# YoshikiMaekawa2000/ccv_mppi_path_tracker

Measured on AMD Instinct MI355X. Metric: trajectory rollouts/s (K×iters/s) + ms/MPPI-iteration, diff-drive T=50, higher is better.
Workload: dtype f64; 1 GPU; C2: diff_drive K=65536 T=50 sinusoid, u_dim=2, launch parameters; samples_per_gpu=65536, horizon=50, state_store=True

## Files before the change

ccv_mppi_path_tracker_amd/build.py:

```python
import os
import shutil
import subprocess

_PKG = os.path.dirname(os.path.abspath(__file__))
CSRC = os.path.join(_PKG, "csrc")
LIBDIR = os.path.join(_PKG, "lib")
LIB = os.path.join(LIBDIR, "libccv_mppi_hip.so")
KERNEL_UNITS = ["k_r4_fb.hip", "k_batch.hip", "k_batch_varied.hip", "k_batch_shift.hip", "k_batch_obst.hip", "k_batch_obst_shift.hip", "k_batch_moving.hip", "k_batch_moving_shift.hip", "k_batch_grid.hip", "k_batch_grid_shift.hip", "k_r4.hip", "k_r3.hip", "k_pc.hip", "k_pc_fb.hip",
                "k_solo.hip", "k_solo_fb.hip", "k_plain.hip", "k_update.hip", "k_fleet.hip", "k_fleet_pred.hip"]
CAPI_UNITS = ["ccv_mppi_capi.hip", "capi_exchange.hip", "capi_resident.hip", "capi_stage.hip", "capi_batch.hip"]
SOURCES = KERNEL_UNITS + ["mppi_launch.hip"] + CAPI_UNITS + ["ccv_mppi_host.cpp", os.path.join("host", "mppi_node.cpp")]
HEADERS = ["capi_internal.h", "mppi_diag.h", "mppi_kernels.h", "mppi_update.h", "mppi_launch.h", "mppi_rollout_pc.h", "mppi_rollout_r3.h", "mppi_rollout_r4.h",
           "mppi_rollout_solo.h", "k_batch_form.h", "mppi_resident.h", "mppi_update_device.h", "mppi_fleet.h", "mppi_fleet_device.h", "fast_trig.h", "noise_spec.h",
           os.path.join("..", "..", "include", "ccv_mppi.h"), os.path.join("..", "..", "include", "ccv_mppi_host.h"),
           os.path.join("..", "..", "include", "ccv_mppi_fleet.h"),
           os.path.join("..", "..", "include", "ccv_mppi_node.hpp")]
DEPS = SOURCES + HEADERS

HIPCC_FLAGS = [
    "--offload-arch=gfx950", "-O3", "-std=c++17", "-fPIC",
    "-ffp-contract=off",
    "-fhip-fp32-correctly-rounded-divide-sqrt",
    "-Wall", "-Wno-unused-result",
]


def hipcc():
    for cand in (shutil.which("hipcc"), "/opt/rocm/bin/hipcc"):
        if cand and os.path.exists(cand):
            return cand
    raise RuntimeError("hipcc not found: the MI355X path cannot be built (there is no CPU fallback)")


def stale():
    if not os.path.exists(LIB):
        return True
    t = os.path.getmtime(LIB)
    return any(os.path.getmtime(os.path.join(CSRC, d)) > t for d in DEPS)


def _run(cmd, verbose):
    if verbose:
        print(" ".join(cmd))
    res = subprocess.run(cmd, capture_output=True, text=True)
    if res.returncode != 0:
        raise RuntimeError("hipcc failed:\n" + " ".join(cmd) + "\n" + res.stdout + res.stderr)
    if verbose and res.stderr:
        print(res.stderr)


def build(force=False, verbose=False, extra_flags=(), out=None, jobs=None):
    if out is None and not force and not stale():
        return LIB
    os.makedirs(LIBDIR, exist_ok=True)
    target = out or LIB
    import fcntl
    with open(os.path.join(LIBDIR, ".build.lock"), "w") as lock:
        fcntl.flock(lock, fcntl.LOCK_EX)
        try:
            if out is None and not force and not stale():
                return LIB
            objdir = os.path.join(os.path.dirname(os.path.abspath(target)), "obj_%s_%d" % (os.path.basename(target), os.getpid()))
            os.makedirs(objdir, exist_ok=True)
            cc = hipcc()
            objs = [os.path.join(objdir, os.path.basename(s).rsplit(".", 1)[0] + ".o") for s in SOURCES]
            cmds = [[cc] + HIPCC_FLAGS + list(extra_flags) + ["-c", "-o", o, os.path.join(CSRC, s)] for s, o in zip(SOURCES, objs)]
            if jobs is None:
                try:
                    jobs = len(os.sched_getaffinity(0))
                except AttributeError:
                    jobs = os.cpu_count() or 1
                jobs = max(1, min(8, jobs))
            from concurrent.futures import ThreadPoolExecutor
            try:
                with ThreadPoolExecutor(jobs) as pool:
                    list(pool.map(lambda c: _run(c, verbose), cmds))
                tmp = target + ".tmp%d" % os.getpid()
                _run([cc, "--offload-arch=gfx950", "-fPIC", "-shared", "-o", tmp] + objs, verbose)
                os.replace(tmp, target)
            finally:
                shutil.rmtree(objdir, ignore_errors=True)
        finally:
            fcntl.flock(lock, fcntl.LOCK_UN)
    return target


if __name__ == "__main__":
    print(build(force=True, verbose=True))
```

ccv_mppi_path_tracker_amd/capi.py:

```python
import ctypes as C
import os

import numpy as np

from . import build as _build

MAX_UDIM = 5
MAX_HORIZON = 128
ABI_VERSION = 1

OK = 0
ERR_INVALID_ARG = -1
ERR_NO_DEVICE = -2
ERR_HIP = -3
ERR_STATE = -4
ERR_ALLOC = -5
ERR_TIMEOUT = -6

DIFF_DRIVE, STEERING_DIFF_DRIVE, FULL_BODY = 0, 1, 2
FLAG_ROLL_OFF, FLAG_STEER_OFF, FLAG_MIN_SHIFT, FLAG_NO_STATE_STORE = 0x1, 0x2, 0x4, 0x8
BATCH_MAX_SAMPLES = 1 << 29
BATCH_KERNEL_PLAIN, BATCH_KERNEL_ONE_WAVE, BATCH_KERNEL_FOUR_WAVE, BATCH_KERNEL_WIDE = 0, 1, 4, 16
BATCH_KERNEL_VARIED = 32
BATCH_KERNEL_SHIFT = 64
BATCH_KERNEL_OBST = 128
BATCH_KERNEL_MOVING = 256
BATCH_KERNEL_GRID = 512
MAX_OBSTACLES = 32
BATCH_TRACE_ROWS = 1024


class Config(C.Structure):
    _fields_ = [
        ("abi_version", C.c_int32), ("model", C.c_int32), ("num_samples", C.c_int32), ("horizon", C.c_int32),
        ("sample_offset", C.c_int32), ("device", C.c_int32), ("flags", C.c_int32), ("reserved", C.c_int32),
        ("control_noise", C.c_double), ("lam", C.c_double), ("v_ref", C.c_double),
        ("u_min", C.c_double * MAX_UDIM), ("u_max", C.c_double * MAX_UDIM),
        ("path_weight", C.c_double), ("v_weight", C.c_double), ("zmp_weight", C.c_double),
        ("roll_v_weight", C.c_double), ("back_weight", C.c_double), ("yaw_weight", C.c_double),
    ]


class Stats(C.Structure):
    _fields_ = [
        ("sum_w", C.c_double), ("min_cost", C.c_double), ("max_cost", C.c_double),
        ("n_zero_weight", C.c_int64), ("nonfinite", C.c_int32), ("reserved", C.c_int32),
        ("device_us", C.c_float), ("rollout_us", C.c_float),
    ]


class Grid(C.Structure):
    _fields_ = [
        ("origin_x", C.c_double), ("origin_y", C.c_double), ("resolution", C.c_double),
        ("outside", C.c_float), ("nx", C.c_int32), ("ny", C.c_int32), ("cells", C.POINTER(C.c_float)),
    ]


_dp = C.POINTER(C.c_double)
_H = C.c_void_p

SIGNATURES = {
    "ccv_mppi_create": (C.c_int, [C.POINTER(Config), C.POINTER(_H)]),
    "ccv_mppi_destroy": (C.c_int, [_H]),
    "ccv_mppi_set_stream": (C.c_int, [_H, C.c_void_p]),
    "ccv_mppi_last_error": (C.c_char_p, [_H]),
    "ccv_mppi_version": (C.c_char_p, []),
    "ccv_mppi_udim": (C.c_int, [C.c_int]),
    "ccv_mppi_set_nominal": (C.c_int, [_H, _dp]),
    "ccv_mppi_get_nominal": (C.c_int, [_H, _dp]),
    "ccv_mppi_iterate": (C.c_int, [_H, _dp, C.c_double, _dp, _dp, C.c_double, C.c_uint64, C.c_uint64, _dp,
                                   C.POINTER(Stats)]),
    "ccv_mppi_iterate_enqueue": (C.c_int, [_H, _dp, C.c_double, _dp, _dp, C.c_double, C.c_uint64, C.c_uint64]),
    "ccv_mppi_synchronize": (C.c_int, [_H]),
    "ccv_mppi_sample": (C.c_int, [_H, C.c_uint64, C.c_uint64]),
    "ccv_mppi_inject_controls": (C.c_int, [_H, _dp]),
    "ccv_mppi_rollout": (C.c_int, [_H, _dp, C.c_double]),
    "ccv_mppi_weights": (C.c_int, [_H, _dp, _dp, C.c_double]),
    "ccv_mppi_update": (C.c_int, [_H, _dp, C.POINTER(Stats)]),
    "ccv_mppi_read_candidates": (C.c_int, [_H, C.c_int32, C.c_int32, C.c_int32, _dp]),
    "ccv_mppi_read_top_candidates": (C.c_int, [_H, C.c_int32, C.POINTER(C.c_int32), _dp, _dp]),
    "ccv_mppi_read_costs": (C.c_int, [_H, C.c_int32, C.c_int32, _dp]),
    "ccv_mppi_read_weights": (C.c_int, [_H, C.c_int32, C.c_int32, _dp]),
    "ccv_mppi_read_controls": (C.c_int, [_H, C.c_int32, C.c_int32, _dp]),
    "ccv_mppi_partials_size": (C.c_int, [_H]),
    "ccv_mppi_iterate_partials_enqueue": (C.c_int, [_H, _dp, C.c_double, _dp, _dp, C.c_double, C.c_uint64,
                                                    C.c_uint64, C.c_void_p]),
    "ccv_mppi_apply_partials_enqueue": (C.c_int, [_H, C.c_void_p]),
    "ccv_mppi_exchange_handle_bytes": (C.c_int, []),
    "ccv_mppi_exchange_create": (C.c_int, [_H, C.c_int32, C.c_int32, C.c_void_p]),
    "ccv_mppi_exchange_connect": (C.c_int, [_H, C.c_void_p]),
    "ccv_mppi_exchange_info": (C.c_int, [_H, C.POINTER(C.c_int32), C.POINTER(C.c_int32), C.POINTER(C.c_int32), C.POINTER(C.c_int32)]),
    "ccv_mppi_iterate_exchange_enqueue": (C.c_int, [_H, _dp, C.c_double, _dp, _dp, C.c_double, C.c_uint64, C.c_uint64]),
    "ccv_mppi_resident_set_path": (C.c_int, [_H, _dp, _dp, C.c_int32, C.c_double]),
    "ccv_mppi_resident_set_pose": (C.c_int, [_H, _dp]),
    "ccv_mppi_resident_step_enqueue": (C.c_int, [_H, C.c_double, C.c_uint64, C.c_uint64, C.c_int32]),
    "ccv_mppi_resident_step_partials_enqueue": (C.c_int, [_H, C.c_double, C.c_uint64, C.c_uint64, C.c_int32, C.c_void_p]),
    "ccv_mppi_resident_step_exchange_enqueue": (C.c_int, [_H, C.c_double, C.c_uint64, C.c_uint64, C.c_int32]),
    "ccv_mppi_resident_read": (C.c_int, [_H, _dp, C.POINTER(C.c_int32), _dp, _dp, _dp, C.POINTER(C.c_int64)]),
    "ccv_mppi_resident_read_trace": (C.c_int, [_H, C.c_int32, _dp, C.POINTER(C.c_int32)]),
    "ccv_mppi_timing_enable": (C.c_int, [_H, C.c_int32]),
    "ccv_mppi_timing_read": (C.c_int, [_H, _dp, _dp, C.POINTER(C.c_int64), C.c_int32]),
    "ccv_mppi_batch_create": (C.c_int, [C.POINTER(Config), C.c_int32, C.POINTER(_H)]),
    "ccv_mppi_batch_destroy": (C.c_int, [_H]),
    "ccv_mppi_batch_set_stream": (C.c_int, [_H, C.c_void_p]),
    "ccv_mppi_batch_synchronize": (C.c_int, [_H]),
    "ccv_mppi_batch_last_error": (C.c_char_p, [_H]),
    "ccv_mppi_batch_size": (C.c_int, [_H]),
    "ccv_mppi_batch_last_kernel": (C.c_int, [_H]),
    "ccv_mppi_batch_set_nominal": (C.c_int, [_H, _dp]),
    "ccv_mppi_batch_get_nominal": (C.c_int, [_H, _dp]),
    "ccv_mppi_batch_set_params": (C.c_int, [_H, C.POINTER(Config)]),
    "ccv_mppi_batch_get_params": (C.c_int, [_H, C.POINTER(Config)]),
    "ccv_mppi_batch_set_min_shift": (C.c_int, [_H, C.c_int32]),
    "ccv_mppi_batch_get_min_shift": (C.c_int, [_H]),
    "ccv_mppi_batch_set_obstacles": (C.c_int, [_H, _dp, C.POINTER(C.c_int32), C.c_int32, _dp]),
    "ccv_mppi_batch_get_obstacles": (C.c_int, [_H, _dp, C.POINTER(C.c_int32), C.c_int32, _dp]),
    "ccv_mppi_batch_set_obstacle_velocities": (C.c_int, [_H, _dp, C.c_int32]),
    "ccv_mppi_batch_get_obstacle_velocities": (C.c_int, [_H, _dp, C.c_int32]),
    "ccv_mppi_batch_set_fleet_prediction": (C.c_int, [_H, C.c_int32]),
    "ccv_mppi_batch_get_fleet_prediction": (C.c_int, [_H]),
    "ccv_mppi_batch_read_fleet_velocities": (C.c_int, [_H, _dp]),
    "ccv_mppi_batch_set_grids": (C.c_int, [_H, C.POINTER(Grid), C.c_int32, C.POINTER(C.c_int32), _dp]),
    "ccv_mppi_batch_get_grids": (C.c_int, [_H, C.POINTER(Grid), C.c_int32, C.POINTER(C.c_int32), C.POINTER(C.c_int32), _dp]),
    "ccv_mppi_batch_read_grid_cells": (C.c_int, [_H, C.c_int32, C.POINTER(C.c_float)]),
    "ccv_mppi_batch_iterate": (C.c_int, [_H, _dp, _dp, _dp, _dp, _dp, C.POINTER(C.c_uint64), C.c_uint64, _dp,
                                         C.POINTER(Stats)]),
    "ccv_mppi_batch_iterate_enqueue": (C.c_int, [_H, _dp, _dp, _dp, _dp, _dp, C.POINTER(C.c_uint64), C.c_uint64]),
    "ccv_mppi_batch_read_costs": (C.c_int, [_H, C.c_int32, C.c_int32, C.c_int32, _dp]),
    "ccv_mppi_batch_read_weights": (C.c_int, [_H, C.c_int32, C.c_int32, C.c_int32, _dp]),
    "ccv_mppi_batch_read_candidates": (C.c_int, [_H, C.c_int32, C.c_int32, C.c_int32, C.c_int32, _dp]),
    "ccv_mppi_batch_timing_enable": (C.c_int, [_H, C.c_int32]),
    "ccv_mppi_batch_timing_read": (C.c_int, [_H, _dp, _dp, C.POINTER(C.c_int64), C.c_int32]),
    "ccv_mppi_batch_resident_set_paths": (C.c_int, [_H, _dp, _dp, C.POINTER(C.c_int32), _dp]),
    "ccv_mppi_batch_resident_set_poses": (C.c_int, [_H, _dp, C.POINTER(C.c_uint64)]),
    "ccv_mppi_batch_resident_step_enqueue": (C.c_int, [_H, C.c_double, C.c_uint64, C.c_int32]),
    "ccv_mppi_batch_resident_read": (C.c_int, [_H, _dp, C.POINTER(C.c_int32), _dp, _dp, _dp, C.POINTER(C.c_int64)]),
    "ccv_mppi_batch_resident_read_trace": (C.c_int, [_H, C.c_int32, C.c_int32, _dp, C.POINTER(C.c_int32)]),
    "ccv_mppi_calc_ref_path": (C.c_int, [_dp, _dp, C.c_int32, C.c_double, C.c_double, C.c_double, C.c_double,
                                         C.c_double, C.c_int32, _dp, _dp, _dp]),
    "ccv_mppi_path_cosine": (C.c_int, [_dp, _dp, _dp, C.c_double, C.c_double, C.c_double, C.c_double, _dp, _dp,
                                       C.c_int32]),
    "ccv_mppi_path_dkan": (C.c_int, [C.c_double, _dp, _dp, C.c_int32]),
    "ccv_mppi_plant_step": (C.c_int, [C.c_int32, _dp, _dp, C.c_double]),
    "ccv_mppi_node_create": (C.c_int, [C.c_int, C.POINTER(C.c_char_p), _dp, C.c_int, C.c_int, C.POINTER(_H)]),
    "ccv_mppi_node_destroy": (C.c_int, [_H]),
    "ccv_mppi_node_set_path": (C.c_int, [_H, _dp, _dp, C.c_int]),
    "ccv_mppi_node_set_state": (C.c_int, [_H, _dp]),
    "ccv_mppi_node_set_seed": (C.c_int, [_H, C.c_uint64]),
    "ccv_mppi_node_set_fused": (C.c_int, [_H, C.c_int]),
    "ccv_mppi_node_set_device_prologue": (C.c_int, [_H, C.c_int]),
    "ccv_mppi_node_run_once": (C.c_int, [_H, C.c_double, _dp]),
    "ccv_mppi_node_get_optimal": (C.c_int, [_H, _dp]),
    "ccv_mppi_node_get_ref_path": (C.c_int, [_H, _dp]),
    "ccv_mppi_node_get_optimal_path": (C.c_int, [_H, _dp]),
    "ccv_mppi_node_fb_imu": (C.c_int, [_H, _dp, _dp, _dp, _dp]),
    "ccv_mppi_node_fb_wrench": (C.c_int, [_H, C.c_int, _dp, _dp]),
    "ccv_mppi_node_fb_pose": (C.c_int, [_H, C.c_double, C.c_double, C.c_double]),
    "ccv_mppi_node_fb_update_state": (C.c_int, [_H, C.c_double]),
    "ccv_mppi_node_fb_read": (C.c_int, [_H, _dp]),
    "ccv_mppi_fb_estimator_create": (C.c_int, [C.POINTER(_H)]),
    "ccv_mppi_fb_estimator_destroy": (C.c_int, [_H]),
    "ccv_mppi_fb_estimator_imu": (C.c_int, [_H, _dp, _dp, _dp, _dp]),
    "ccv_mppi_fb_estimator_wrench": (C.c_int, [_H, C.c_int, _dp, _dp]),
    "ccv_mppi_fb_estimator_update": (C.c_int, [_H, C.c_double, C.c_double, C.c_double, C.c_double]),
    "ccv_mppi_fb_estimator_read": (C.c_int, [_H, _dp]),
}
FLEET_SIGNATURES = {
    "ccv_mppi_batch_resident_set_fleet": (C.c_int, [_H, _dp, C.c_double, C.c_int32, _dp]),
    "ccv_mppi_batch_resident_get_fleet": (C.c_int, [_H, _dp, C.POINTER(C.c_double), C.POINTER(C.c_int32)]),
    "ccv_mppi_batch_resident_read_fleet": (C.c_int, [_H, C.POINTER(C.c_int32), C.POINTER(C.c_int32), _dp]),
}

_lib = None


def load():
    global _lib
    if _lib is None:
        path = os.environ.get("CCV_MPPI_LIB") or _build.build()
        if not os.path.exists(path):
            raise ImportError("libccv_mppi_hip.so is missing and could not be built; there is no CPU fallback")
        lib = C.CDLL(path)
        for name, (res, args) in list(SIGNATURES.items()) + list(FLEET_SIGNATURES.items()):
            fn = getattr(lib, name)
            fn.restype = res
            fn.argtypes = args
        _lib = lib
    return _lib


def dptr(a):
    return a.ctypes.data_as(_dp)


def as_f64(a, shape=None):
    a = np.ascontiguousarray(a, dtype=np.float64)
    if shape is not None and tuple(a.shape) != tuple(shape):
        raise ValueError("expected shape %s, got %s" % (shape, a.shape))
    return a
```

ccv_mppi_path_tracker_amd/controller.py:

```python
import ctypes as C

import numpy as np

from . import capi
from .configs import MODEL_IDS, MPPIParams


class MPPIError(RuntimeError):
    def __init__(self, code, msg):
        super().__init__("ccv_mppi error %d: %s" % (code, msg))
        self.code = code


def make_config(p: MPPIParams, device=0, sample_offset=0, min_shift=False, no_state_store=False, num_samples=None):
    cfg = capi.Config()
    cfg.abi_version = capi.ABI_VERSION
    cfg.model = MODEL_IDS[p.model]
    cfg.num_samples = int(num_samples if num_samples is not None else p.num_samples)
    cfg.horizon = int(p.horizon)
    cfg.sample_offset = int(sample_offset)
    cfg.device = int(device)
    cfg.flags = ((capi.FLAG_ROLL_OFF if p.roll_off else 0) | (capi.FLAG_STEER_OFF if p.steer_off else 0) |
                 (capi.FLAG_MIN_SHIFT if min_shift else 0) | (capi.FLAG_NO_STATE_STORE if no_state_store else 0))
    cfg.control_noise, cfg.lam, cfg.v_ref = p.control_noise, p.lam, p.v_ref
    for d in range(p.udim):
        cfg.u_min[d], cfg.u_max[d] = p.u_min[d], p.u_max[d]
    cfg.path_weight, cfg.v_weight, cfg.zmp_weight = p.path_weight, p.v_weight, p.zmp_weight
    cfg.roll_v_weight, cfg.back_weight, cfg.yaw_weight = p.roll_v_weight, p.back_weight, p.yaw_weight
    return cfg


class MPPIController:

    def __init__(self, params: MPPIParams, device=0, sample_offset=0, num_samples=None, min_shift=False,
                 no_state_store=False):
        self.lib = capi.load()
        self.params = params
        self.K = int(num_samples if num_samples is not None else params.num_samples)
        self.H = params.horizon
        self.udim = params.udim
        self.nstate = params.nstate
        self._h = capi._H()
        cfg = make_config(params, device, sample_offset, min_shift, no_state_store, self.K)
        rc = self.lib.ccv_mppi_create(C.byref(cfg), C.byref(self._h))
        if rc != capi.OK:
            self._h = capi._H()
            raise MPPIError(rc, "ccv_mppi_create failed (no usable MI355X/HIP device?) -- there is no CPU fallback")

    def _check(self, rc):
        if rc != capi.OK:
            msg = self.lib.ccv_mppi_last_error(self._h)
            raise MPPIError(rc, msg.decode() if msg else "")

    def close(self):
        if getattr(self, "_h", None) and self._h.value:
            self.lib.ccv_mppi_destroy(self._h)
            self._h = capi._H()

    def __del__(self):
        try:
            self.close()
        except Exception:
            pass

    def _x0(self, x0):
        x = np.zeros(5)
        x[:len(x0)] = x0
        return x

    def set_stream(self, stream_ptr):
        self._check(self.lib.ccv_mppi_set_stream(self._h, C.c_void_p(stream_ptr)))

    def synchronize(self):
        self._check(self.lib.ccv_mppi_synchronize(self._h))

    def set_nominal(self, u):
        u = capi.as_f64(u, (self.H - 1, self.udim))
        self._check(self.lib.ccv_mppi_set_nominal(self._h, capi.dptr(u)))

    def get_nominal(self):
        u = np.empty((self.H - 1, self.udim))
        self._check(self.lib.ccv_mppi_get_nominal(self._h, capi.dptr(u)))
        return u

    def iterate(self, x0, dt, x_ref, y_ref, yaw_ref0, seed, iteration, want_stats=True):
        x = self._x0(x0)
        xr, yr = capi.as_f64(x_ref, (self.H,)), capi.as_f64(y_ref, (self.H,))
        u = np.empty((self.H - 1, self.udim))
        st = capi.Stats()
        self._check(self.lib.ccv_mppi_iterate(self._h, capi.dptr(x), float(dt), capi.dptr(xr), capi.dptr(yr),
                                              float(yaw_ref0), int(seed), int(iteration), capi.dptr(u),
                                              C.byref(st) if want_stats else None))
        return (u, st) if want_stats else u

    def iterate_enqueue(self, x0, dt, x_ref, y_ref, yaw_ref0, seed, iteration):
        x = self._x0(x0)
        xr, yr = capi.as_f64(x_ref, (self.H,)), capi.as_f64(y_ref, (self.H,))
        self._check(self.lib.ccv_mppi_iterate_enqueue(self._h, capi.dptr(x), float(dt), capi.dptr(xr), capi.dptr(yr),
                                                      float(yaw_ref0), int(seed), int(iteration)))

    def sampling(self, seed, iteration):
        self._check(self.lib.ccv_mppi_sample(self._h, int(seed), int(iteration)))

    def inject_controls(self, u_samples):
        u = capi.as_f64(u_samples, (self.K, self.H - 1, self.udim))
        self._check(self.lib.ccv_mppi_inject_controls(self._h, capi.dptr(u)))

    def predict_States(self, x0, dt):
        x = self._x0(x0)
        self._check(self.lib.ccv_mppi_rollout(self._h, capi.dptr(x), float(dt)))

    def calc_Weights(self, x_ref, y_ref, yaw_ref0=0.0):
        xr, yr = capi.as_f64(x_ref, (self.H,)), capi.as_f64(y_ref, (self.H,))
        self._check(self.lib.ccv_mppi_weights(self._h, capi.dptr(xr), capi.dptr(yr), float(yaw_ref0)))

    def determine_OptimalSolution(self, want_stats=False):
        u = np.empty((self.H - 1, self.udim))
        st = capi.Stats()
        self._check(self.lib.ccv_mppi_update(self._h, capi.dptr(u), C.byref(st)))
        return (u, st) if want_stats else u

    def read_candidates(self, first=0, count=None, stride=1):
        count = self.K if count is None else count
        out = np.empty((count, self.H, 2))
        self._check(self.lib.ccv_mppi_read_candidates(self._h, first, count, stride, capi.dptr(out)))
        return out

    def read_top_candidates(self, count, with_paths=True):
        idx = np.empty(count, dtype=np.int32)
        wts = np.empty(count)
        xy = np.empty((count, self.H, 2)) if with_paths else None
        self._check(self.lib.ccv_mppi_read_top_candidates(self._h, int(count), idx.ctypes.data_as(C.POINTER(C.c_int32)),
                                                          capi.dptr(wts), capi.dptr(xy) if with_paths else None))
        return idx, wts, xy

    def read_costs(self, first=0, count=None):
        count = self.K - first if count is None else count
        out = np.empty(count)
        self._check(self.lib.ccv_mppi_read_costs(self._h, first, count, capi.dptr(out)))
        return out

    def read_weights(self, first=0, count=None):
        count = self.K - first if count is None else count
        out = np.empty(count)
        self._check(self.lib.ccv_mppi_read_weights(self._h, first, count, capi.dptr(out)))
        return out

    def read_controls(self, first=0, count=None):
        count = self.K - first if count is None else count
        out = np.empty((count, self.H - 1, self.udim))
        self._check(self.lib.ccv_mppi_read_controls(self._h, first, count, capi.dptr(out)))
        return out

    def partials_size(self):
        return self.lib.ccv_mppi_partials_size(self._h)

    def iterate_partials_enqueue(self, x0, dt, x_ref, y_ref, yaw_ref0, seed, iteration, dev_ptr):
        x = self._x0(x0)
        xr, yr = capi.as_f64(x_ref, (self.H,)), capi.as_f64(y_ref, (self.H,))
        self._check(self.lib.ccv_mppi_iterate_partials_enqueue(
            self._h, capi.dptr(x), float(dt), capi.dptr(xr), capi.dptr(yr), float(yaw_ref0), int(seed),
            int(iteration), C.c_void_p(dev_ptr)))

    def apply_partials_enqueue(self, dev_ptr):
        self._check(self.lib.ccv_mppi_apply_partials_enqueue(self._h, C.c_void_p(dev_ptr)))

    def exchange_create(self, world, rank):
        buf = C.create_string_buffer(self.lib.ccv_mppi_exchange_handle_bytes())
        self._check(self.lib.ccv_mppi_exchange_create(self._h, int(world), int(rank), C.cast(buf, C.c_void_p)))
        return bytes(buf.raw)

    def exchange_connect(self, handles):
        blob = b"".join(handles)
        buf = C.create_string_buffer(blob, len(blob))
        self._check(self.lib.ccv_mppi_exchange_connect(self._h, C.cast(buf, C.c_void_p)))

    def exchange_info(self):
        w, r, f, c = C.c_int32(), C.c_int32(), C.c_int32(), C.c_int32()
        self._check(self.lib.ccv_mppi_exchange_info(self._h, C.byref(w), C.byref(r), C.byref(f), C.byref(c)))
        return {"world": w.value, "rank": r.value, "fine_grained": bool(f.value), "connected": bool(c.value)}

    def iterate_exchange_enqueue(self, x0, dt, x_ref, y_ref, yaw_ref0, seed, iteration):
        x = self._x0(x0)
        xr, yr = capi.as_f64(x_ref, (self.H,)), capi.as_f64(y_ref, (self.H,))
        self._check(self.lib.ccv_mppi_iterate_exchange_enqueue(
            self._h, capi.dptr(x), float(dt), capi.dptr(xr), capi.dptr(yr), float(yaw_ref0), int(seed), int(iteration)))

    def resident_set_path(self, path_x, path_y, resolution=None):
        px, py = capi.as_f64(path_x), capi.as_f64(path_y)
        res = self.params.resolution if resolution is None else resolution
        self._check(self.lib.ccv_mppi_resident_set_path(self._h, capi.dptr(px), capi.dptr(py), len(px), float(res)))

    def resident_set_pose(self, state):
        x = self._x0(state)
        self._check(self.lib.ccv_mppi_resident_set_pose(self._h, capi.dptr(x)))

    def resident_step_enqueue(self, dt, seed, iteration, advance=True):
        self._check(self.lib.ccv_mppi_resident_step_enqueue(self._h, float(dt), int(seed), int(iteration),
                                                            1 if advance else 0))

    def resident_step_partials_enqueue(self, dt, seed, iteration, advance, dev_ptr):
        self._check(self.lib.ccv_mppi_resident_step_partials_enqueue(self._h, float(dt), int(seed), int(iteration),
                                                                     1 if advance else 0, C.c_void_p(dev_ptr)))

    def resident_step_exchange_enqueue(self, dt, seed, iteration, advance=True):
        self._check(self.lib.ccv_mppi_resident_step_exchange_enqueue(self._h, float(dt), int(seed), int(iteration),
                                                                     1 if advance else 0))

    def resident_read(self):
        st = np.zeros(5)
        xr, yr = np.zeros(self.H), np.zeros(self.H)
        idx, yaw0, steps = C.c_int32(), C.c_double(), C.c_int64()
        self._check(self.lib.ccv_mppi_resident_read(self._h, capi.dptr(st), C.byref(idx), capi.dptr(xr), capi.dptr(yr),
                                                    C.byref(yaw0), C.byref(steps)))
        return st[:self.params.nstate].copy(), idx.value, xr, yr, yaw0.value, steps.value

    def resident_read_trace(self, max_rows=8192):
        rows = np.zeros((max_rows, 6))
        n = C.c_int32()
        self._check(self.lib.ccv_mppi_resident_read_trace(self._h, int(max_rows), capi.dptr(rows), C.byref(n)))
        return rows[:n.value].copy()

    def timing_enable(self, on=True, every=1):
        self._check(self.lib.ccv_mppi_timing_enable(self._h, (max(1, int(every)) if on else 0)))

    def timing_read(self, reset=True):
        a, b, n = C.c_double(), C.c_double(), C.c_int64()
        self._check(self.lib.ccv_mppi_timing_read(self._h, C.byref(a), C.byref(b), C.byref(n), 1 if reset else 0))
        return a.value, b.value, n.value



def calc_ref_path(path_x, path_y, cur_x, cur_y, v_ref, dt, resolution, horizon):
    lib = capi.load()
    px, py = capi.as_f64(path_x), capi.as_f64(path_y)
    xr, yr, yaw = np.zeros(horizon), np.zeros(horizon), np.zeros(horizon)
    idx = lib.ccv_mppi_calc_ref_path(capi.dptr(px), capi.dptr(py), len(px), cur_x, cur_y, v_ref, dt, resolution,
                                     horizon, capi.dptr(xr), capi.dptr(yr), capi.dptr(yaw))
    if idx < 0:
        raise MPPIError(idx, "ccv_mppi_calc_ref_path")
    return idx, xr, yr, yaw


def make_path(kind, resolution=0.1, length=None):
    lib = capi.load()
    cap = 4096 if length is None else int(length / resolution) + 16
    px, py = np.zeros(cap), np.zeros(cap)
    if kind == "dkan":
        n = lib.ccv_mppi_path_dkan(resolution, capi.dptr(px), capi.dptr(py), cap)
    else:
        if kind == "straight":
            A, om, de, course = (0.0, 0.0, 0.0), (0.0, 0.0, 0.0), (1.57, 1.57, 1.57), 10.0
        elif kind == "sinusoid":
            A, om, de, course = (1.0, 0.0, 0.0), (0.25, 0.0, 0.0), (0.0, 0.0, 0.0), 10.0
        else:
            raise KeyError(kind)
        A, om, de = capi.as_f64(A), capi.as_f64(om), capi.as_f64(de)
        n = lib.ccv_mppi_path_cosine(capi.dptr(A), capi.dptr(om), capi.dptr(de), resolution,
                                     course if length is None else float(length), 0.0, 0.0,
                                     capi.dptr(px), capi.dptr(py), cap)
    if n < 0:
        raise MPPIError(n, "path generator")
    return px[:n].copy(), py[:n].copy()


def plant_step(model, state, u, dt):
    lib = capi.load()
    s = capi.as_f64(state).copy()
    s5 = np.zeros(5)
    s5[:len(s)] = s
    uu = np.zeros(5)
    uu[:len(u)] = u
    rc = lib.ccv_mppi_plant_step(MODEL_IDS[model], capi.dptr(s5), capi.dptr(uu), float(dt))
    if rc != capi.OK:
        raise MPPIError(rc, "ccv_mppi_plant_step")
    return s5[:len(s)]
```

ccv_mppi_path_tracker_amd/csrc/capi_internal.h:

```cpp
#pragma once
#include <hip/hip_runtime.h>
#include <hip/hip_ext.h>

#include <cmath>
#include <cstddef>
#include <cstdint>
#include <cstdio>
#include <cstdlib>
#include <cstring>
#include <string>
#include <vector>

#include "fast_trig.h"
#include "mppi_kernels.h"
#include "mppi_launch.h"
#include "mppi_update.h"
#include "mppi_resident.h"
#include "mppi_fleet.h"

namespace ccv {

struct Shape {
    ccv_mppi_config cfg{};
    int udim = 0, K = 0, H = 0, R = 0, pitch = 0, nchunks = 0, nblocks = 0;
    int cu_count = 256;
};

struct KernelChoice {
    KernelFamily stagewise = KernelFamily::FourWave;
    KernelFamily fused = KernelFamily::FourWave;
    int lds_window = 1;
    bool fast_clamp_allowed = true;
    int prio_rotate = 0;
    int prune = 0;
};

struct DeviceBuffers {
    hipStream_t own_stream = nullptr;
    hipStream_t stream = nullptr;
    double* d_nominal = nullptr;
    double* d_u = nullptr;
    void* d_arena = nullptr;
    float* d_z = nullptr;
    double* d_nom_used = nullptr;
    bool controls_in_z = false;
    double* d_xs = nullptr;
    double* d_ys = nullptr;
    double* d_cost = nullptr;
    double* d_w = nullptr;
    double* d_partial = nullptr;
    double* d_statpart = nullptr;
    double* d_vec = nullptr;
    double* d_stats = nullptr;
    unsigned long long* d_dbg = nullptr;
    double* d_scratch = nullptr;
    size_t scratch_bytes = 0;
    int nparts_last = 0;
    double inj_absmax[CCV_MPPI_MAX_UDIM] = {0, 0, 0, 0, 0};
    double nom_absmax[CCV_MPPI_MAX_UDIM] = {0, 0, 0, 0, 0};
};

struct Mailbox {
    double* h_pin = nullptr;
    size_t pin_doubles = 0;
    unsigned long long* h_mail = nullptr;
    unsigned long long* d_mail = nullptr;
    uint32_t mail_seq = 0;
    bool want_mail = false;
    bool mail_pending = false;
    bool use_mail = true;
};

struct Throttle {
    static constexpr int kThrottleEvery = 16, kThrottleSlots = 3;
    hipEvent_t throttle_ev[kThrottleSlots] = {nullptr, nullptr, nullptr};
    bool throttle_used[kThrottleSlots] = {false, false, false};
    uint64_t enqueued = 0;
    bool throttle = true;
};

struct Timing {
    bool timing = false;
    int timing_every = 1;
    int64_t timing_count = 0;
    std::vector<hipEvent_t> ev;
    bool timed_now = false;
    size_t ev_slot = 0;
    size_t ev_used = 0;
    double t_roll_sum = 0.0, t_iter_sum = 0.0;
    int64_t t_n = 0;
    float last_iter_us = 0.f, last_roll_us = 0.f;
};

struct UpdatePlan {
    FinalizeArgs args{};
    int batch = 0;
    bool fused = true;
    const BatchParams* shift = nullptr;
    int K = 0;
};

struct DeferredUpdate {
    bool fin_pending = false;
    UpdatePlan fin{};
};

struct Core : Shape, KernelChoice, DeviceBuffers, Mailbox, Throttle, Timing, DeferredUpdate {
    std::string err;
};

struct StageState {
    bool have_controls = false, have_rollout = false, have_weights = false;
    double st_x0[5] = {0, 0, 0, 0, 0};
    double st_dt = 0.1;
    double* d_cmin = nullptr;
};

struct ResidentLoop {
    ResidentFrame* d_frame = nullptr;
    double* d_path = nullptr;
    double* d_trace = nullptr;
    static constexpr int kTraceRows = 8192;
    int n_path = 0;
    double path_resolution = 0.0;
    bool have_pose = false;
    int64_t res_steps = 0;
    double res_angle_abs[3] = {0, 0, 0};
};

struct Exchange {
    ExchangeBox* d_box = nullptr;
    ExchangeBox* box_peer[kMaxRanks] = {nullptr};
    bool box_opened[kMaxRanks] = {false};
    double* d_xvec = nullptr;
    int32_t* h_xflag = nullptr;
    int32_t* d_xflag = nullptr;
    double xchg_timeout_s = 10.0;
    int xchg_world = 0, xchg_rank = 0;
    bool xchg_connected = false;
    bool box_fine_grained = false;
    uint32_t xchg_nonce = 0;
    uint32_t xchg_base = 0;
    unsigned long long xchg_seq = 0;
    unsigned long long xchg_timeout_ticks = 1000000000ull;
};

}

using namespace ccv;

struct ccv_mppi_handle : Core, StageState, ResidentLoop, Exchange {
    const double* pending_vec = nullptr;
};

struct ccv_mppi_batch : Core {
    int B = 0, kpad = 0, rec_doubles = 0;
    double* d_rec = nullptr;
    static constexpr int kRecSlots = 4;
    double* h_rec[kRecSlots] = {nullptr, nullptr, nullptr, nullptr};
    hipEvent_t rec_ev[kRecSlots] = {nullptr, nullptr, nullptr, nullptr};
    bool rec_used[kRecSlots] = {false, false, false, false};
    int rec_next = 0;
    int last_kernel = -1;
    bool mail_any_size = false;
    bool have_result = false;
    ResidentFrame* d_rframe = nullptr;
    BatchInstance* d_inst = nullptr;
    double* d_rpath = nullptr;
    double* d_rtrace = nullptr;
    int64_t n_total = 0;
    std::vector<BatchInstance> inst;
    std::vector<double> res_angle_abs;
    bool have_paths = false, have_poses = false;
    int64_t res_steps = 0;
    bool varied = false;
    std::vector<ccv_mppi_config> cfgs;
    BatchParams* d_params = nullptr;
    bool min_shift = false;
    double* d_cmin = nullptr;
    bool obst = false;
    double* d_obst = nullptr;
    std::vector<double> obst_xyr;
    std::vector<int32_t> obst_n;
    std::vector<double> obst_w;
    bool moving = false;
    double* d_obst_v = nullptr;
    std::vector<double> obst_vxy;
    bool grid = false;
    GridRow* d_grid_rows = nullptr;
    float* d_grid_cells = nullptr;
    std::vector<ccv_mppi_grid> grid_maps;
    std::vector<size_t> grid_offset;
    std::vector<int32_t> grid_map_of;
    std::vector<double> grid_w;
    bool shift_result = false;
    bool fleet = false;
    double* d_fleet_xy = nullptr;
    double* d_fleet_radius = nullptr;
    int32_t* d_fleet_nstatic = nullptr;
    std::vector<double> fleet_radius;
    double fleet_range = 0.0;
    int32_t fleet_maxn = 0;
    bool fleet_pred = false;
    double* d_fleet_v = nullptr;
};

namespace ccv {

inline int fail(Core* h, int code, const char* what, hipError_t e = hipSuccess) {
    if (h) {
        h->err = what;
        if (e != hipSuccess) {
            h->err += ": ";
            h->err += hipGetErrorString(e);
        }
    }
    return code;
}

#define HIP_TRY(h, call)                                                            \
    do {                                                                            \
        hipError_t e__ = (call);                                                    \
        if (e__ != hipSuccess) return fail((h), CCV_MPPI_ERR_HIP, #call, e__);      \
    } while (0)

inline int round_up(int v, int m) { return (v + m - 1) / m * m; }

struct DeviceGuard {
    int prev = -1, mine = -1;
    explicit DeviceGuard(int device) : mine(device) {
        if (hipGetDevice(&prev) != hipSuccess) prev = -1;
    }
    ~DeviceGuard() {
        if (prev >= 0 && prev != mine) (void)hipSetDevice(prev);
    }
};

int check_config(const ccv_mppi_config* cfg);
int check_device(int device);
void set_shape(Shape& s, const ccv_mppi_config& cfg, int pitch, int nblocks);
void select_kernels(KernelChoice& k, const Shape& s, int64_t workgroups, bool batched);
struct BufferCounts {
    size_t nparts_max;
    size_t nominal, vec, stats;
    double** extra;
    size_t n_extra;
    size_t pin_doubles, mail_slots;
};
int create_buffers(Core* h, const BufferCounts& n);
void release_buffers(Core* h);
int set_stream(Core* h, void* hip_stream);
hipError_t ensure_scratch(DeviceBuffers& d, size_t bytes);

enum : int { kTrigUnsafe = 0, kTrigSafe = 1, kTrigWide = 2 };
int fast_trig_safe(const Core* h, const ccv_mppi_config& c, const RolloutArgs& A, int mode, bool has_wide);
inline KernelFamily family_of(const KernelChoice& k, const int mode) { return mode == MODE_FUSED ? k.fused : k.stagewise; }
inline bool has_wide_form(const KernelChoice& k, const int mode) {
    return mode == MODE_FUSED && (k.fused == KernelFamily::FourWave || k.fused == KernelFamily::OneWave);
}
inline RolloutPlan make_plan(const KernelChoice& k, const int model, const int mode, const int trig, const int batch, const BatchForm form,
                             const bool shift) {
    KernelFamily f = trig == kTrigUnsafe ? KernelFamily::Plain : family_of(k, mode);
    if (f == KernelFamily::OneWave && !has_one_wave_form(model, form)) f = KernelFamily::FourWave;
    return RolloutPlan{f, model, mode, f != KernelFamily::Plain && trig == kTrigWide, batch, form, shift, k.lds_window != 0};
}

RolloutPlan plan_of(const ccv_mppi_handle* h, const RolloutArgs& A, int mode);

void fill_params(const ccv_mppi_config& c, bool fast_clamp_allowed, RolloutArgs& A);
void fill_args(const Core* h, RolloutArgs& A, const double* x0, double dt, double yaw_ref0, uint64_t seed, uint64_t iter);
void window_coeffs(int H, const double* x_ref, const double* y_ref, double px, double py, double* a, double* b, double* c);
void track_absmax(const double* u, size_t n, int udim, double* absmax);
void launch_finalize(Core& h, const UpdatePlan& p);
void launch_finalize_advance(Core& h, const UpdatePlan& p, const AdvanceArgs& V);
void launch_finalize_advance(Core& h, const UpdatePlan& p, const BatchAdvanceArgs& G, BatchParams* table, const FleetArgs* fleet = nullptr,
                             const FleetPredArgs* pred = nullptr);
int flush_finalize(Core* h);
int flush_division(ccv_mppi_handle* h);
int flush_pending(ccv_mppi_handle* h);
int materialize_controls(ccv_mppi_handle* h);
int launch_rollout(ccv_mppi_handle* h, const RolloutArgs& A, const Window& W, int mode);
int launch_sample(ccv_mppi_handle* h, const RolloutArgs& A);
UpdateArgs update_args(const Core* h);
FinalizeArgs finalize_args(const Core* h, double* vec, int nparts, bool normalise);
void post_to_mail(Mailbox& m, FinalizeArgs& F);
int launch_update(ccv_mppi_handle* h, bool normalise, double* vec_out, bool exchange = false, bool defer = false);
int check_iter_args(ccv_mppi_handle* h, const double* x0, double dt, const double* x_ref, const double* y_ref);
int enqueue_iteration(ccv_mppi_handle* h, const double* x0, double dt, const double* x_ref, const double* y_ref, double yaw_ref0,
                      uint64_t seed, uint64_t iter, bool normalise, double* vec_out, bool resident = false, bool exchange = false);
hipError_t throttle_tick(Throttle& t, hipStream_t stream);
hipError_t timing_begin(Timing& t);
hipError_t timing_rollout_at(const Timing& t, hipStream_t stream, bool plain, LaunchAt& at);
hipError_t timing_rollout_done(const Timing& t, hipStream_t stream, bool plain);
hipError_t timing_end(Timing& t, hipStream_t stream);
hipError_t timing_collect(Timing& t, hipStream_t stream);
int timing_enable(Core* h, int32_t on);
int timing_read(Core* h, double* rollout_us_sum, double* iter_us_sum, int64_t* n_iters, int32_t reset);
int read_mail(Core* h, size_t n_slots, double* out);
void unpack_result(const Timing& t, int R, const double* v, double* u_opt_out, ccv_mppi_stats* stats);
int fetch_result(ccv_mppi_handle* h, double* u_opt_out, ccv_mppi_stats* stats);

void exchange_release(ccv_mppi_handle* h);
int exchange_check(ccv_mppi_handle* h);

struct FrameHead {
    double x0[5];
    double yaw_ref0;
    int32_t index, steps;
};
static_assert(offsetof(ResidentFrame, W) == sizeof(FrameHead), "frame head layout");
struct ResidentBounds {
    double angle[3];
    double heading;
};
ResidentBounds resident_bounds(const DeviceBuffers& d, const ccv_mppi_config& c, const double* angle_abs, double dt, int32_t advance);
hipError_t read_trace_ring(const double* d_ring, int64_t cap, int64_t steps, int32_t max_rows, double* rows, int32_t* n_rows);

}
```

ccv_mppi_path_tracker_amd/csrc/capi_stage.hip:

```cpp
#include <algorithm>

#include "capi_internal.h"

extern "C" {


int ccv_mppi_sample(ccv_mppi_handle* h, uint64_t seed, uint64_t iter) {
    if (!h) return CCV_MPPI_ERR_INVALID_ARG;
    RolloutArgs A;
    const double zero[5] = {0, 0, 0, 0, 0};
    fill_args(h, A, zero, 0.1, 0.0, seed, iter);
    int rc = launch_sample(h, A);
    if (rc) return rc;
    for (int d = 0; d < h->udim; ++d) h->inj_absmax[d] = std::fmax(std::fabs(h->cfg.u_min[d]), std::fabs(h->cfg.u_max[d]));
    h->controls_in_z = false;
    h->have_controls = true;
    h->have_rollout = h->have_weights = false;
    return CCV_MPPI_OK;
}

int ccv_mppi_inject_controls(ccv_mppi_handle* h, const double* u_samples) {
    if (!h || !u_samples) return CCV_MPPI_ERR_INVALID_ARG;
    std::vector<double> tmp((size_t)h->R * h->pitch, 0.0);
    for (int d = 0; d < CCV_MPPI_MAX_UDIM; ++d) h->inj_absmax[d] = 0.0;
    for (int i = 0; i < h->K; ++i)
        for (int n = 0; n < h->R; ++n) {
            const double v = u_samples[(size_t)i * h->R + n];
            tmp[(size_t)n * h->pitch + i] = v;
            const int d = n % h->udim;
            if (!(std::fabs(v) <= h->inj_absmax[d])) h->inj_absmax[d] = std::fabs(v);
        }
    HIP_TRY(h, hipMemcpyAsync(h->d_u, tmp.data(), tmp.size() * sizeof(double), hipMemcpyHostToDevice, h->stream));
    HIP_TRY(h, hipStreamSynchronize(h->stream));
    h->controls_in_z = false;
    h->have_controls = true;
    h->have_rollout = h->have_weights = false;
    return CCV_MPPI_OK;
}

int ccv_mppi_rollout(ccv_mppi_handle* h, const double* x0, double dt) {
    if (!h || !x0) return CCV_MPPI_ERR_INVALID_ARG;
    if (!h->have_controls) return fail(h, CCV_MPPI_ERR_STATE, "ccv_mppi_rollout before ccv_mppi_sample/inject_controls");
    RolloutArgs A;
    Window W;
    std::memset(&W, 0, sizeof(W));
    fill_args(h, A, x0, dt, 0.0, 0, 0);
    A.store_u = 0;
    A.store_xy = 1;
    A.do_cost = 0;
    int rc = launch_rollout(h, A, W, MODE_ROLLOUT);
    if (rc) return rc;
    std::memcpy(h->st_x0, A.x0, sizeof(h->st_x0));
    h->st_dt = dt;
    h->have_rollout = true;
    h->have_weights = false;
    return CCV_MPPI_OK;
}

int ccv_mppi_weights(ccv_mppi_handle* h, const double* x_ref, const double* y_ref, double yaw_ref0) {
    if (!h || !x_ref || !y_ref) return CCV_MPPI_ERR_INVALID_ARG;
    if (!h->have_rollout) return fail(h, CCV_MPPI_ERR_STATE, "ccv_mppi_weights before ccv_mppi_rollout");
    RolloutArgs A;
    Window W;
    fill_args(h, A, h->st_x0, h->st_dt, yaw_ref0, 0, 0);
    window_coeffs(h->H, x_ref, y_ref, h->st_x0[0], h->st_x0[1], W.a, W.b, W.c);
    A.store_u = 0;
    A.store_xy = 0;
    A.do_cost = 1;
    int rc = launch_rollout(h, A, W, MODE_COST);
    if (rc) return rc;
    rc = launch_update(h, false, nullptr);
    if (rc) return rc;
    h->have_weights = true;
    return CCV_MPPI_OK;
}

int ccv_mppi_update(ccv_mppi_handle* h, double* u_opt_out, ccv_mppi_stats* stats) {
    if (!h) return CCV_MPPI_ERR_INVALID_ARG;
    if (!h->have_weights) return fail(h, CCV_MPPI_ERR_STATE, "ccv_mppi_update before ccv_mppi_weights");
    h->want_mail = !(stats && h->timing);
    int rc = launch_update(h, true, nullptr);
    h->want_mail = false;
    if (rc) return rc;
    return fetch_result(h, u_opt_out, stats);
}


int ccv_mppi_read_candidates(ccv_mppi_handle* h, int32_t first, int32_t count, int32_t stride, double* xy_out) {
    if (!h || !xy_out || first < 0 || count < 0 || stride < 1) return CCV_MPPI_ERR_INVALID_ARG;
    if (h->cfg.flags & CCV_MPPI_FLAG_NO_STATE_STORE) return fail(h, CCV_MPPI_ERR_STATE, "state buffer disabled (NO_STATE_STORE)");
    if (!h->have_rollout) return fail(h, CCV_MPPI_ERR_STATE, "no rollout yet");
    if (count == 0) return CCV_MPPI_OK;
    if ((int64_t)first + (int64_t)(count - 1) * stride >= h->K) return fail(h, CCV_MPPI_ERR_INVALID_ARG, "candidate range exceeds num_samples");
    const size_t n = (size_t)count * h->H * 2;
    HIP_TRY(h, ensure_scratch(*h, n * sizeof(double)));
    hipLaunchKernelGGL(k_gather_xy, dim3((count * h->H + kBlock - 1) / kBlock), dim3(kBlock), 0, h->stream, h->d_xs, h->d_ys,
                       h->pitch, h->H, first, count, stride, h->d_scratch);
    HIP_TRY(h, hipGetLastError());
    HIP_TRY(h, hipMemcpyAsync(xy_out, h->d_scratch, n * sizeof(double), hipMemcpyDeviceToHost, h->stream));
    HIP_TRY(h, hipStreamSynchronize(h->stream));
    return CCV_MPPI_OK;
}

int ccv_mppi_read_top_candidates(ccv_mppi_handle* h, int32_t count, int32_t* sample_out, double* weight_out, double* xy_out) {
    if (!h || !sample_out || count < 0) return CCV_MPPI_ERR_INVALID_ARG;
    if (!h->have_weights) return fail(h, CCV_MPPI_ERR_STATE, "no weights yet");
    if (count > h->K) return fail(h, CCV_MPPI_ERR_INVALID_ARG, "count exceeds num_samples");
    if (xy_out && (h->cfg.flags & CCV_MPPI_FLAG_NO_STATE_STORE)) return fail(h, CCV_MPPI_ERR_STATE, "state buffer disabled (NO_STATE_STORE)");
    if (count == 0) return CCV_MPPI_OK;
    const size_t n_xy = xy_out ? (size_t)count * h->H * 2 : 0;
    HIP_TRY(h, ensure_scratch(*h, ((size_t)count * 2 + n_xy) * sizeof(double)));
    int* d_idx = reinterpret_cast<int*>(h->d_scratch);
    double* d_wsel = h->d_scratch + count;
    double* d_xy = h->d_scratch + 2 * (size_t)count;
    hipLaunchKernelGGL(k_top_weights, dim3(1), dim3(kTopBlock), 0, h->stream, h->d_w, h->K, count, d_idx, d_wsel);
    HIP_TRY(h, hipGetLastError());
    std::vector<int> idx(count);
    std::vector<double> wsel(count);
    HIP_TRY(h, hipMemcpyAsync(idx.data(), d_idx, (size_t)count * sizeof(int), hipMemcpyDeviceToHost, h->stream));
    HIP_TRY(h, hipMemcpyAsync(wsel.data(), d_wsel, (size_t)count * sizeof(double), hipMemcpyDeviceToHost, h->stream));
    HIP_TRY(h, hipStreamSynchronize(h->stream));
    std::vector<int> order(count);
    for (int i = 0; i < count; ++i) order[i] = i;
    auto key = [&](int i) { return (unsigned long long)*reinterpret_cast<const long long*>(&wsel[i]); };
    std::sort(order.begin(), order.end(), [&](int a, int b) { return key(a) != key(b) ? key(a) > key(b) : idx[a] < idx[b]; });
    std::vector<int> sorted_idx(count);
    for (int i = 0; i < count; ++i) {
        sorted_idx[i] = idx[order[i]];
        sample_out[i] = sorted_idx[i];
        if (weight_out) weight_out[i] = wsel[order[i]];
    }
    if (xy_out) {
        HIP_TRY(h, hipMemcpyAsync(d_idx, sorted_idx.data(), (size_t)count * sizeof(int), hipMemcpyHostToDevice, h->stream));
        hipLaunchKernelGGL(k_gather_xy_list, dim3((count * h->H + kBlock - 1) / kBlock), dim3(kBlock), 0, h->stream, h->d_xs, h->d_ys,
                           h->pitch, h->H, d_idx, count, d_xy);
        HIP_TRY(h, hipGetLastError());
        HIP_TRY(h, hipMemcpyAsync(xy_out, d_xy, n_xy * sizeof(double), hipMemcpyDeviceToHost, h->stream));
        HIP_TRY(h, hipStreamSynchronize(h->stream));
    }
    return CCV_MPPI_OK;
}

static int check_range(ccv_mppi_handle* h, int32_t first, int32_t count, const void* out) {
    if (!h || !out || first < 0 || count < 0) return CCV_MPPI_ERR_INVALID_ARG;
    if ((int64_t)first + count > h->K) return fail(h, CCV_MPPI_ERR_INVALID_ARG, "range exceeds num_samples");
    return CCV_MPPI_OK;
}

int ccv_mppi_read_costs(ccv_mppi_handle* h, int32_t first, int32_t count, double* out) {
    int rc = check_range(h, first, count, out);
    if (rc) return rc;
    if (!h->have_weights) return fail(h, CCV_MPPI_ERR_STATE, "no costs yet");
    HIP_TRY(h, hipMemcpyAsync(out, h->d_cost + first, (size_t)count * sizeof(double), hipMemcpyDeviceToHost, h->stream));
    HIP_TRY(h, hipStreamSynchronize(h->stream));
    return CCV_MPPI_OK;
}

int ccv_mppi_read_weights(ccv_mppi_handle* h, int32_t first, int32_t count, double* out) {
    int rc = check_range(h, first, count, out);
    if (rc) return rc;
    if (!h->have_weights) return fail(h, CCV_MPPI_ERR_STATE, "no weights yet");
    if (count == 0) return CCV_MPPI_OK;
    if ((rc = flush_pending(h)) != CCV_MPPI_OK) return rc;
    HIP_TRY(h, ensure_scratch(*h, (size_t)count * sizeof(double)));
    hipLaunchKernelGGL(k_normalise_weights, dim3((count + kBlock - 1) / kBlock), dim3(kBlock), 0, h->stream, h->d_w, h->d_stats,
                       first, count, h->d_scratch);
    HIP_TRY(h, hipGetLastError());
    HIP_TRY(h, hipMemcpyAsync(out, h->d_scratch, (size_t)count * sizeof(double), hipMemcpyDeviceToHost, h->stream));
    HIP_TRY(h, hipStreamSynchronize(h->stream));
    return CCV_MPPI_OK;
}

int ccv_mppi_read_controls(ccv_mppi_handle* h, int32_t first, int32_t count, double* out) {
    int rc = check_range(h, first, count, out);
    if (rc) return rc;
    if (!h->have_controls) return fail(h, CCV_MPPI_ERR_STATE, "no controls yet");
    if (count == 0) return CCV_MPPI_OK;
    std::vector<double> tmp((size_t)h->R * count);
    HIP_TRY(h, hipStreamSynchronize(h->stream));
    if (h->controls_in_z) {
        std::vector<float> zt((size_t)h->R * count);
        std::vector<double> nom((size_t)h->R);
        HIP_TRY(h, hipMemcpy2D(zt.data(), (size_t)count * sizeof(float), h->d_z + first, (size_t)h->pitch * sizeof(float),
                               (size_t)count * sizeof(float), (size_t)h->R, hipMemcpyDeviceToHost));
        HIP_TRY(h, hipMemcpy(nom.data(), h->d_nom_used, (size_t)h->R * sizeof(double), hipMemcpyDeviceToHost));
        const bool steer_off = h->cfg.model == CCV_MPPI_FULL_BODY && (h->cfg.flags & CCV_MPPI_FLAG_STEER_OFF);
        for (int n = 0; n < h->R; ++n) {
            const int d = n % h->udim;
            const double lo = h->cfg.u_min[d], hi = h->cfg.u_max[d], sigma = h->cfg.control_noise;
            for (int i = 0; i < count; ++i) {
                const double prod = (double)zt[(size_t)n * count + i] * sigma;
                double v = prod + nom[n];
                v = v < lo ? lo : (v > hi ? hi : v);
                if (steer_off && d == 2) v = 0.0;
                tmp[(size_t)n * count + i] = v;
            }
        }
    } else
    HIP_TRY(h, hipMemcpy2D(tmp.data(), (size_t)count * sizeof(double), h->d_u + first, (size_t)h->pitch * sizeof(double),
                           (size_t)count * sizeof(double), (size_t)h->R, hipMemcpyDeviceToHost));
    for (int i = 0; i < count; ++i)
        for (int n = 0; n < h->R; ++n) out[(size_t)i * h->R + n] = tmp[(size_t)n * count + i];
    return CCV_MPPI_OK;
}


#if defined(CCV_DIAG)
extern "C" int ccv_mppi_debug_blocks(ccv_mppi_handle* h, unsigned long long* out, int nblocks) {
    if (!h || !out || nblocks < 0 || nblocks > kDiagBlocks) return CCV_MPPI_ERR_INVALID_ARG;
    HIP_TRY(h, hipStreamSynchronize(h->stream));
    HIP_TRY(h, hipMemcpy(out, h->d_dbg + kDiagHeader, (size_t)nblocks * kDiagSlots * sizeof(unsigned long long), hipMemcpyDeviceToHost));
    return CCV_MPPI_OK;
}
#endif


int ccv_mppi_timing_enable(ccv_mppi_handle* h, int32_t on) { return h ? timing_enable(h, on) : CCV_MPPI_ERR_INVALID_ARG; }

int ccv_mppi_timing_read(ccv_mppi_handle* h, double* rollout_us_sum, double* iter_us_sum, int64_t* n_iters, int32_t reset) {
    return h ? timing_read(h, rollout_us_sum, iter_us_sum, n_iters, reset) : CCV_MPPI_ERR_INVALID_ARG;
}

int ccv_mppi_batch_timing_enable(ccv_mppi_batch* bh, int32_t on) { return bh ? timing_enable(bh, on) : CCV_MPPI_ERR_INVALID_ARG; }

int ccv_mppi_batch_timing_read(ccv_mppi_batch* bh, double* rollout_us_sum, double* iter_us_sum, int64_t* n_iters, int32_t reset) {
    return bh ? timing_read(bh, rollout_us_sum, iter_us_sum, n_iters, reset) : CCV_MPPI_ERR_INVALID_ARG;
}

}
```

ccv_mppi_path_tracker_amd/csrc/ccv_mppi_capi.hip:

```cpp
#include <chrono>
#include <new>

#include "capi_internal.h"

namespace ccv {

hipError_t ensure_scratch(DeviceBuffers& d, size_t bytes) {
    if (bytes <= d.scratch_bytes) return hipSuccess;
    if (d.d_scratch) {
        if (hipError_t e = hipFree(d.d_scratch)) return e;
    }
    d.d_scratch = nullptr;
    d.scratch_bytes = 0;
    if (hipError_t e = hipMalloc(&d.d_scratch, bytes)) return e;
    d.scratch_bytes = bytes;
    return hipSuccess;
}

void fill_params(const ccv_mppi_config& c, const bool fast_clamp_allowed, RolloutArgs& A) {
    A.sigma = c.control_noise;
    A.lambda = c.lambda;
    A.v_ref = c.v_ref;
    for (int d = 0; d < CCV_MPPI_MAX_UDIM; ++d) {
        A.umin[d] = c.u_min[d];
        A.umax[d] = c.u_max[d];
    }
    A.fast_clamp = std::isfinite(c.control_noise) ? 1 : 0;
    for (int d = 0; d < udim_of(c.model); ++d)
        if (!(c.u_min[d] <= c.u_max[d])) A.fast_clamp = 0;
    if (!fast_clamp_allowed) A.fast_clamp = 0;
    const bool roll_off = (c.flags & CCV_MPPI_FLAG_ROLL_OFF) != 0;
    A.w_path = c.path_weight;
    A.w_v = c.v_weight;
    A.w_zmp = roll_off ? 0.0 : c.zmp_weight;
    A.w_rollv = roll_off ? 0.0 : c.roll_v_weight;
    A.w_back = c.back_weight;
    A.w_yaw = c.yaw_weight;
}

void fill_args(const Core* h, RolloutArgs& A, const double* x0, double dt, double yaw_ref0, uint64_t seed,
               uint64_t iter) {
    const ccv_mppi_config& c = h->cfg;
    std::memset(&A, 0, sizeof(A));
    const int nx = c.model == CCV_MPPI_FULL_BODY ? 5 : 3;
    for (int i = 0; i < nx; ++i) A.x0[i] = x0[i];
    A.dt = dt;
    A.yaw_ref0 = yaw_ref0;
    fill_params(c, h->fast_clamp_allowed, A);
    const double upper_body_height = 0.8075, upper_body_width = 0.208, mass = 60.0;
    const double base2CoM = upper_body_height / 2;
    A.fb_mass = mass;
    A.fb_L = base2CoM;
    A.fb_Ixx = (mass * (upper_body_width * upper_body_width + upper_body_height * upper_body_height)) / 12 + mass * base2CoM * base2CoM;
    A.fb_gz = -9.8;
    A.inv_dt = 1.0 / dt;
    A.seed_lo = (uint32_t)seed;
    A.seed_hi = (uint32_t)(seed >> 32);
    A.iter_lo = (uint32_t)iter;
    A.iter_hi = (uint32_t)(iter >> 32);
    A.K = h->K;
    A.pitch = h->pitch;
    A.H = h->H;
    A.k_offset = c.sample_offset;
    A.steer_off = (c.flags & CCV_MPPI_FLAG_STEER_OFF) ? 1 : 0;
    A.nominal = h->d_nominal;
    A.u = h->d_u;
    A.z = h->d_z;
    A.nominal_used = h->d_nom_used;
    A.xs = h->d_xs;
    A.ys = h->d_ys;
    A.cost = h->d_cost;
    A.w = h->d_w;
    A.partial = h->d_partial;
    A.statpart = h->d_statpart;
    A.nparts = h->nblocks;
    A.fuse_update = 0;
    A.prio_rotate = h->prio_rotate;
    A.pending_vec = nullptr;
    A.nominal_w = h->d_nominal;
    A.stats_w = h->d_stats;
    A.cu_count = h->cu_count;
    A.prune = h->prune;
    A.dbg = h->d_dbg;
}

void window_coeffs(const int H, const double* x_ref, const double* y_ref, const double px, const double py, double* a, double* b,
                   double* c) {
    for (int j = 0; j < H; ++j) {
        const double xl = x_ref[j] - px, yl = y_ref[j] - py;
        a[j] = -2.0 * xl;
        b[j] = -2.0 * yl;
        c[j] = xl * xl + yl * yl;
    }
}

void launch_finalize(Core& h, const UpdatePlan& p) {
    const unsigned blocks = finalize_blocks(p.args.R);
    if (p.batch && p.shift) hipLaunchKernelGGL(k_finalize_batch_shift, dim3(blocks, p.batch), dim3(kBlock), 0, h.stream, p.args, p.shift, p.K);
    else if (p.batch) hipLaunchKernelGGL(k_finalize_batch, dim3(blocks, p.batch), dim3(kBlock), 0, h.stream, p.args, p.fused ? 1 : 0);
    else hipLaunchKernelGGL(k_finalize, dim3(blocks), dim3(kBlock), 0, h.stream, p.args);
}

void launch_finalize_advance(Core& h, const UpdatePlan& p, const AdvanceArgs& V) {
    hipLaunchKernelGGL(k_finalize_advance, dim3(finalize_blocks(p.args.R) + 1), dim3(kBlock), 0, h.stream, p.args, V);
}

void launch_finalize_advance(Core& h, const UpdatePlan& p, const BatchAdvanceArgs& G, BatchParams* table, const FleetArgs* fleet,
                             const FleetPredArgs* pred) {
    const dim3 grid(finalize_blocks(p.args.R) + 1, p.batch);
    if (fleet && pred && p.shift)
        hipLaunchKernelGGL(k_finalize_advance_batch_shift_fleet_pred, grid, dim3(kBlock), 0, h.stream, p.args, G, table, *fleet, *pred);
    else if (fleet && pred) hipLaunchKernelGGL(k_finalize_advance_batch_fleet_pred, grid, dim3(kBlock), 0, h.stream, p.args, G, table, *fleet, *pred);
    else if (fleet && p.shift) hipLaunchKernelGGL(k_finalize_advance_batch_shift_fleet, grid, dim3(kBlock), 0, h.stream, p.args, G, table, *fleet);
    else if (fleet) hipLaunchKernelGGL(k_finalize_advance_batch_fleet, grid, dim3(kBlock), 0, h.stream, p.args, G, table, *fleet);
    else if (p.shift) hipLaunchKernelGGL(k_finalize_advance_batch_shift, grid, dim3(kBlock), 0, h.stream, p.args, G, p.shift);
    else if (table) hipLaunchKernelGGL(k_finalize_advance_batch_varied, grid, dim3(kBlock), 0, h.stream, p.args, G, table);
    else hipLaunchKernelGGL(k_finalize_advance_batch, grid, dim3(kBlock), 0, h.stream, p.args, G);
}

int flush_finalize(Core* h) {
    if (!h->fin_pending) return CCV_MPPI_OK;
    launch_finalize(*h, h->fin);
    h->fin_pending = false;
    HIP_TRY(h, hipGetLastError());
    return CCV_MPPI_OK;
}

int flush_division(ccv_mppi_handle* h) {
    if (!h->pending_vec) return CCV_MPPI_OK;
    hipLaunchKernelGGL(k_apply_partials, dim3(1), dim3(kBlock), 0, h->stream, h->pending_vec, h->d_nominal, h->d_stats, h->R);
    h->pending_vec = nullptr;
    HIP_TRY(h, hipGetLastError());
    return CCV_MPPI_OK;
}

int flush_pending(ccv_mppi_handle* h) {
    if (int rc = flush_finalize(h)) return rc;
    return flush_division(h);
}

int materialize_controls(ccv_mppi_handle* h) {
    if (!h->controls_in_z) return CCV_MPPI_OK;
    MaterializeArgs M;
    M.z = h->d_z;
    M.nominal_used = h->d_nom_used;
    M.u = h->d_u;
    M.sigma = h->cfg.control_noise;
    for (int d = 0; d < CCV_MPPI_MAX_UDIM; ++d) {
        M.umin[d] = h->cfg.u_min[d];
        M.umax[d] = h->cfg.u_max[d];
    }
    M.K = h->K;
    M.pitch = h->pitch;
    M.R = h->R;
    M.udim = h->udim;
    M.zero_dim = (h->cfg.model == CCV_MPPI_FULL_BODY && (h->cfg.flags & CCV_MPPI_FLAG_STEER_OFF)) ? 2 : -1;
    hipLaunchKernelGGL(k_materialize_controls, dim3((h->K + kBlock - 1) / kBlock, h->R), dim3(kBlock), 0, h->stream, M);
    HIP_TRY(h, hipGetLastError());
    h->controls_in_z = false;
    return CCV_MPPI_OK;
}

int fast_trig_safe(const Core* h, const ccv_mppi_config& c, const RolloutArgs& A, const int mode, const bool has_wide) {
    const int ud = h->udim;
    double umax[CCV_MPPI_MAX_UDIM];
    for (int d = 0; d < ud; ++d) {
        umax[d] = mode == MODE_FUSED ? std::fmax(std::fabs(c.u_min[d]), std::fabs(c.u_max[d])) : h->inj_absmax[d];
    }
    const double steps = (double)(h->H - 1) * std::fabs(A.dt);
    double bound = std::fabs(A.x0[2]) + steps * umax[1];
    if (h->cfg.model != CCV_MPPI_DIFF_DRIVE) bound += umax[2];
    if (h->cfg.model == CCV_MPPI_FULL_BODY) {
        bound = std::fmax(bound, std::fabs(A.x0[3]) + steps * umax[3]);
        bound = std::fmax(bound, std::fabs(A.x0[4]) + steps * umax[4]);
    }
    bool wide = false;
    if (h->cfg.model == CCV_MPPI_DIFF_DRIVE && !(umax[1] * std::fabs(A.dt) <= kSmallTurnLimit)) {
        if (!has_wide) return kTrigUnsafe;
        wide = true;
    }
    if (h->cfg.model == CCV_MPPI_FULL_BODY) {
        if (!(umax[1] * std::fabs(A.dt) <= kSmallTurnLimit) || !(umax[3] * std::fabs(A.dt) <= kSmallTurnLimit) ||
            !(umax[4] * std::fabs(A.dt) <= kSmallTurnLimit) || !(umax[2] <= kSmallTurnLimit))
            return kTrigUnsafe;
        if (!(std::fabs(A.dt) >= 1.0e-100 && std::fabs(A.dt) <= 1.0e100) || !(umax[0] <= 1.0e100) || !(umax[3] <= 1.0e100)) return kTrigUnsafe;
    }
    if (!(bound <= kFastTrigLimit)) return kTrigUnsafe;
    return wide ? kTrigWide : kTrigSafe;
}

RolloutPlan plan_of(const ccv_mppi_handle* h, const RolloutArgs& A, const int mode) {
    return make_plan(*h, h->cfg.model, mode, fast_trig_safe(h, h->cfg, A, mode, has_wide_form(*h, mode)), 0, BatchForm::Single, false);
}

int launch_rollout(ccv_mppi_handle* h, const RolloutArgs& A_in, const Window& W, int mode) {
    RolloutArgs A = A_in;
    const RolloutPlan plan = plan_of(h, A, mode);
    const bool coop = plan.family != KernelFamily::Plain;
    A.fuse_update = (coop && mode != MODE_ROLLOUT && !(h->cfg.flags & CCV_MPPI_FLAG_MIN_SHIFT)) ? 1 : 0;
    if (int rc = flush_finalize(h)) return rc;
    if (h->pending_vec) {
        if (coop && mode == MODE_FUSED) {
            A.pending_vec = h->pending_vec;
            h->pending_vec = nullptr;
        } else {
            if (int rc = flush_division(h)) return rc;
        }
    }
    if (mode != MODE_ROLLOUT) h->nparts_last = A.fuse_update ? h->nblocks : 0;
    if (mode != MODE_FUSED) {
        if (int rc = materialize_controls(h)) return rc;
    }
    LaunchAt at{h->stream, nullptr, nullptr};
    if (mode == MODE_FUSED) HIP_TRY(h, timing_rollout_at(*h, h->stream, !coop, at));
    launch_rollout(plan, at, A, W);
    if (mode == MODE_FUSED) HIP_TRY(h, timing_rollout_done(*h, h->stream, !coop));
    HIP_TRY(h, hipGetLastError());
    if (mode == MODE_FUSED) h->controls_in_z = coop;
    return CCV_MPPI_OK;
}

int launch_sample(ccv_mppi_handle* h, const RolloutArgs& A) {
    if (int rc = flush_pending(h)) return rc;
    launch_sample(h->cfg.model, h->stream, A);
    HIP_TRY(h, hipGetLastError());
    return CCV_MPPI_OK;
}

UpdateArgs update_args(const Core* h) {
    UpdateArgs U;
    U.u = h->d_u;
    U.w = h->d_w;
    U.cost = h->d_cost;
    U.partial = h->d_partial;
    U.statpart = h->d_statpart;
    U.K = h->K;
    U.pitch = h->pitch;
    U.R = h->R;
    U.nchunks = h->nchunks;
    return U;
}

FinalizeArgs finalize_args(const Core* h, double* vec, const int nparts, const bool normalise) {
    FinalizeArgs F;
    F.partial = h->d_partial;
    F.statpart = h->d_statpart;
    F.nominal = h->d_nominal;
    F.vec = vec;
    F.stats = h->d_stats;
    F.R = h->R;
    F.nchunks = nparts;
    F.normalise = normalise ? 1 : 0;
    F.mail = nullptr;
    F.mail_seq = 0;
    return F;
}

void post_to_mail(Mailbox& m, FinalizeArgs& F) {
    if (++m.mail_seq == 0) m.mail_seq = 1;
    F.mail = m.d_mail;
    F.mail_seq = m.mail_seq;
    m.mail_pending = true;
}

int launch_update(ccv_mppi_handle* h, bool normalise, double* vec_out, bool exchange, bool defer) {
    if (h->fin_pending) {
        if (int rc = flush_pending(h)) return rc;
    }
    int nparts = h->nparts_last;
    if (nparts == 0) {
        if (int rc = materialize_controls(h)) return rc;
        if (h->cfg.flags & CCV_MPPI_FLAG_MIN_SHIFT) {
            hipLaunchKernelGGL(k_min_cost, dim3(1), dim3(1024), 0, h->stream, h->d_cost, h->K, h->d_cmin);
            hipLaunchKernelGGL(k_reweight, dim3((h->K + kBlock - 1) / kBlock), dim3(kBlock), 0, h->stream, h->d_cost, h->d_cmin,
                               h->cfg.lambda, h->K, h->d_w);
        }
        hipLaunchKernelGGL(k_update_partials, dim3(h->nchunks, h->R + 1), dim3(kBlock), 0, h->stream, update_args(h));
        nparts = h->nchunks;
    }
    FinalizeArgs F = finalize_args(h, vec_out ? vec_out : h->d_vec, nparts, normalise);
    const bool post = h->want_mail && h->use_mail && normalise && !exchange && !defer && h->d_mail;
    h->want_mail = false;
    if (post) post_to_mail(*h, F);
    if (exchange) {
        ExchangeArgs X;
        for (int r = 0; r < kMaxRanks; ++r) X.peer[r] = h->box_peer[r];
        X.local = h->d_box;
        X.reduced = h->d_xvec;
        ++h->xchg_seq;
        X.seq = (uint32_t)(((unsigned long long)h->xchg_base + h->xchg_seq) % 0xFFFFFFFFull) + 1u;
        X.timeout_flag = h->d_xflag;
        X.world = h->xchg_world;
        X.rank = h->xchg_rank;
        X.parity = (int)(h->xchg_seq & 1);
        X.timeout_ticks = h->xchg_timeout_ticks;
        hipLaunchKernelGGL(k_finalize_exchange, dim3(finalize_blocks(h->R)), dim3(kBlock), 0, h->stream, F, X);
        HIP_TRY(h, hipGetLastError());
        h->pending_vec = h->d_xvec;
        return CCV_MPPI_OK;
    }
    if (defer && nparts == h->nblocks && normalise) {
        h->fin = UpdatePlan{F};
        h->fin_pending = true;
        return CCV_MPPI_OK;
    }
    launch_finalize(*h, UpdatePlan{F});
    HIP_TRY(h, hipGetLastError());
    return CCV_MPPI_OK;
}

hipError_t timing_begin(Timing& t) {
    t.timed_now = t.timing && (t.timing_count++ % t.timing_every) == 0;
    if (!t.timed_now) return hipSuccess;
    const size_t slot = t.ev_slot = t.ev_used;
    if (t.ev.size() < slot + 3) {
        for (int i = 0; i < 3; ++i) {
            hipEvent_t e;
            if (hipError_t err = hipEventCreate(&e)) return err;
            t.ev.push_back(e);
        }
    }
    t.ev_used += 3;
    return hipSuccess;
}

hipError_t timing_rollout_at(const Timing& t, hipStream_t stream, const bool plain, LaunchAt& at) {
    at = LaunchAt{stream, nullptr, nullptr};
    if (!t.timed_now) return hipSuccess;
    if (plain) return hipEventRecord(t.ev[t.ev_slot], stream);
    at = LaunchAt{stream, t.ev[t.ev_slot], t.ev[t.ev_slot + 1]};
    return hipSuccess;
}

hipError_t timing_rollout_done(const Timing& t, hipStream_t stream, const bool plain) {
    return t.timed_now && plain ? hipEventRecord(t.ev[t.ev_slot + 1], stream) : hipSuccess;
}

hipError_t timing_end(Timing& t, hipStream_t stream) {
    const bool timed = t.timed_now;
    t.timed_now = false;
    return timed ? hipEventRecord(t.ev[t.ev_slot + 2], stream) : hipSuccess;
}

hipError_t throttle_tick(Throttle& t, hipStream_t stream) {
    if (!t.throttle || ++t.enqueued % Throttle::kThrottleEvery != 0) return hipSuccess;
    const int ts = (int)((t.enqueued / Throttle::kThrottleEvery) % Throttle::kThrottleSlots);
    if (t.throttle_used[ts]) {
        if (hipError_t e = hipEventSynchronize(t.throttle_ev[ts])) return e;
    }
    if (hipError_t e = hipEventRecord(t.throttle_ev[ts], stream)) return e;
    t.throttle_used[ts] = true;
    return hipSuccess;
}

hipError_t timing_collect(Timing& t, hipStream_t stream) {
    if (t.ev_used == 0) return hipSuccess;
    if (hipError_t e = hipStreamSynchronize(stream)) return e;
    for (size_t s = 0; s + 3 <= t.ev_used; s += 3) {
        float a = 0.f, b = 0.f;
        if (hipError_t e = hipEventElapsedTime(&a, t.ev[s], t.ev[s + 1])) return e;
        if (hipError_t e = hipEventElapsedTime(&b, t.ev[s], t.ev[s + 2])) return e;
        t.t_roll_sum += (double)a * 1000.0;
        t.t_iter_sum += (double)b * 1000.0;
        t.t_n += 1;
        t.last_roll_us = a * 1000.f;
        t.last_iter_us = b * 1000.f;
    }
    t.ev_used = 0;
    return hipSuccess;
}

int timing_enable(Core* h, const int32_t on) {
    HIP_TRY(h, timing_collect(*h, h->stream));
    h->timing = on != 0;
    h->timing_every = on > 1 ? on : 1;
    h->timing_count = 0;
    return CCV_MPPI_OK;
}

int timing_read(Core* h, double* rollout_us_sum, double* iter_us_sum, int64_t* n_iters, const int32_t reset) {
    HIP_TRY(h, timing_collect(*h, h->stream));
    if (rollout_us_sum) *rollout_us_sum = h->t_roll_sum;
    if (iter_us_sum) *iter_us_sum = h->t_iter_sum;
    if (n_iters) *n_iters = h->t_n;
    if (reset) {
        h->t_roll_sum = h->t_iter_sum = 0.0;
        h->t_n = 0;
    }
    return CCV_MPPI_OK;
}

int check_iter_args(ccv_mppi_handle* h, const double* x0, double dt, const double* x_ref, const double* y_ref) {
    if (!h) return CCV_MPPI_ERR_INVALID_ARG;
    if (!x0 || !x_ref || !y_ref) return fail(h, CCV_MPPI_ERR_INVALID_ARG, "null pointer argument");
    if (!(dt == dt)) return fail(h, CCV_MPPI_ERR_INVALID_ARG, "dt is NaN");
    return CCV_MPPI_OK;
}

int enqueue_iteration(ccv_mppi_handle* h, const double* x0, double dt, const double* x_ref, const double* y_ref,
                      double yaw_ref0, uint64_t seed, uint64_t iter, bool normalise, double* vec_out, bool resident, bool exchange) {
    RolloutArgs A;
    Window W;
    fill_args(h, A, x0, dt, yaw_ref0, seed, iter);
    if (resident) {
        std::memset(&W, 0, sizeof(W));
        A.frame = h->d_frame;
        if (plan_of(h, A, MODE_FUSED).family == KernelFamily::Plain)
            return fail(h, CCV_MPPI_ERR_STATE, "the resident loop needs the cooperative kernels and bounded pose angles");
    } else {
        window_coeffs(h->H, x_ref, y_ref, x0[0], x0[1], W.a, W.b, W.c);
    }
    A.store_u = 1;
    A.store_xy = (h->cfg.flags & CCV_MPPI_FLAG_NO_STATE_STORE) ? 0 : 1;
    A.do_cost = 1;
    HIP_TRY(h, timing_begin(*h));
    int rc = launch_rollout(h, A, W, MODE_FUSED);
    if (rc) return rc;
    rc = launch_update(h, normalise, vec_out, exchange, resident && normalise && !vec_out && !exchange && !h->timed_now);
    if (rc) return rc;
    HIP_TRY(h, timing_end(*h, h->stream));
    HIP_TRY(h, throttle_tick(*h, h->stream));
    std::memcpy(h->st_x0, A.x0, sizeof(h->st_x0));
    h->st_dt = dt;
    h->have_controls = h->have_rollout = h->have_weights = true;
    return CCV_MPPI_OK;
}

int read_mail(Core* h, const size_t n_slots, double* out) {
    const uint32_t seq = h->mail_seq;
    volatile unsigned long long* m = h->h_mail;
    const auto t0 = std::chrono::steady_clock::now();
    size_t next = 0;
    bool synced = false;
    for (unsigned spin = 0; next < n_slots; ++spin) {
        while (next < n_slots && (uint32_t)m[2 * next] == seq && (uint32_t)m[2 * next + 1] == seq) ++next;
        if (next == n_slots) break;
        if (synced) return fail(h, CCV_MPPI_ERR_HIP, "the update kernel finished without posting its result");
        asm volatile("" ::: "memory");
        if ((spin & 1023u) == 1023u) {
            const double waited = std::chrono::duration<double>(std::chrono::steady_clock::now() - t0).count();
            if (waited > 1.0e-3) {
                HIP_TRY(h, hipStreamSynchronize(h->stream));
                synced = true;
            }
        }
    }
    for (size_t i = 0; i < n_slots; ++i) {
        const unsigned long long hi = h->h_mail[2 * i], lo = h->h_mail[2 * i + 1];
        const unsigned long long bits = (hi & 0xFFFFFFFF00000000ull) | (lo >> 32);
        std::memcpy(&out[i], &bits, sizeof(double));
    }
    return CCV_MPPI_OK;
}

void unpack_result(const Timing& t, const int R, const double* v, double* u_opt_out, ccv_mppi_stats* stats) {
    const size_t n = (size_t)R;
    int nonfinite = 0;
    for (size_t i = 0; i < n; ++i) {
        if (!std::isfinite(v[i])) nonfinite = 1;
        if (u_opt_out) u_opt_out[i] = v[i];
    }
    if (!stats) return;
    std::memset(stats, 0, sizeof(*stats));
    stats->sum_w = v[n + 0];
    stats->min_cost = v[n + 1];
    stats->max_cost = v[n + 2];
    stats->n_zero_weight = (int64_t)v[n + 3];
    stats->nonfinite = nonfinite;
    if (t.timing) {
        stats->device_us = t.last_iter_us;
        stats->rollout_us = t.last_roll_us;
    }
}

int fetch_result(ccv_mppi_handle* h, double* u_opt_out, ccv_mppi_stats* stats) {
    if (int rc = flush_pending(h)) return rc;
    const size_t n = (size_t)h->R;
    if (h->mail_pending) {
        h->mail_pending = false;
        if (int rc = read_mail(h, n + (stats ? 4u : 0u), h->h_pin)) return rc;
    } else {
        HIP_TRY(h, hipMemcpyAsync(h->h_pin, h->d_nominal, n * sizeof(double), hipMemcpyDeviceToHost, h->stream));
        HIP_TRY(h, hipMemcpyAsync(h->h_pin + n, h->d_stats, 4 * sizeof(double), hipMemcpyDeviceToHost, h->stream));
        HIP_TRY(h, hipStreamSynchronize(h->stream));
    }
    if (stats && h->timing) HIP_TRY(h, timing_collect(*h, h->stream));
    unpack_result(*h, h->R, h->h_pin, u_opt_out, stats);
    return CCV_MPPI_OK;
}

static int r4_prio_levels(int model) {
    auto levels = [](int noise, int dynamics, int distance, int store) { return 16 + (noise | dynamics << 2 | distance << 4 | store << 6); };
    return model == CCV_MPPI_DIFF_DRIVE ? levels(3, 2, 1, 0) : model == CCV_MPPI_STEERING_DIFF_DRIVE ? levels(2, 3, 1, 0) : levels(0, 1, 2, 3);
}

void select_kernels(KernelChoice& k, const Shape& s, const int64_t workgroups, const bool batched) {
    const int64_t cus = s.cu_count;
    const bool fb = s.cfg.model == CCV_MPPI_FULL_BODY;
    const char* kenv = getenv("CCV_MPPI_KERNEL");
    const bool coop = !(kenv && std::strcmp(kenv, "v1") == 0) && k.lds_window;
    const char* forced = batched || !coop ? nullptr : kenv;
    KernelFamily f = coop ? KernelFamily::TwoWave : KernelFamily::Plain;
    if (coop && (!fb || workgroups <= cus)) f = KernelFamily::FourWave;
    if (forced && std::strcmp(forced, "r4") == 0) f = KernelFamily::FourWave;
    if (forced && std::strcmp(forced, "r3") == 0 && !fb) f = KernelFamily::ThreeWave;
    if (forced && std::strcmp(forced, "pc") == 0) f = KernelFamily::TwoWave;
    bool solo = coop && !forced && workgroups > (fb ? (batched ? 1 : 4) : 5) * cus;
    if (forced && std::strcmp(forced, "solo") == 0) solo = true;
    k.stagewise = f;
    k.fused = solo ? KernelFamily::OneWave : f;
    k.prio_rotate = f == KernelFamily::FourWave ? r4_prio_levels(s.cfg.model) : coop ? 1 : 0;
    k.prune = (coop && s.H > 16) ? 1 : 0;
}

int check_config(const ccv_mppi_config* cfg) {
    if (cfg->abi_version != CCV_MPPI_ABI_VERSION) return CCV_MPPI_ERR_INVALID_ARG;
    if (cfg->model < CCV_MPPI_DIFF_DRIVE || cfg->model > CCV_MPPI_FULL_BODY) return CCV_MPPI_ERR_INVALID_ARG;
    if (cfg->num_samples < 1 || cfg->horizon < 3 || cfg->horizon > CCV_MPPI_MAX_HORIZON) return CCV_MPPI_ERR_INVALID_ARG;
    return CCV_MPPI_OK;
}

int check_device(const int device) {
    int ndev = 0;
    if (hipGetDeviceCount(&ndev) != hipSuccess || ndev <= 0) return CCV_MPPI_ERR_NO_DEVICE;
    if (device < 0 || device >= ndev) return CCV_MPPI_ERR_NO_DEVICE;
    return CCV_MPPI_OK;
}

void set_shape(Shape& s, const ccv_mppi_config& cfg, const int pitch, const int nblocks) {
    s.cfg = cfg;
    s.udim = udim_of(cfg.model);
    s.K = cfg.num_samples;
    s.H = cfg.horizon;
    s.R = (s.H - 1) * s.udim;
    s.pitch = pitch;
    s.nchunks = (s.K + kChunk - 1) / kChunk;
    s.nblocks = nblocks;
    hipDeviceProp_t prop;
    if (hipGetDeviceProperties(&prop, cfg.device) == hipSuccess && prop.multiProcessorCount > 0) s.cu_count = prop.multiProcessorCount;
}

int create_buffers(Core* h, const BufferCounts& n) {
    hipError_t e;
    if ((e = hipStreamCreateWithFlags(&h->own_stream, hipStreamNonBlocking)) != hipSuccess) return fail(h, CCV_MPPI_ERR_HIP, "hipStreamCreate", e);
    h->stream = h->own_stream;
    const size_t P = (size_t)h->pitch;
    struct Piece { void** p; size_t bytes; } pieces[] = {
        {(void**)&h->d_z, (size_t)h->R * P * sizeof(float)},
        {(void**)&h->d_xs, (size_t)h->H * P * sizeof(double)},
        {(void**)&h->d_ys, (size_t)h->H * P * sizeof(double)},
        {(void**)&h->d_u, (size_t)h->R * P * sizeof(double)},
        {(void**)&h->d_cost, P * sizeof(double)},
        {(void**)&h->d_w, P * sizeof(double)},
        {(void**)&h->d_partial, (size_t)(h->R + 1) * n.nparts_max * sizeof(double)},
    };
    constexpr size_t kPieceAlign = (size_t)2 << 20;
    size_t arena_bytes = 0;
    for (const Piece& pc : pieces) arena_bytes += (pc.bytes + kPieceAlign - 1) / kPieceAlign * kPieceAlign;
    if ((e = hipMalloc(&h->d_arena, arena_bytes)) != hipSuccess) return fail(h, CCV_MPPI_ERR_ALLOC, "hipMalloc", e);
    if ((e = hipMemset(h->d_arena, 0, arena_bytes)) != hipSuccess) return fail(h, CCV_MPPI_ERR_HIP, "hipMemset", e);
    {
        size_t at = 0;
        for (const Piece& pc : pieces) {
            *pc.p = static_cast<char*>(h->d_arena) + at;
            at += (pc.bytes + kPieceAlign - 1) / kPieceAlign * kPieceAlign;
        }
    }
    struct { double** p; size_t n; } allocs[] = {
        {&h->d_nominal, n.nominal},
        {&h->d_nom_used, (size_t)(CCV_MPPI_MAX_HORIZON + 8) * CCV_MPPI_MAX_UDIM},
        {&h->d_statpart, n.nparts_max * 3},
        {&h->d_vec, n.vec},
        {&h->d_stats, n.stats},
        {n.extra, n.n_extra},
    };
    for (auto& a : allocs) {
        if ((e = hipMalloc(a.p, a.n * sizeof(double))) != hipSuccess) return fail(h, CCV_MPPI_ERR_ALLOC, "hipMalloc", e);
        if ((e = hipMemset(*a.p, 0, a.n * sizeof(double))) != hipSuccess) return fail(h, CCV_MPPI_ERR_HIP, "hipMemset", e);
    }
    if (const char* tv = std::getenv("CCV_MPPI_THROTTLE")) h->throttle = std::strcmp(tv, "0") != 0;
    for (hipEvent_t& te : h->throttle_ev)
        if ((e = hipEventCreateWithFlags(&te, hipEventDisableTiming)) != hipSuccess) return fail(h, CCV_MPPI_ERR_HIP, "hipEventCreate", e);
    h->pin_doubles = n.pin_doubles;
    if ((e = hipHostMalloc(&h->h_pin, h->pin_doubles * sizeof(double), hipHostMallocDefault)) != hipSuccess)
        return fail(h, CCV_MPPI_ERR_ALLOC, "hipHostMalloc", e);
    const size_t mail_bytes = n.mail_slots * 2 * sizeof(unsigned long long);
    if ((e = hipHostMalloc(reinterpret_cast<void**>(&h->h_mail), mail_bytes, hipHostMallocMapped)) != hipSuccess)
        return fail(h, CCV_MPPI_ERR_ALLOC, "hipHostMalloc(mailbox)", e);
    std::memset(h->h_mail, 0, mail_bytes);
    if ((e = hipHostGetDevicePointer(reinterpret_cast<void**>(&h->d_mail), h->h_mail, 0)) != hipSuccess)
        return fail(h, CCV_MPPI_ERR_HIP, "hipHostGetDevicePointer(mailbox)", e);
    if (const char* mv = std::getenv("CCV_MPPI_MAILBOX")) h->use_mail = std::strcmp(mv, "0") != 0;
    if ((e = hipDeviceSynchronize()) != hipSuccess) return fail(h, CCV_MPPI_ERR_HIP, "hipDeviceSynchronize", e);
    return CCV_MPPI_OK;
}

void release_buffers(Core* h) {
    if (h->stream) (void)hipStreamSynchronize(h->stream);
    if (h->own_stream && h->own_stream != h->stream) (void)hipStreamSynchronize(h->own_stream);
    for (hipEvent_t e : h->ev) (void)hipEventDestroy(e);
    for (hipEvent_t e : h->throttle_ev)
        if (e) (void)hipEventDestroy(e);
    void* bufs[] = {h->d_arena, h->d_nominal, h->d_nom_used, h->d_statpart, h->d_vec, h->d_stats,
                    h->d_scratch, h->d_dbg};
    for (void* b : bufs)
        if (b) (void)hipFree(b);
    if (h->h_pin) (void)hipHostFree(h->h_pin);
    if (h->h_mail) (void)hipHostFree(h->h_mail);
    if (h->own_stream) (void)hipStreamDestroy(h->own_stream);
}

int set_stream(Core* h, void* hip_stream) {
    HIP_TRY(h, hipStreamSynchronize(h->stream));
    h->stream = hip_stream ? (hipStream_t)hip_stream : h->own_stream;
    for (bool& u : h->throttle_used) u = false;
    return CCV_MPPI_OK;
}

void track_absmax(const double* u, const size_t n, const int udim, double* absmax) {
    for (int d = 0; d < CCV_MPPI_MAX_UDIM; ++d) absmax[d] = 0.0;
    for (size_t i = 0; i < n; ++i) {
        const double a = std::fabs(u[i]), m = absmax[i % (size_t)udim];
        if (a != a || (m == m && a > m)) absmax[i % (size_t)udim] = a;
    }
}

}

extern "C" {

const char* ccv_mppi_version(void) { return "ccv_mppi_hip 0.1 (gfx950)"; }

int ccv_mppi_udim(int model) {
    if (model < CCV_MPPI_DIFF_DRIVE || model > CCV_MPPI_FULL_BODY) return CCV_MPPI_ERR_INVALID_ARG;
    return udim_of(model);
}

const char* ccv_mppi_last_error(const ccv_mppi_handle* h) { return h ? h->err.c_str() : "null handle"; }

int ccv_mppi_create(const ccv_mppi_config* cfg, ccv_mppi_handle** out) {
    if (!cfg || !out) return CCV_MPPI_ERR_INVALID_ARG;
    *out = nullptr;
    if (int rc = check_config(cfg)) return rc;
    if (cfg->sample_offset < 0 || cfg->sample_offset > INT32_MAX - cfg->num_samples) return CCV_MPPI_ERR_INVALID_ARG;
    if (int rc = check_device(cfg->device)) return rc;
    ccv_mppi_handle* h = new (std::nothrow) ccv_mppi_handle();
    if (!h) return CCV_MPPI_ERR_ALLOC;
    set_shape(*h, *cfg, round_up(cfg->num_samples, 64), (cfg->num_samples + kPcSamples - 1) / kPcSamples);
    const char* env = getenv("CCV_MPPI_WINDOW");
    h->lds_window = !(env && std::strcmp(env, "scalar") == 0);
    select_kernels(*h, *h, h->nblocks, false);
    if (const char* pv = std::getenv("CCV_MPPI_PRIO")) {
        const int v = std::atoi(pv);
        h->prio_rotate = v == 0 ? 0 : (((v >= 2 && v <= 5) || (v >= 16 && v < 16 + 256)) && h->stagewise == KernelFamily::FourWave) ? v : h->prio_rotate;
    }
    if (const char* pv = std::getenv("CCV_MPPI_PRUNE")) h->prune = std::strcmp(pv, "0") != 0;
    if (const char* pv = std::getenv("CCV_MPPI_FAST_CLAMP")) h->fast_clamp_allowed = std::strcmp(pv, "0") != 0;

    auto bail = [&](int code) {
        std::fprintf(stderr, "ccv_mppi_create: %s\n", h->err.c_str());
        ccv_mppi_destroy(h);
        return code;
    };
    const DeviceGuard guard(cfg->device);
    hipError_t e;
    if ((e = hipSetDevice(cfg->device)) != hipSuccess) return bail(fail(h, CCV_MPPI_ERR_NO_DEVICE, "hipSetDevice", e));
    const size_t nparts_max = (size_t)(h->nblocks > h->nchunks ? h->nblocks : h->nchunks);
    const size_t pad = (size_t)(CCV_MPPI_MAX_HORIZON + 8) * CCV_MPPI_MAX_UDIM;
    const size_t R = (size_t)h->R;
    if (int rc = create_buffers(h, BufferCounts{nparts_max, pad, R + 1, 4, &h->d_cmin, 1,
                                                R + 16, R + 4}))
        return bail(rc);
#if defined(CCV_DIAG)
    {
        const size_t dbg_bytes = (size_t)(kDiagHeader + kDiagSlots * kDiagBlocks) * sizeof(unsigned long long);
        if ((e = hipMalloc(&h->d_dbg, dbg_bytes)) != hipSuccess) return bail(fail(h, CCV_MPPI_ERR_ALLOC, "hipMalloc", e));
        if ((e = hipMemset(h->d_dbg, 0, dbg_bytes)) != hipSuccess) return bail(fail(h, CCV_MPPI_ERR_HIP, "hipMemset", e));
        if ((e = hipDeviceSynchronize()) != hipSuccess) return bail(fail(h, CCV_MPPI_ERR_HIP, "hipDeviceSynchronize", e));
    }
#endif
    *out = h;
    return CCV_MPPI_OK;
}

int ccv_mppi_destroy(ccv_mppi_handle* h) {
    if (!h) return CCV_MPPI_ERR_INVALID_ARG;
    const DeviceGuard guard(h->cfg.device);
    (void)hipSetDevice(h->cfg.device);
    release_buffers(h);
    exchange_release(h);
    void* bufs[] = {h->d_cmin, h->d_frame, h->d_path, h->d_trace};
    for (void* b : bufs)
        if (b) (void)hipFree(b);
    delete h;
    return CCV_MPPI_OK;
}

int ccv_mppi_set_stream(ccv_mppi_handle* h, void* hip_stream) {
    if (!h) return CCV_MPPI_ERR_INVALID_ARG;
    if (int rc = flush_pending(h)) return rc;
    return set_stream(h, hip_stream);
}

int ccv_mppi_synchronize(ccv_mppi_handle* h) {
    if (!h) return CCV_MPPI_ERR_INVALID_ARG;
    if (int rc = flush_pending(h)) return rc;
    HIP_TRY(h, hipStreamSynchronize(h->stream));
    return exchange_check(h);
}

int ccv_mppi_set_nominal(ccv_mppi_handle* h, const double* u) {
    if (!h || !u) return CCV_MPPI_ERR_INVALID_ARG;
    h->pending_vec = nullptr;
    if (int rc = flush_pending(h)) return rc;
    HIP_TRY(h, hipMemcpyAsync(h->d_nominal, u, (size_t)h->R * sizeof(double), hipMemcpyHostToDevice, h->stream));
    HIP_TRY(h, hipStreamSynchronize(h->stream));
    track_absmax(u, (size_t)h->R, h->udim, h->nom_absmax);
    return CCV_MPPI_OK;
}

int ccv_mppi_get_nominal(ccv_mppi_handle* h, double* u) {
    if (!h || !u) return CCV_MPPI_ERR_INVALID_ARG;
    if (int rc = flush_pending(h)) return rc;
    HIP_TRY(h, hipMemcpyAsync(u, h->d_nominal, (size_t)h->R * sizeof(double), hipMemcpyDeviceToHost, h->stream));
    HIP_TRY(h, hipStreamSynchronize(h->stream));
    return exchange_check(h);
}

int ccv_mppi_iterate(ccv_mppi_handle* h, const double* x0, double dt, const double* x_ref, const double* y_ref,
                     double yaw_ref0, uint64_t seed, uint64_t iter, double* u_opt_out, ccv_mppi_stats* stats) {
    int rc = check_iter_args(h, x0, dt, x_ref, y_ref);
    if (rc) return rc;
    h->want_mail = !(stats && h->timing);
    rc = enqueue_iteration(h, x0, dt, x_ref, y_ref, yaw_ref0, seed, iter, true, nullptr);
    h->want_mail = false;
    if (rc) return rc;
    return fetch_result(h, u_opt_out, stats);
}

int ccv_mppi_iterate_enqueue(ccv_mppi_handle* h, const double* x0, double dt, const double* x_ref, const double* y_ref,
                             double yaw_ref0, uint64_t seed, uint64_t iter) {
    int rc = check_iter_args(h, x0, dt, x_ref, y_ref);
    if (rc) return rc;
    return enqueue_iteration(h, x0, dt, x_ref, y_ref, yaw_ref0, seed, iter, true, nullptr);
}

int ccv_mppi_partials_size(const ccv_mppi_handle* h) { return h ? h->R + 1 : CCV_MPPI_ERR_INVALID_ARG; }

int ccv_mppi_iterate_partials_enqueue(ccv_mppi_handle* h, const double* x0, double dt, const double* x_ref,
                                      const double* y_ref, double yaw_ref0, uint64_t seed, uint64_t iter,
                                      double* dev_partials) {
    int rc = check_iter_args(h, x0, dt, x_ref, y_ref);
    if (rc) return rc;
    if (!dev_partials) return fail(h, CCV_MPPI_ERR_INVALID_ARG, "dev_partials is null");
    if (h->cfg.flags & CCV_MPPI_FLAG_MIN_SHIFT)
        return fail(h, CCV_MPPI_ERR_INVALID_ARG, "MIN_SHIFT needs a cross-device min; not supported with partials");
    return enqueue_iteration(h, x0, dt, x_ref, y_ref, yaw_ref0, seed, iter, false, dev_partials);
}

int ccv_mppi_apply_partials_enqueue(ccv_mppi_handle* h, const double* dev_partials) {
    if (!h || !dev_partials) return CCV_MPPI_ERR_INVALID_ARG;
    if (int rc = flush_pending(h)) return rc;
    h->pending_vec = dev_partials;
    return CCV_MPPI_OK;
}

}
```

ccv_mppi_path_tracker_amd/csrc/k_update.hip:

```cpp
#include "mppi_update_device.h"

namespace ccv {

__global__ __launch_bounds__(kBlock) void k_materialize_controls(const MaterializeArgs A) {
    const int k = blockIdx.x * kBlock + threadIdx.x;
    const int n = blockIdx.y;
    if (k >= A.K) return;
    const int d = n % A.udim;
    double v = (double)A.z[(size_t)n * A.pitch + k] * A.sigma + A.nominal_used[n];
    v = clampd(v, A.umin[d], A.umax[d]);
    if (d == A.zero_dim) v = 0.0;
    A.u[(size_t)n * A.pitch + k] = v;
}

__device__ __forceinline__ void update_partials(const UpdateArgs& A) {
    __shared__ double red[4][4];
    const int row = blockIdx.y;
    const int chunk = blockIdx.x;
    const int base = chunk * kChunk;
    const bool wrow = row == A.R;
    const double* urow = A.u + (size_t)row * A.pitch;
    double acc = 0.0, mn = INFINITY, mx = -INFINITY, nz = 0.0;
#pragma unroll
    for (int i = 0; i < kChunk / (2 * kBlock); ++i) {
        const int k = base + i * 2 * kBlock + threadIdx.x * 2;
        if (k + 1 < A.K) {
            const double2 wv = *reinterpret_cast<const double2*>(A.w + k);
            if (wrow) {
                acc += wv.x;
                acc += wv.y;
                const double2 cv = *reinterpret_cast<const double2*>(A.cost + k);
                mn = fmin(mn, fmin(cv.x, cv.y));
                mx = fmax(mx, fmax(cv.x, cv.y));
                nz += (wv.x == 0.0 ? 1.0 : 0.0) + (wv.y == 0.0 ? 1.0 : 0.0);
            } else {
                const double2 uv = *reinterpret_cast<const double2*>(urow + k);
                acc += wv.x * uv.x;
                acc += wv.y * uv.y;
            }
        } else if (k < A.K) {
            const double wv = A.w[k];
            if (wrow) {
                acc += wv;
                const double cv = A.cost[k];
                mn = fmin(mn, cv);
                mx = fmax(mx, cv);
                nz += (wv == 0.0 ? 1.0 : 0.0);
            } else {
                acc += wv * urow[k];
            }
        }
    }
    const int lane = threadIdx.x & 63, wid = threadIdx.x >> 6;
    acc = wave_sum(acc);
    if (wrow) {
        mn = wave_min(mn);
        mx = wave_max(mx);
        nz = wave_sum(nz);
    }
    if (lane == 0) {
        red[0][wid] = acc;
        red[1][wid] = mn;
        red[2][wid] = mx;
        red[3][wid] = nz;
    }
    __syncthreads();
    if (threadIdx.x == 0) {
        A.partial[(size_t)row * A.nchunks + chunk] = (red[0][0] + red[0][1]) + (red[0][2] + red[0][3]);
        if (wrow) {
            A.statpart[chunk * 3 + 0] = fmin(fmin(red[1][0], red[1][1]), fmin(red[1][2], red[1][3]));
            A.statpart[chunk * 3 + 1] = fmax(fmax(red[2][0], red[2][1]), fmax(red[2][2], red[2][3]));
            A.statpart[chunk * 3 + 2] = (red[3][0] + red[3][1]) + (red[3][2] + red[3][3]);
        }
    }
}
__global__ __launch_bounds__(kBlock) void k_update_partials(const UpdateArgs A) { update_partials(A); }
__global__ __launch_bounds__(kBlock) void k_update_partials_batch(UpdateArgs A, const int kpad) {
    const size_t b = blockIdx.z;
    A.u += b * kpad;
    A.w += b * kpad;
    A.cost += b * kpad;
    A.partial += b * (size_t)(A.R + 1) * A.nchunks;
    A.statpart += b * (size_t)A.nchunks * 3;
    update_partials(A);
}

__global__ __launch_bounds__(kBlock) void k_finalize(const FinalizeArgs A) { finalize_rows(A, (size_t)A.nchunks, RowSum<false>{}); }

__global__ __launch_bounds__(kBlock) void k_finalize_batch(FinalizeArgs A, const int fused) {
    const size_t b = blockIdx.y;
    const size_t stride = fused ? (size_t)gridDim.y * A.nchunks : (size_t)A.nchunks;
    A.partial += fused ? b * A.nchunks : b * (size_t)(A.R + 1) * A.nchunks;
    A.statpart += b * (size_t)A.nchunks * 3;
    A.nominal += b * A.R;
    A.vec += b * (size_t)(A.R + 1);
    A.stats += b * 4;
    if (A.mail) A.mail += 2 * b * (size_t)(A.R + 4);
    finalize_rows(A, stride, RowSum<false>{});
}
__global__ __launch_bounds__(kBlock) void k_finalize_batch_shift(FinalizeArgs A, const BatchParams* P, const int K) {
    const size_t b = blockIdx.y;
    const size_t stride = (size_t)gridDim.y * A.nchunks;
    A.partial += b * A.nchunks;
    A.statpart += b * (size_t)A.nchunks * 3;
    A.nominal += b * A.R;
    A.vec += b * (size_t)(A.R + 1);
    A.stats += b * 4;
    if (A.mail) A.mail += 2 * b * (size_t)(A.R + 4);
    finalize_rows(A, stride, RowSum<true>{P[b].lambda, K});
}

__device__ __forceinline__ unsigned long long load_system(const unsigned long long* p) {
    unsigned long long v;
    asm volatile("global_load_dwordx2 %0, %1, off sc0 sc1\n\ts_waitcnt vmcnt(0)" : "=&v"(v) : "v"(p) : "memory");
    return v;
}

__global__ __launch_bounds__(kBlock) void k_finalize_exchange(const FinalizeArgs A, const ExchangeArgs X) {
    const int lane = threadIdx.x & 63;
    const int n = blockIdx.x * (kBlock / 64) + (threadIdx.x >> 6);
    if (n > A.R) {
        if (n == A.R + 1) finalize_cost_stats(A, lane);
        return;
    }
    double s, v;
    RowSum<false>{}(A, (size_t)A.nchunks, n < A.R ? n : A.R, lane, s, v);
    const int slot = n < A.R ? 1 + n : 0;
    const double mine = n < A.R ? v : s;
    if (lane < X.world) {
        const uint32_t seq = X.seq;
        store_packets(&X.peer[lane]->pkt[X.parity][X.rank][slot][0], mine, seq);
    }
    if (lane == 0) {
        A.vec[slot] = mine;
        if (n == A.R) A.stats[0] = s;
    }
    const unsigned long long t0 = __builtin_amdgcn_s_memrealtime();
    const unsigned long long* src = &X.local->pkt[X.parity][lane < X.world ? lane : 0][slot][0];
    unsigned long long hi = 0, lo = 0;
    bool arrived = lane >= X.world;
    while (true) {
        if (!arrived) {
            hi = load_system(src + 0);
            lo = load_system(src + 1);
            arrived = (uint32_t)hi == X.seq && (uint32_t)lo == X.seq;
        }
        if (__all(arrived)) break;
        if (__builtin_amdgcn_s_memrealtime() - t0 > X.timeout_ticks) break;
        __builtin_amdgcn_s_sleep(4);
    }
    const bool ok = __all(arrived);
    const double theirs = __longlong_as_double((long long)((hi & 0xFFFFFFFF00000000ull) | (lo >> 32)));
    double acc = 0.0;
    for (int r = 0; r < X.world; ++r) acc += lane_value(theirs, r);
    if (lane == 0) {
        X.reduced[slot] = ok ? acc : __builtin_nan("");
        if (!ok && X.timeout_flag) __hip_atomic_store(X.timeout_flag, 1, __ATOMIC_RELAXED, __HIP_MEMORY_SCOPE_SYSTEM);
    }
}

__global__ __launch_bounds__(kBlock) void k_apply_partials(const double* vec, double* nominal, double* stats, int R) {
    const double S = vec[0];
    if (threadIdx.x == 0) stats[0] = S;
    for (int n = threadIdx.x; n < R; n += kBlock) nominal[n] = vec[1 + n] / S;
}

__device__ __forceinline__ double block_min_cost(const double* cost, const int K) {
    __shared__ double red[16];
    double mn = INFINITY;
    for (int k = threadIdx.x; k < K; k += 1024) mn = fmin(mn, cost[k]);
    mn = wave_min(mn);
    if ((threadIdx.x & 63) == 0) red[threadIdx.x >> 6] = mn;
    __syncthreads();
    double r = red[0];
    if (threadIdx.x == 0) {
        for (int i = 1; i < 16; ++i) r = fmin(r, red[i]);
    }
    return r;
}
__global__ __launch_bounds__(1024) void k_min_cost(const double* cost, int K, double* out_min) {
    const double r = block_min_cost(cost, K);
    if (threadIdx.x == 0) *out_min = r;
}
__global__ __launch_bounds__(kBlock) void k_reweight(const double* cost, const double* cmin, double lambda, int K, double* w) {
    const int k = blockIdx.x * kBlock + threadIdx.x;
    if (k < K) w[k] = exp(-(cost[k] - *cmin) / lambda);
}

__global__ __launch_bounds__(1024) void k_min_cost_batch(const double* cost, int K, int kpad, double* out_min) {
    const double r = block_min_cost(cost + (size_t)blockIdx.x * kpad, K);
    if (threadIdx.x == 0) out_min[blockIdx.x] = r;
}
__global__ __launch_bounds__(kBlock) void k_reweight_batch(const double* cost, const double* cmin, const BatchParams* P, int K,
                                                          int kpad, double* w) {
    const int k = blockIdx.x * kBlock + threadIdx.x;
    const size_t b = blockIdx.y;
    if (k < K) w[b * kpad + k] = exp(-(cost[b * kpad + k] - cmin[b]) / P[b].lambda);
}

__global__ __launch_bounds__(kBlock) void k_gather_xy(const double* xs, const double* ys, int pitch, int H, int first,
                                                      int count, int stride, double* out) {
    const int idx = blockIdx.x * kBlock + threadIdx.x;
    if (idx >= count * H) return;
    const int c = idx / H, t = idx % H;
    const size_t src = (size_t)t * pitch + first + (size_t)c * stride;
    out[(size_t)idx * 2 + 0] = xs[src];
    out[(size_t)idx * 2 + 1] = ys[src];
}

__global__ __launch_bounds__(kTopBlock) void k_top_weights(const double* w, int K, int N, int* idx_out, double* w_out) {
    __shared__ unsigned int hist[256];
    __shared__ unsigned long long s_prefix;
    __shared__ int s_remaining;
    __shared__ int wsum[kTopBlock / 64][2];
    __shared__ int s_base[2];
    const int tid = threadIdx.x, lane = tid & 63, wv = tid >> 6;
    if (tid == 0) {
        s_prefix = 0ull;
        s_remaining = N;
    }
    __syncthreads();
    for (int pass = 7; pass >= 0; --pass) {
        if (tid < 256) hist[tid] = 0u;
        __syncthreads();
        const unsigned long long prefix = s_prefix;
        for (int i = tid; i < K; i += kTopBlock) {
            const unsigned long long key = (unsigned long long)__double_as_longlong(w[i]);
            const bool match = pass == 7 || (key >> (8 * (pass + 1))) == prefix;
            if (match) atomicAdd(&hist[(unsigned int)(key >> (8 * pass)) & 255u], 1u);
        }
        __syncthreads();
        if (tid == 0) {
            int rem = s_remaining, b = 255;
            for (; b > 0; --b) {
                if ((int)hist[b] >= rem) break;
                rem -= (int)hist[b];
            }
            s_remaining = rem;
            s_prefix = (prefix << 8) | (unsigned long long)b;
        }
        __syncthreads();
    }
    const unsigned long long T = s_prefix;
    const int n_equal = s_remaining, n_greater = N - n_equal;
    if (tid == 0) s_base[0] = s_base[1] = 0;
    __syncthreads();
    for (int i0 = 0; i0 < K; i0 += kTopBlock) {
        const int i = i0 + tid;
        const unsigned long long key = i < K ? (unsigned long long)__double_as_longlong(w[i]) : 0ull;
        const int fg = (i < K && key > T) ? 1 : 0, fe = (i < K && key == T) ? 1 : 0;
        const unsigned long long bg = __ballot(fg), be = __ballot(fe);
        const unsigned long long below = lane == 0 ? 0ull : (~0ull >> (64 - lane));
        const int pg = __popcll(bg & below), pe = __popcll(be & below);
        if (lane == 0) {
            wsum[wv][0] = __popcll(bg);
            wsum[wv][1] = __popcll(be);
        }
        __syncthreads();
        int og = s_base[0], oe = s_base[1];
        for (int j = 0; j < wv; ++j) {
            og += wsum[j][0];
            oe += wsum[j][1];
        }
        if (fg) {
            idx_out[og + pg] = i;
            w_out[og + pg] = w[i];
        }
        if (fe && oe + pe < n_equal) {
            idx_out[n_greater + oe + pe] = i;
            w_out[n_greater + oe + pe] = w[i];
        }
        __syncthreads();
        if (tid == 0) {
            int tg = 0, te = 0;
            for (int j = 0; j < kTopBlock / 64; ++j) {
                tg += wsum[j][0];
                te += wsum[j][1];
            }
            s_base[0] += tg;
            s_base[1] += te;
        }
        __syncthreads();
    }
}

__global__ __launch_bounds__(kBlock) void k_gather_xy_list(const double* xs, const double* ys, int pitch, int H, const int* idx,
                                                           int count, double* out) {
    const int j = blockIdx.x * kBlock + threadIdx.x;
    if (j >= count * H) return;
    const int c = j / H, t = j % H;
    const size_t src = (size_t)t * pitch + idx[c];
    out[(size_t)j * 2 + 0] = xs[src];
    out[(size_t)j * 2 + 1] = ys[src];
}

__global__ __launch_bounds__(kBlock) void k_normalise_weights(const double* w, const double* stats, int first, int count,
                                                             double* out) {
    const int i = blockIdx.x * kBlock + threadIdx.x;
    if (i < count) out[i] = w[first + i] / stats[0];
}

__global__ __launch_bounds__(kBlock) void k_normalise_weights_shift(const double* w, const double* statpart, const double* stats,
                                                                   double lambda, int first, int count, double* out) {
    const int i = blockIdx.x * kBlock + threadIdx.x;
    if (i >= count) return;
    const int k = first + i;
    const double sg = exp(-(statpart[(k / kPcSamples) * 3 + 0] - stats[1]) / lambda);
    out[i] = (w[k] * sg) / stats[0];
}

__global__ __launch_bounds__(kAdvanceThreads) void k_advance(const AdvanceArgs A) { advance_body<kAdvanceThreads>(A, A.nominal); }

__global__ __launch_bounds__(kBlock) void k_finalize_advance(const FinalizeArgs F, const AdvanceArgs A) {
    if ((int)blockIdx.x < finalize_blocks(F.R)) {
        finalize_rows(F, (size_t)F.nchunks, RowSum<false>{});
        return;
    }
    __shared__ double cmd[CCV_MPPI_MAX_UDIM + 3];
    if (A.advance) form_command(cmd, F, (size_t)F.nchunks, A.model, RowSum<false>{});
    __syncthreads();
    advance_body<kBlock>(A, cmd);
}

__global__ __launch_bounds__(kBatchAdvanceThreads) void k_advance_batch(const BatchAdvanceArgs G) {
    double* rec;
    const AdvanceArgs A = batch_advance_view(G, (int)blockIdx.x, rec);
    advance_body<kBatchAdvanceThreads, true>(A, A.nominal, rec);
}

template <bool VARIED>
__device__ __forceinline__ void finalize_advance_batch(FinalizeArgs I, const BatchAdvanceArgs& G, const BatchParams* P) {
    const size_t b = blockIdx.y;
    const size_t stride = (size_t)gridDim.y * I.nchunks;
    const RowSum<false> sum{};
    I.partial += b * I.nchunks;
    if ((int)blockIdx.x < finalize_blocks(I.R)) {
        I.statpart += b * (size_t)I.nchunks * 3;
        I.nominal += b * I.R;
        I.vec += b * (size_t)(I.R + 1);
        I.stats += b * 4;
        finalize_rows(I, stride, sum);
        return;
    }
    __shared__ double cmd[CCV_MPPI_MAX_UDIM + 3];
    if (G.advance) form_command(cmd, I, stride, G.model, sum);
    __syncthreads();
    double* rec;
    const AdvanceArgs A = batch_advance_view<VARIED>(G, (int)b, rec, P);
    advance_body<kBlock, true>(A, cmd, rec);
}
__global__ __launch_bounds__(kBlock) void k_finalize_advance_batch(FinalizeArgs F, const BatchAdvanceArgs G) {
    finalize_advance_batch<false>(F, G, nullptr);
}

__global__ __launch_bounds__(kBatchAdvanceThreads) void k_advance_batch_varied(const BatchAdvanceArgs G, const BatchParams* P) {
    double* rec;
    const AdvanceArgs A = batch_advance_view<true>(G, (int)blockIdx.x, rec, P);
    advance_body<kBatchAdvanceThreads, true>(A, A.nominal, rec);
}
__global__ __launch_bounds__(kBlock) void k_finalize_advance_batch_varied(FinalizeArgs F, const BatchAdvanceArgs G,
                                                                           const BatchParams* P) {
    finalize_advance_batch<true>(F, G, P);
}

__global__ __launch_bounds__(kBlock) void k_finalize_advance_batch_shift(FinalizeArgs F, const BatchAdvanceArgs G, const BatchParams* P) {
    const size_t b = blockIdx.y;
    const size_t stride = (size_t)gridDim.y * F.nchunks;
    const double lambda = P[b].lambda;
    F.partial += b * F.nchunks;
    F.statpart += b * (size_t)F.nchunks * 3;
    if ((int)blockIdx.x < finalize_blocks(F.R)) {
        F.nominal += b * F.R;
        F.vec += b * (size_t)(F.R + 1);
        F.stats += b * 4;
        finalize_rows(F, stride, RowSum<true>{lambda, G.K});
        return;
    }
    __shared__ double cmd[CCV_MPPI_MAX_UDIM + 3];
    if (G.advance) {
        const int lane = threadIdx.x & 63, wv = threadIdx.x >> 6, ud = udim_of(G.model);
        for (int d = wv; d < ud; d += kBlock / 64) {
            double s, v;
            shift_scaled_sum2(F.partial + (size_t)F.R * stride, F.partial + (size_t)d * stride, F.statpart, lambda, F.nchunks, lane, s, v);
            s = wave_sum(s);
            v = wave_sum(v);
            if (lane == 0) cmd[d] = v / s;
        }
    }
    __syncthreads();
    double* rec;
    const AdvanceArgs A = batch_advance_view<true>(G, (int)b, rec, P);
    advance_body<kBlock, true>(A, cmd, rec);
}

}
```

ccv_mppi_path_tracker_amd/csrc/mppi_launch.h:

```cpp
#pragma once
#include <hip/hip_runtime.h>
#include <hip/hip_ext.h>

#include "mppi_kernels.h"

namespace ccv {

struct LaunchAt {
    hipStream_t stream;
    hipEvent_t ev_start, ev_stop;
};

enum class KernelFamily : int { Plain, TwoWave, ThreeWave, FourWave, OneWave };

struct RolloutPlan {
    KernelFamily family;
    int model;
    int mode;
    bool wide;
    int batch;
    BatchForm form;
    bool shift;
    bool lds_window;
};

constexpr bool has_one_wave_form(const int model, const BatchForm form) { return !(model == CCV_MPPI_FULL_BODY && form >= BatchForm::Grid); }

void launch_rollout(const RolloutPlan& plan, const LaunchAt& at, const RolloutArgs& A, const Window& W);
void launch_sample(int model, hipStream_t stream, const RolloutArgs& A);

template <class KERNEL>
inline void launch_at(KERNEL kernel, const dim3 grid, const dim3 block, const LaunchAt& at, const RolloutArgs& A, const Window& W) {
    if (at.ev_start) hipExtLaunchKernelGGL(kernel, grid, block, 0, at.stream, at.ev_start, at.ev_stop, 0, A, W);
    else hipLaunchKernelGGL(kernel, grid, block, 0, at.stream, A, W);
}
inline dim3 blocks_of_64(const RolloutArgs& A, const int batch) { return dim3((unsigned)(batch ? batch : 1) * (unsigned)((A.K + 63) / 64)); }
inline dim3 blocks_plain(const RolloutArgs& A, const int batch) { return dim3((unsigned)((A.K + kBlock - 1) / kBlock), (unsigned)(batch ? batch : 1)); }

}
```

ccv_mppi_path_tracker_amd/csrc/mppi_launch.hip:

```cpp
#include "mppi_launch.h"
#include "mppi_rollout_pc.h"

namespace ccv {

void launch_r4(const RolloutPlan& p, bool tail, const LaunchAt& at, const RolloutArgs& A, const Window& W);
void launch_r4_fb(const RolloutPlan& p, bool tail, const LaunchAt& at, const RolloutArgs& A, const Window& W);
void launch_r3(const RolloutPlan& p, const LaunchAt& at, const RolloutArgs& A, const Window& W);
void launch_pc(const RolloutPlan& p, const LaunchAt& at, const RolloutArgs& A, const Window& W);
void launch_pc_fb(const RolloutPlan& p, const LaunchAt& at, const RolloutArgs& A, const Window& W);
void launch_solo(const RolloutPlan& p, const LaunchAt& at, const RolloutArgs& A, const Window& W);
void launch_solo_fb(const RolloutPlan& p, const LaunchAt& at, const RolloutArgs& A, const Window& W);
void launch_plain(const RolloutPlan& p, const LaunchAt& at, const RolloutArgs& A, const Window& W);
void launch_batch(const RolloutPlan& p, bool tail, const LaunchAt& at, const RolloutArgs& A, const Window& W);
void launch_batch_varied(const RolloutPlan& p, bool tail, const LaunchAt& at, const RolloutArgs& A, const Window& W);
void launch_batch_shift(const RolloutPlan& p, bool tail, const LaunchAt& at, const RolloutArgs& A, const Window& W);
void launch_batch_obst(const RolloutPlan& p, bool tail, const LaunchAt& at, const RolloutArgs& A, const Window& W);
void launch_batch_obst_shift(const RolloutPlan& p, bool tail, const LaunchAt& at, const RolloutArgs& A, const Window& W);
void launch_batch_moving(const RolloutPlan& p, bool tail, const LaunchAt& at, const RolloutArgs& A, const Window& W);
void launch_batch_moving_shift(const RolloutPlan& p, bool tail, const LaunchAt& at, const RolloutArgs& A, const Window& W);
void launch_batch_grid(const RolloutPlan& p, bool tail, const LaunchAt& at, const RolloutArgs& A, const Window& W);
void launch_batch_grid_shift(const RolloutPlan& p, bool tail, const LaunchAt& at, const RolloutArgs& A, const Window& W);

void launch_rollout(const RolloutPlan& p, const LaunchAt& at, const RolloutArgs& A, const Window& W) {
    const bool fb = p.model == CCV_MPPI_FULL_BODY;
    const bool tail = (A.H - 1) % kTU >= kPartialMin;
    const bool shift = p.shift && p.family != KernelFamily::Plain;
    switch (p.form) {
    case BatchForm::Grid: return shift ? launch_batch_grid_shift(p, tail, at, A, W) : launch_batch_grid(p, tail, at, A, W);
    case BatchForm::Moving: return shift ? launch_batch_moving_shift(p, tail, at, A, W) : launch_batch_moving(p, tail, at, A, W);
    case BatchForm::Obst: return shift ? launch_batch_obst_shift(p, tail, at, A, W) : launch_batch_obst(p, tail, at, A, W);
    case BatchForm::Varied: return shift ? launch_batch_shift(p, tail, at, A, W) : launch_batch_varied(p, tail, at, A, W);
    case BatchForm::Batch:
        if (p.family == KernelFamily::Plain) return launch_plain(p, at, A, W);
        return p.family == KernelFamily::FourWave && !fb ? launch_r4(p, tail, at, A, W) : launch_batch(p, tail, at, A, W);
    case BatchForm::Single: break;
    }
    switch (p.family) {
    case KernelFamily::Plain: return launch_plain(p, at, A, W);
    case KernelFamily::TwoWave: return fb ? launch_pc_fb(p, at, A, W) : launch_pc(p, at, A, W);
    case KernelFamily::ThreeWave: return launch_r3(p, at, A, W);
    case KernelFamily::FourWave: return fb ? launch_r4_fb(p, tail, at, A, W) : launch_r4(p, tail, at, A, W);
    case KernelFamily::OneWave: return fb ? launch_solo_fb(p, at, A, W) : launch_solo(p, at, A, W);
    }
}

}
```

ccv_mppi_path_tracker_amd/csrc/mppi_rollout_r4.h:

```cpp
#pragma once
#include "mppi_rollout_r3.h"

namespace ccv {

constexpr int kR4Waves = 4;
template <int MODEL>
constexpr int kR4RB = MODEL == CCV_MPPI_FULL_BODY ? 15 : 12;

struct R4Rows {
    static constexpr int BR = 60;
    int first, n;
    __device__ __forceinline__ int count() const { return n; }
    __device__ __forceinline__ int row(const int m) const { return first + m; }
};
template <int UD>
__device__ __forceinline__ R4Rows r4_rows(const int H, const int nblocks, const int wv, int& nb_early) {
    const int R = (H - 1) * UD;
    nb_early = max(0, nblocks - 3);
    if (nb_early == 0) {
        const int per = ((R / UD + kR4Waves - 1) / kR4Waves) * UD;
        const int first = min(R, wv * per);
        return R4Rows{first, min(per, R - first)};
    }
    const int r_early = min(R, nb_early * kTU * UD);
    const int half_e = ((r_early / UD + 1) / 2) * UD, half_l = (((R - r_early) / UD + 1) / 2) * UD;
    switch (wv) {
        case 0: return R4Rows{0, half_e};
        case 1: return R4Rows{half_e, r_early - half_e};
        case 2: return R4Rows{r_early, half_l};
        default: return R4Rows{r_early + half_l, R - r_early - half_l};
    }
}
template <class T>
__device__ __forceinline__ void r4_fetch0(const RolloutArgs& A, T (&v)[kUpdCH], const R4Rows& rows, const int kk) {
    const size_t pitch = (size_t)A.pitch;
    const char* p0;
    if constexpr (std::is_same<T, float>::value) p0 = reinterpret_cast<const char*>(A.z + (size_t)rows.first * pitch);
    else p0 = reinterpret_cast<const char*>(A.u + (size_t)rows.first * pitch);
    const uint32_t koff = (uint32_t)kk * (uint32_t)sizeof(T);
#pragma unroll
    for (int i = 0; i < kUpdCH; ++i) {
        v[i] = 0;
        if (i < rows.n) v[i] = *reinterpret_cast<const T*>(p0 + (size_t)i * (pitch * sizeof(T)) + koff);
    }
}

template <int MODEL>
struct R4Shared {
    static constexpr bool kStage = true;
    static constexpr int kPBuf = 2;
    double p[2][kTU][2][kPcSamples];
    double2 ab[kMaxH + 4];
    double c[kMaxH + 4];
    float zs[2][kTU * udim_of(MODEL)][kPcSamples];
    double cost[kR4Waves][kPcSamples];
    alignas(32) double nom[(kMaxH + 8) * udim_of(MODEL)];
    int seq[8];
    int nan_seen[kR4Waves];
};

template <int MODEL, class SH>
__device__ __forceinline__ void r4_noise_block(const RolloutArgs& A, SH& sh, const int b, const int lane, const uint32_t kg) {
    constexpr int UD = udim_of(MODEL), NCALL = kTU * UD / 4;
    auto group = [&](auto C0_, auto CN_) {
        constexpr int C0 = decltype(C0_)::value, CN = decltype(CN_)::value;
        float z[4 * CN];
        pc_block_normals<MODEL, C0, CN>(A, b, kg, z);
#pragma unroll
        for (int i = 0; i < 4 * CN; ++i) sh.zs[b & 1][4 * C0 + i][lane] = z[i];
    };
    using std::integral_constant;
    if constexpr (NCALL == 4) {
        group(integral_constant<int, 0>{}, integral_constant<int, 4>{});
    } else if constexpr (NCALL == 6) {
        group(integral_constant<int, 0>{}, integral_constant<int, 3>{});
        group(integral_constant<int, 3>{}, integral_constant<int, 3>{});
    } else {
        static_assert(NCALL == 10, "full body: 4 + 3 + 3 Philox calls");
        group(integral_constant<int, 0>{}, integral_constant<int, 4>{});
        group(integral_constant<int, 4>{}, integral_constant<int, 3>{});
        group(integral_constant<int, 7>{}, integral_constant<int, 3>{});
    }
}

template <int MODEL, class SH>
__device__ __forceinline__ void r4_noise_call(const RolloutArgs& A, SH& sh, const int b, const int call, const int lane, const uint32_t kg) {
    constexpr int UD = udim_of(MODEL);
    const Philox4 r = philox4x32_10(kg, (uint32_t)((b * kTU * UD) >> 2) + (uint32_t)call, A.iter_lo, A.iter_hi, A.seed_lo, A.seed_hi);
    float z[4];
    box_muller_f32(r.x, r.y, z[0], z[1]);
    box_muller_f32(r.z, r.w, z[2], z[3]);
#pragma unroll
    for (int i = 0; i < 4; ++i) sh.zs[b & 1][4 * call + i][lane] = z[i];
}

template <int MODEL, int NT>
struct R4Staged {
    static constexpr int kPerThread = ((kMaxH - 1 + kTU) * udim_of(MODEL) + NT - 1) / NT;
    double wa, wb, wc;
    double nv[kPerThread];
    double S;
};
template <int MODEL, int NT, bool BATCH = false>
__device__ __forceinline__ void r4_stage_issue(const RolloutArgs& A, const Window& Wk, const int tid, R4Staged<MODEL, NT>& L) {
    static_assert(NT >= kMaxH + 4, "one window point per thread");
    const int H = A.H, R = (H - 1) * udim_of(MODEL);
    L.wa = L.wb = 0.0;
    L.wc = INFINITY;
    if (tid < H) {
        if constexpr (BATCH) {
            const double* win = reinterpret_cast<const double*>(A.frame) + kBatchHeadDoubles;
            L.wa = win[tid];
            L.wb = win[H + tid];
            L.wc = win[2 * H + tid];
        } else if (A.frame) {
            const Window& W = A.frame->W;
            L.wa = W.a[tid];
            L.wb = W.b[tid];
            L.wc = W.c[tid];
        } else {
            L.wa = Wk.a[tid];
            L.wb = Wk.b[tid];
            L.wc = Wk.c[tid];
        }
    }
    const double* src = A.pending_vec ? A.pending_vec + 1 : A.nominal;
    L.S = A.pending_vec ? A.pending_vec[0] : 1.0;
#pragma unroll
    for (int i = 0; i < R4Staged<MODEL, NT>::kPerThread; ++i) {
        const int j = tid + i * NT;
        L.nv[i] = j < R ? src[j] : 0.0;
    }
}
template <int MODEL, int NT, class SH>
__device__ __forceinline__ bool r4_stage_commit(const RolloutArgs& A, SH& sh, const int tid, const R4Staged<MODEL, NT>& L) {
    const int H = A.H, H4 = (H + 3) & ~3, R = (H - 1) * udim_of(MODEL);
    if (tid < H4) {
        sh.ab[tid] = make_double2(L.wa, L.wb);
        sh.c[tid] = L.wc;
    }
    bool bad = false;
#pragma unroll
    for (int i = 0; i < R4Staged<MODEL, NT>::kPerThread; ++i) {
        const int j = tid + i * NT;
        if (j < R + kTU * udim_of(MODEL)) {
            const double v = (A.pending_vec && j < R) ? L.nv[i] / L.S : L.nv[i];
            sh.nom[j] = v;
            bad |= v != v;
            if (blockIdx.x == 0 && j < R) {
                if (A.pending_vec) A.nominal_w[j] = v;
                A.nominal_used[j] = v;
            }
        }
    }
    if (A.pending_vec && blockIdx.x == 0 && tid == 0) A.stats_w[0] = L.S;
    return bad;
}

struct R4Lane {
    int lane, k, kk;
    bool live;
    uint32_t kg;
};
__device__ __forceinline__ R4Lane r4_lane(const RolloutArgs& A) {
    R4Lane L;
    L.lane = (int)__builtin_amdgcn_mbcnt_hi(~0u, __builtin_amdgcn_mbcnt_lo(~0u, 0u));
    asm volatile("" : "+v"(L.lane));
    L.k = (int)blockIdx.x * kPcSamples + L.lane;
    L.live = L.k < A.K;
    L.kk = L.live ? L.k : A.K - 1;
    L.kg = (uint32_t)(A.k_offset + L.kk);
    return L;
}

template <int MODEL, int MODE, bool WIDE = false, bool TAIL = false, BatchForm FORM = BatchForm::Single, bool SHIFT = false>
__global__ __launch_bounds__(kR4Waves * 64, MODEL == CCV_MPPI_FULL_BODY ? 1 : 4) void k_rollout_r4(const RolloutArgs Ak, const Window Wk) {
    constexpr bool BATCH = FORM >= BatchForm::Batch, VARIED = FORM >= BatchForm::Varied, OBST = FORM >= BatchForm::Obst,
                   MOVING = FORM >= BatchForm::Moving, GRID = FORM >= BatchForm::Grid;
    constexpr bool FB = MODEL == CCV_MPPI_FULL_BODY;
    constexpr bool COST = MODE != MODE_ROLLOUT;
    constexpr int UD = udim_of(MODEL);
    static_assert(!WIDE || (MODEL == CCV_MPPI_DIFF_DRIVE && MODE == MODE_FUSED), "the wide-turn form exists for the fused diff-drive iteration");
    static_assert(!TAIL || MODE == MODE_FUSED, "the stage-wise modes carry the masked producer anyway");
    static_assert(!BATCH || MODE == MODE_FUSED, "batch handles run the fused iteration only");
    static_assert(!SHIFT || VARIED, "the shifted weights are built on the per-instance-parameter kernels");
    static_assert(!OBST || MODE == MODE_FUSED, "the obstacle term is the fused iteration's");
    __shared__ R4Shared<MODEL> sh;
    ObstLds* obst_lds = nullptr;
    ObstMovLds* obst_mov = nullptr;
    if constexpr (MOVING) {
        __shared__ ObstMovLds s_obst_mov;
        obst_mov = &s_obst_mov;
    } else if constexpr (OBST) {
        __shared__ ObstLds s_obst;
        obst_lds = &s_obst;
    }
    static_assert(offsetof(R4Shared<MODEL>, zs) + sizeof(sh.zs) >= kR4Waves * kR4RB<MODEL> * (kPcSamples + 2) * sizeof(double), "epilogue buffers");
    touch_rollout_args();
    const RolloutArgs A = rollout_view<MODEL, BATCH, VARIED>(Ak);
    if (A.prio_rotate) pc_set_priority((int)blockIdx.x / A.cu_count);
    const int H = A.H;
    const int wv = __builtin_amdgcn_readfirstlane(threadIdx.x >> 6);
    if (wv == 0) CCV_DIAG_STAMP(A, 0);
    const int nblocks = (H + kTU - 1) / kTU;
    const int nstates = FB ? H - 2 : H;
    const int nfull = MODE == MODE_FUSED ? (TAIL ? (H - 1 + kTU - kPartialMin) / kTU : (H - 1) / kTU) : 0;
    int* const seq_noise = &sh.seq[0];
    if (threadIdx.x < 8) sh.seq[threadIdx.x] = (threadIdx.x == 0 && nfull > 0) ? 1 : 0;
    PcState<MODEL> S;
    bool bad_nominal = false;
    if constexpr (MODE == MODE_FUSED) {
        R4Staged<MODEL, kR4Waves * 64> staged;
        r4_stage_issue<MODEL, kR4Waves * 64, BATCH>(A, Wk, (int)threadIdx.x, staged);
        if (nfull > 0) {
            constexpr int NCALL = kTU * UD / 4;
            const R4Lane L = r4_lane(A);
            for (int c = wv; c < NCALL; c += kR4Waves) r4_noise_call<MODEL>(A, sh, 0, c, L.lane, L.kg);
        }
        if (wv == 0) CCV_DIAG_STAMP(A, 3);
        if (wv == 1) {
            S.x = A.x0[0];
            S.y = A.x0[1];
            S.yaw = A.x0[2];
            S.roll = A.x0[3];
            S.pitch = A.x0[4];
            S.p_v = S.p_rv = S.p_sdir = S.p_c2 = S.p_c3 = S.p_ac = 0.0;
            S.p_cdir = 1.0;
            fast_sincos(A.x0[2], S.sn, S.cs);
            CCV_DIAG_STAMP(A, 1);
        }
        bad_nominal = r4_stage_commit<MODEL>(A, sh, (int)threadIdx.x, staged);
        if constexpr (MOVING) {
            const int j = (int)threadIdx.x - 2 * 64;
            if (j >= 0 && j < kMaxObst) obst_stage_moving(A, *obst_mov, j);
        } else if constexpr (OBST) {
            const int j = (int)threadIdx.x - 2 * 64;
            if (j >= 0 && j < kMaxObst) obst_stage(A, *obst_lds, j);
        }
        const bool wave_bad = __builtin_amdgcn_ballot_w64(bad_nominal) != 0ull;
        if (r4_lane(A).lane == 0) sh.nan_seen[wv] = wave_bad ? 1 : 0;
    } else {
        if constexpr (COST) stage_window(A, Wk, sh, kR4Waves * 64);
        if (wv == 1) {
            S.x = A.x0[0];
            S.y = A.x0[1];
            S.yaw = A.x0[2];
            S.roll = A.x0[3];
            S.pitch = A.x0[4];
            S.p_v = S.p_rv = S.p_sdir = S.p_c2 = S.p_c3 = S.p_ac = 0.0;
            S.p_cdir = 1.0;
            fast_sincos(A.x0[2], S.sn, S.cs);
        }
    }
    __syncthreads();
    if (wv == 1) CCV_DIAG_STAMP(A, 2);
    const bool fast_clamp = MODE == MODE_FUSED && A.fast_clamp &&
                            __builtin_amdgcn_readfirstlane(sh.nan_seen[0] | sh.nan_seen[1] | sh.nan_seen[2] | sh.nan_seen[3]) == 0;
    int* const seq_ready = &sh.seq[1];
    int* const seq_dist = &sh.seq[2];
    int* const seq_store = &sh.seq[3];
    int* const seq_stored = &sh.seq[4];
    int nb_early;
    R4Rows rows = r4_rows<UD>(H, nblocks, wv, nb_early);
    if (!(COST && A.fuse_update)) rows.n = 0;
    UpdT<MODE> upd[kUpdCH];
    auto early_fetch = [&]() {
        if constexpr (MODE == MODE_FUSED) {
            if (rows.n > 0 && nb_early > 0) {
                pc_wait_for(seq_stored, nb_early);
                r4_fetch0(A, upd, rows, r4_lane(A).kk);
            }
        }
    };
    if (wv == 0) {
        if constexpr (MODE == MODE_FUSED) {
            const R4Lane L = r4_lane(A);
            const int lane = L.lane;
            const uint32_t kg = L.kg;
            for (int b = 1; b < nfull; ++b) {
                r4_rotate_priority(A, b, 0);
                if (b >= 2) {
                    pc_wait_for(seq_ready, b - 1);
                    pc_wait_for(seq_store, b - 1);
                }
                r4_noise_block<MODEL>(A, sh, b, lane, kg);
                pc_publish(seq_noise, b + 1);
            }
            CCV_DIAG_STAMP(A, 15);
        }
        if constexpr (COST) sh.cost[0][r4_lane(A).lane] = 0.0;
        if (A.prio_rotate) __builtin_amdgcn_s_setprio(0);
        early_fetch();
    } else if (wv == 1) {
        const R4Lane L = r4_lane(A);
        const int lane = L.lane, k = L.k, kk = L.kk;
        const bool live = L.live;
        const uint32_t kg = L.kg;
        double cost = 0.0;
        if constexpr (FB && COST) cost += A.w_yaw * (A.x0[2] - A.yaw_ref0) * (A.x0[2] - A.yaw_ref0);
        for (int b = 0; b < nblocks; ++b) {
            r4_rotate_priority(A, b, 1);
            if (b >= 2) {
                pc_wait_for(seq_dist, b - 1);
                pc_wait_for(seq_store, b - 1);
            }
            const int nctl = min(kTU, H - 1 - b * kTU);
            if (b < nfull) {
                pc_wait_for(seq_noise, b + 1);
                if (b == 0) CCV_DIAG_STAMP(A, 4);
                if (!TAIL || nctl == kTU) {
                    if (fast_clamp)
                        pc_produce_batched<MODEL, MODE, R4Shared<MODEL>, true, true, WIDE>(A, sh, S, cost, b, lane, k, kk, live, kg);
                    else
                        pc_produce_batched<MODEL, MODE, R4Shared<MODEL>, true, false, WIDE>(A, sh, S, cost, b, lane, k, kk, live, kg);
                } else if constexpr (TAIL) {
                    if (fast_clamp && nctl == 6)
                        pc_produce_batched<MODEL, MODE, R4Shared<MODEL>, true, true, WIDE, true, 6>(A, sh, S, cost, b, lane, k, kk, live, kg, nullptr, nctl);
                    else if (fast_clamp)
                        pc_produce_batched<MODEL, MODE, R4Shared<MODEL>, true, true, WIDE, true>(A, sh, S, cost, b, lane, k, kk, live, kg, nullptr, nctl);
                    else
                        pc_produce_batched<MODEL, MODE, R4Shared<MODEL>, true, false, WIDE, true>(A, sh, S, cost, b, lane, k, kk, live, kg, nullptr, nctl);
                }
            } else if (MODE != MODE_FUSED && nctl == kTU) {
                pc_produce_batched<MODEL, MODE>(A, sh, S, cost, b, lane, k, kk, live, kg);
            } else if (MODE != MODE_FUSED && nctl >= kPartialMin) {
                pc_produce_batched<MODEL, MODE, R4Shared<MODEL>, false, false, false, true>(A, sh, S, cost, b, lane, k, kk, live, kg, nullptr, nctl);
            } else {
                pc_produce<MODEL, MODE, false>(A, sh, S, cost, b, lane, k, kk, live, kg);
            }
            pc_publish(seq_ready, b + 1);
            if (b == 0) CCV_DIAG_STAMP(A, 5);
        }
        CCV_DIAG_STAMP(A, 6);
        if constexpr (COST) sh.cost[1][lane] = cost;
        if (A.prio_rotate) __builtin_amdgcn_s_setprio(0);
        early_fetch();
    } else if (wv == 2) {
        int prune_on = 1;
        const int lane = r4_lane(A).lane;
        double cost = 0.0;
        for (int b = 0; b < nblocks; ++b) {
            r4_rotate_priority(A, b, 2);
            pc_wait_for(seq_ready, b + 1);
            bool taken = false;
            if constexpr (COST) {
                const int nv = min(kR3CStates, nstates - b * kTU);
                taken = nv > 0;
                switch (nv) {
                    case 8: pc_consume<8, MODEL, R4Shared<MODEL>, true, OBST, MOVING>(A, sh, cost, b, lane, 0, &prune_on, seq_dist, b + 1, obst_lds, obst_mov); break;
                    case 7: pc_consume<7, MODEL, R4Shared<MODEL>, true, OBST, MOVING>(A, sh, cost, b, lane, 0, &prune_on, seq_dist, b + 1, obst_lds, obst_mov); break;
                    case 6: pc_consume<6, MODEL, R4Shared<MODEL>, true, OBST, MOVING>(A, sh, cost, b, lane, 0, &prune_on, seq_dist, b + 1, obst_lds, obst_mov); break;
                    case 5: pc_consume<5, MODEL, R4Shared<MODEL>, true, OBST, MOVING>(A, sh, cost, b, lane, 0, &prune_on, seq_dist, b + 1, obst_lds, obst_mov); break;
                    case 4: pc_consume<4, MODEL, R4Shared<MODEL>, true, OBST, MOVING>(A, sh, cost, b, lane, 0, &prune_on, seq_dist, b + 1, obst_lds, obst_mov); break;
                    case 3: pc_consume<3, MODEL, R4Shared<MODEL>, true, OBST, MOVING>(A, sh, cost, b, lane, 0, &prune_on, seq_dist, b + 1, obst_lds, obst_mov); break;
                    case 2: pc_consume<2, MODEL, R4Shared<MODEL>, true, OBST, MOVING>(A, sh, cost, b, lane, 0, &prune_on, seq_dist, b + 1, obst_lds, obst_mov); break;
                    case 1: pc_consume<1, MODEL, R4Shared<MODEL>, true, OBST, MOVING>(A, sh, cost, b, lane, 0, &prune_on, seq_dist, b + 1, obst_lds, obst_mov); break;
                    default: break;
                }
            }
            if (!taken) pc_publish(seq_dist, b + 1);
            if (b == 0) CCV_DIAG_STAMP(A, 14);
        }
        CCV_DIAG_STAMP(A, 7);
        if constexpr (COST) sh.cost[2][lane] = cost;
    } else {
        const size_t pitch = (size_t)A.pitch;
        const R4Lane L = r4_lane(A);
        const int lane = L.lane;
        const uint32_t koff4 = (uint32_t)L.k * 4u, koff8 = (uint32_t)L.k * 8u;
        GridAcc grid_acc{};
        if constexpr (GRID) grid_acc = GridAcc{grid_row(A), 0.0, nstates, nullptr};
        for (int b = 0; b < nblocks; ++b) {
            r4_rotate_priority(A, b, 3);
            pc_wait_for(seq_ready, b + 1);
            const int t0 = b * kTU;
            float zv[kTU * UD];
            double xv[kTU], yv[kTU];
            if constexpr (MODE == MODE_FUSED) {
#pragma unroll
                for (int r = 0; r < kTU * UD; ++r) zv[r] = sh.zs[b & 1][r][lane];
            }
            if constexpr (MODE != MODE_COST) {
#pragma unroll
                for (int tt = 0; tt < kTU; ++tt) {
                    xv[tt] = sh.p[b & 1][tt][0][lane];
                    yv[tt] = sh.p[b & 1][tt][1][lane];
                }
            }
            asm volatile("s_waitcnt lgkmcnt(0)" ::: "memory");
            pc_publish(seq_store, b + 1);
            GridTap tap[kTU];
            if constexpr (GRID) {
                grid_issue(grid_acc, xv, yv, tap);
            }
            if constexpr (MODE == MODE_FUSED) {
                const int nrows = min(kTU, H - 1 - t0) * UD;
                char* const zrow = reinterpret_cast<char*>(A.z + (size_t)(t0 * UD) * pitch);
                static_for<kTU * UD>([&](auto RR) {
                    constexpr int r = decltype(RR)::value;
                    if (r < nrows) pc_store_f32(zrow + (size_t)r * (pitch * 4), koff4, zv[r]);
                });
            }
            if constexpr (MODE != MODE_COST) {
                if (A.store_xy) {
                    const int nst = min(kTU, H - t0);
                    char* const xrow = reinterpret_cast<char*>(A.xs + (size_t)t0 * pitch);
                    char* const yrow = reinterpret_cast<char*>(A.ys + (size_t)t0 * pitch);
#pragma unroll
                    for (int tt = 0; tt < kTU; ++tt) {
                        if (tt < nst) {
                            pc_store_f64_stream(xrow + (size_t)tt * (pitch * 8), koff8, xv[tt]);
                            pc_store_f64_stream(yrow + (size_t)tt * (pitch * 8), koff8, yv[tt]);
                        }
                    }
                }
            }
            if constexpr (GRID) {
                grid_sum(grid_acc, tap, t0);
            }
            if constexpr (MODE == MODE_FUSED) {
                constexpr int kRowsZ = kTU * UD, kRowsAll = kTU * UD + 2 * kTU;
                static_assert(kRowsAll <= 63, "vmcnt is a 6-bit counter");
                if (t0 + kTU <= H - 1 && A.store_xy) asm volatile("s_waitcnt vmcnt(%0)" ::"n"(kRowsAll) : "memory");
                else if (t0 + kTU <= H - 1) asm volatile("s_waitcnt vmcnt(%0)" ::"n"(kRowsZ) : "memory");
                else asm volatile("s_waitcnt vmcnt(0)" ::: "memory");
                pc_publish(seq_stored, b);
            }
        }
        asm volatile("s_waitcnt vmcnt(0)" ::: "memory");
        if constexpr (GRID) sh.cost[3][lane] = grid_acc.G;
        else if constexpr (COST) sh.cost[3][lane] = 0.0;
    }
    if (A.prio_rotate) __builtin_amdgcn_s_setprio(0);
    if constexpr (COST) {
        const int R = (H - 1) * UD;
        const int mcount = rows.n;
        const R4Lane L = r4_lane(A);
        const int lane = L.lane, k = L.k, kk = L.kk;
        const bool live = L.live;
        pc_barrier_lds();
        if (wv == 0) CCV_DIAG_STAMP(A, 8);
        bool from_lds = false;
        if constexpr (MODE == MODE_FUSED) {
            from_lds = nblocks <= 2;
            if (from_lds) {
                constexpr int kMaxLdsRows = 4 * UD;
                static_assert(kMaxLdsRows <= kUpdCH, "first chunk");
#pragma unroll
                for (int i = 0; i < kMaxLdsRows; ++i) {
                    const int row = rows.first + min(i, max(mcount - 1, 0));
                    upd[i] = sh.zs[(row / (kTU * UD)) & 1][row % (kTU * UD)][lane];
                }
                pc_barrier_lds();
            }
        }
        if (!from_lds && (MODE != MODE_FUSED || wv >= 2 || nb_early == 0) && mcount > 0) r4_fetch0(A, upd, rows, kk);
        double total_;
        if constexpr (GRID) {
            total_ = ((sh.cost[0][lane] + sh.cost[1][lane]) + sh.cost[2][lane]) + 0.0;
            const ConstGridRow g = grid_row(A);
            if (g) total_ = fma(g->w, sh.cost[3][lane], total_);
        } else {
            total_ = ((sh.cost[0][lane] + sh.cost[1][lane]) + sh.cost[2][lane]) + sh.cost[3][lane];
        }
        const double total = total_;
        double wgt_;
        if constexpr (SHIFT) wgt_ = pc_shifted_weight(A, total, live);
        else wgt_ = live ? exp(-total / A.lambda) : 0.0;
        const double wgt = wgt_;
        if (wv == 0 && live) {
            A.cost[k] = total;
            A.w[k] = wgt;
        }
        if (wv == 0) CCV_DIAG_STAMP_VALUE(A, 9, wgt);
        if (wv == 2) CCV_DIAG_STAMP_VALUE(A, 11, wgt);
        if (A.fuse_update) {
            double* buf = &sh.p[0][0][0][0] + wv * (kR4RB<MODEL> * (kPcSamples + 2));
            pc_reduce_rows<kR4RB<MODEL>, MODEL, true>(A, sh, buf, upd, rows, mcount, wgt, lane, kk, fast_clamp);
            if (wv == kR4Waves - 1) pc_block_stats(A, R, wgt, total, live, lane);
        }
        if (wv == 0) CCV_DIAG_STAMP(A, 10);
        if (wv == 2) CCV_DIAG_STAMP(A, 12);
        if (wv == 3) CCV_DIAG_STAMP(A, 13);
    }
}

}
```

ccv_mppi_path_tracker_amd/csrc/mppi_update.h:

```cpp
#pragma once
#include "mppi_kernels.h"

namespace ccv {

struct MaterializeArgs {
    const float* z;
    const double* nominal_used;
    double* u;
    double sigma;
    double umin[5], umax[5];
    int32_t K, pitch, R, udim, zero_dim;
};
__global__ void k_materialize_controls(MaterializeArgs A);

struct UpdateArgs {
    const double* u;
    const double* w;
    const double* cost;
    double* partial;
    double* statpart;
    int32_t K, pitch, R, nchunks;
};
__global__ void k_update_partials(UpdateArgs A);
__global__ void k_update_partials_batch(UpdateArgs A, int kpad);

struct FinalizeArgs {
    const double* partial;
    const double* statpart;
    double* nominal;
    double* vec;
    double* stats;
    int32_t R, nchunks, normalise;
    unsigned long long* mail;
    uint32_t mail_seq;
};
constexpr int finalize_blocks(int R) { return (R + 2 + kBlock / 64 - 1) / (kBlock / 64); }
__global__ void k_finalize(FinalizeArgs A);
__global__ void k_finalize_batch(FinalizeArgs A, int fused);
__global__ void k_finalize_batch_shift(FinalizeArgs A, const BatchParams* P, int K);

constexpr int kMaxRanks = 8;
constexpr int kMaxVec = 1 + (kMaxH - 1) * CCV_MPPI_MAX_UDIM;
struct ExchangeBox {
    unsigned long long pkt[2][kMaxRanks][kMaxVec][2];
};
struct ExchangeArgs {
    ExchangeBox* peer[kMaxRanks];
    ExchangeBox* local;
    double* reduced;
    uint32_t seq;
    int32_t world, rank, parity;
    unsigned long long timeout_ticks;
    int32_t* timeout_flag;
};
__global__ void k_finalize_exchange(FinalizeArgs A, ExchangeArgs X);
__global__ void k_apply_partials(const double* vec, double* nominal, double* stats, int R);

__global__ void k_min_cost(const double* cost, int K, double* out_min);
__global__ void k_reweight(const double* cost, const double* cmin, double lambda, int K, double* w);
__global__ void k_min_cost_batch(const double* cost, int K, int kpad, double* out_min);
__global__ void k_reweight_batch(const double* cost, const double* cmin, const BatchParams* P, int K, int kpad, double* w);

__global__ void k_gather_xy(const double* xs, const double* ys, int pitch, int H, int first, int count, int stride, double* out);
constexpr int kTopBlock = 1024;
__global__ void k_top_weights(const double* w, int K, int N, int* idx_out, double* w_out);
__global__ void k_gather_xy_list(const double* xs, const double* ys, int pitch, int H, const int* idx, int count, double* out);
__global__ void k_normalise_weights(const double* w, const double* stats, int first, int count, double* out);
__global__ void k_normalise_weights_shift(const double* w, const double* statpart, const double* stats, double lambda, int first,
                                          int count, double* out);

}
```

include/ccv_mppi.h:

```cpp
#ifndef CCV_MPPI_H_
#define CCV_MPPI_H_

#include <stdint.h>

#ifdef __cplusplus
extern "C" {
#endif

#define CCV_MPPI_ABI_VERSION 1
#define CCV_MPPI_MAX_UDIM 5
#define CCV_MPPI_MAX_HORIZON 128

#define CCV_MPPI_OK 0
#define CCV_MPPI_ERR_INVALID_ARG (-1)
#define CCV_MPPI_ERR_NO_DEVICE (-2)
#define CCV_MPPI_ERR_HIP (-3)
#define CCV_MPPI_ERR_STATE (-4)
#define CCV_MPPI_ERR_ALLOC (-5)
#define CCV_MPPI_ERR_TIMEOUT (-6)

#define CCV_MPPI_DIFF_DRIVE 0
#define CCV_MPPI_STEERING_DIFF_DRIVE 1
#define CCV_MPPI_FULL_BODY 2

#define CCV_MPPI_FLAG_ROLL_OFF 0x1
#define CCV_MPPI_FLAG_STEER_OFF 0x2
#define CCV_MPPI_FLAG_MIN_SHIFT 0x4
#define CCV_MPPI_FLAG_NO_STATE_STORE 0x8

typedef struct ccv_mppi_config {
    int32_t abi_version;
    int32_t model;
    int32_t num_samples;
    int32_t horizon;
    int32_t sample_offset;
    int32_t device;
    int32_t flags;
    int32_t reserved;
    double control_noise;
    double lambda;
    double v_ref;
    double u_min[CCV_MPPI_MAX_UDIM];
    double u_max[CCV_MPPI_MAX_UDIM];
    double path_weight;
    double v_weight;
    double zmp_weight;
    double roll_v_weight;
    double back_weight;
    double yaw_weight;
} ccv_mppi_config;

typedef struct ccv_mppi_stats {
    double sum_w;
    double min_cost;
    double max_cost;
    int64_t n_zero_weight;
    int32_t nonfinite;
    int32_t reserved;
    float device_us;
    float rollout_us;
} ccv_mppi_stats;

typedef struct ccv_mppi_handle ccv_mppi_handle;

int ccv_mppi_create(const ccv_mppi_config* cfg, ccv_mppi_handle** out);
int ccv_mppi_destroy(ccv_mppi_handle* h);
int ccv_mppi_set_stream(ccv_mppi_handle* h, void* hip_stream);
const char* ccv_mppi_last_error(const ccv_mppi_handle* h);
const char* ccv_mppi_version(void);
int ccv_mppi_udim(int model);

int ccv_mppi_set_nominal(ccv_mppi_handle* h, const double* u);
int ccv_mppi_get_nominal(ccv_mppi_handle* h, double* u);

int ccv_mppi_iterate(ccv_mppi_handle* h, const double* x0, double dt, const double* x_ref, const double* y_ref,
                     double yaw_ref0, uint64_t seed, uint64_t iter, double* u_opt_out, ccv_mppi_stats* stats);
int ccv_mppi_iterate_enqueue(ccv_mppi_handle* h, const double* x0, double dt, const double* x_ref,
                             const double* y_ref, double yaw_ref0, uint64_t seed, uint64_t iter);
int ccv_mppi_synchronize(ccv_mppi_handle* h);

int ccv_mppi_sample(ccv_mppi_handle* h, uint64_t seed, uint64_t iter);
int ccv_mppi_inject_controls(ccv_mppi_handle* h, const double* u_samples);
int ccv_mppi_rollout(ccv_mppi_handle* h, const double* x0, double dt);
int ccv_mppi_weights(ccv_mppi_handle* h, const double* x_ref, const double* y_ref, double yaw_ref0);
int ccv_mppi_update(ccv_mppi_handle* h, double* u_opt_out, ccv_mppi_stats* stats);

int ccv_mppi_read_candidates(ccv_mppi_handle* h, int32_t first, int32_t count, int32_t stride, double* xy_out);
int ccv_mppi_read_top_candidates(ccv_mppi_handle* h, int32_t count, int32_t* sample_out, double* weight_out, double* xy_out);
int ccv_mppi_read_costs(ccv_mppi_handle* h, int32_t first, int32_t count, double* out);
int ccv_mppi_read_weights(ccv_mppi_handle* h, int32_t first, int32_t count, double* out);
int ccv_mppi_read_controls(ccv_mppi_handle* h, int32_t first, int32_t count, double* out);

int ccv_mppi_partials_size(const ccv_mppi_handle* h);
int ccv_mppi_iterate_partials_enqueue(ccv_mppi_handle* h, const double* x0, double dt, const double* x_ref,
                                      const double* y_ref, double yaw_ref0, uint64_t seed, uint64_t iter,
                                      double* dev_partials);
int ccv_mppi_apply_partials_enqueue(ccv_mppi_handle* h, const double* dev_partials);

int ccv_mppi_exchange_handle_bytes(void);
int ccv_mppi_exchange_create(ccv_mppi_handle* h, int32_t world, int32_t rank, void* ipc_handle_out);
int ccv_mppi_exchange_connect(ccv_mppi_handle* h, const void* ipc_handles);
int ccv_mppi_exchange_info(const ccv_mppi_handle* h, int32_t* world, int32_t* rank, int32_t* fine_grained, int32_t* connected);
int ccv_mppi_iterate_exchange_enqueue(ccv_mppi_handle* h, const double* x0, double dt, const double* x_ref,
                                      const double* y_ref, double yaw_ref0, uint64_t seed, uint64_t iter);

int ccv_mppi_resident_set_path(ccv_mppi_handle* h, const double* path_x, const double* path_y, int32_t n_path,
                               double resolution);
int ccv_mppi_resident_set_pose(ccv_mppi_handle* h, const double* state);
int ccv_mppi_resident_step_enqueue(ccv_mppi_handle* h, double dt, uint64_t seed, uint64_t iter, int32_t advance);
int ccv_mppi_resident_step_partials_enqueue(ccv_mppi_handle* h, double dt, uint64_t seed, uint64_t iter, int32_t advance,
                                            double* dev_partials);
int ccv_mppi_resident_step_exchange_enqueue(ccv_mppi_handle* h, double dt, uint64_t seed, uint64_t iter, int32_t advance);
int ccv_mppi_resident_read(ccv_mppi_handle* h, double* state, int32_t* current_index, double* x_ref, double* y_ref,
                           double* yaw_ref0, int64_t* steps);
int ccv_mppi_resident_read_trace(ccv_mppi_handle* h, int32_t max_rows, double* rows, int32_t* n_rows);

int ccv_mppi_timing_enable(ccv_mppi_handle* h, int32_t on);
int ccv_mppi_timing_read(ccv_mppi_handle* h, double* rollout_us_sum, double* iter_us_sum, int64_t* n_iters,
                         int32_t reset);

#define CCV_MPPI_BATCH_MAX_SAMPLES (1 << 29)
#define CCV_MPPI_BATCH_KERNEL_PLAIN 0
#define CCV_MPPI_BATCH_KERNEL_ONE_WAVE 1
#define CCV_MPPI_BATCH_KERNEL_FOUR_WAVE 4
#define CCV_MPPI_BATCH_KERNEL_WIDE 16
#define CCV_MPPI_BATCH_KERNEL_VARIED 32
#define CCV_MPPI_BATCH_KERNEL_SHIFT 64
#define CCV_MPPI_BATCH_KERNEL_OBST 128
#define CCV_MPPI_BATCH_KERNEL_MOVING 256
#define CCV_MPPI_BATCH_KERNEL_GRID 512
#define CCV_MPPI_MAX_OBSTACLES 32
#define CCV_MPPI_GRID_MAX_DIM 32768
#define CCV_MPPI_GRID_MAX_CELLS (1 << 26)

typedef struct ccv_mppi_batch ccv_mppi_batch;

int ccv_mppi_batch_create(const ccv_mppi_config* cfg, int32_t batch, ccv_mppi_batch** out);
int ccv_mppi_batch_destroy(ccv_mppi_batch* b);
int ccv_mppi_batch_set_stream(ccv_mppi_batch* b, void* hip_stream);
int ccv_mppi_batch_synchronize(ccv_mppi_batch* b);
const char* ccv_mppi_batch_last_error(const ccv_mppi_batch* b);
int ccv_mppi_batch_size(const ccv_mppi_batch* b);
int ccv_mppi_batch_last_kernel(const ccv_mppi_batch* b);
int ccv_mppi_batch_set_nominal(ccv_mppi_batch* b, const double* u);
int ccv_mppi_batch_get_nominal(ccv_mppi_batch* b, double* u);
int ccv_mppi_batch_set_params(ccv_mppi_batch* b, const ccv_mppi_config* cfgs);
int ccv_mppi_batch_get_params(ccv_mppi_batch* b, ccv_mppi_config* out);
int ccv_mppi_batch_set_min_shift(ccv_mppi_batch* b, int32_t on);
int ccv_mppi_batch_get_min_shift(const ccv_mppi_batch* b);
int ccv_mppi_batch_set_obstacles(ccv_mppi_batch* b, const double* xyr, const int32_t* n, int32_t max_n, const double* weight);
int ccv_mppi_batch_get_obstacles(ccv_mppi_batch* b, double* xyr, int32_t* n, int32_t max_n, double* weight);
int ccv_mppi_batch_set_obstacle_velocities(ccv_mppi_batch* b, const double* vxy, int32_t max_n);
int ccv_mppi_batch_get_obstacle_velocities(ccv_mppi_batch* b, double* vxy, int32_t max_n);
int ccv_mppi_batch_set_fleet_prediction(ccv_mppi_batch* b, int32_t on);
int ccv_mppi_batch_get_fleet_prediction(const ccv_mppi_batch* b);
int ccv_mppi_batch_read_fleet_velocities(ccv_mppi_batch* b, double* vxy);
typedef struct ccv_mppi_grid { double origin_x, origin_y, resolution; float outside; int32_t nx, ny; const float* cells; } ccv_mppi_grid;
int ccv_mppi_batch_set_grids(ccv_mppi_batch* b, const ccv_mppi_grid* maps, int32_t n_maps, const int32_t* map_of, const double* weight);
int ccv_mppi_batch_get_grids(ccv_mppi_batch* b, ccv_mppi_grid* maps, int32_t max_maps, int32_t* n_maps, int32_t* map_of, double* weight);
int ccv_mppi_batch_read_grid_cells(ccv_mppi_batch* b, int32_t map, float* cells_out);
int ccv_mppi_batch_iterate(ccv_mppi_batch* b, const double* x0, const double* dt, const double* x_ref, const double* y_ref,
                           const double* yaw_ref0, const uint64_t* seed, uint64_t iter, double* u_opt_out, ccv_mppi_stats* stats);
int ccv_mppi_batch_iterate_enqueue(ccv_mppi_batch* b, const double* x0, const double* dt, const double* x_ref, const double* y_ref,
                                   const double* yaw_ref0, const uint64_t* seed, uint64_t iter);
int ccv_mppi_batch_read_costs(ccv_mppi_batch* b, int32_t instance, int32_t first, int32_t count, double* out);
int ccv_mppi_batch_read_weights(ccv_mppi_batch* b, int32_t instance, int32_t first, int32_t count, double* out);
int ccv_mppi_batch_read_candidates(ccv_mppi_batch* b, int32_t instance, int32_t first, int32_t count, int32_t stride,
                                   double* xy_out);
int ccv_mppi_batch_timing_enable(ccv_mppi_batch* b, int32_t on);
int ccv_mppi_batch_timing_read(ccv_mppi_batch* b, double* rollout_us_sum, double* iter_us_sum, int64_t* n_iters, int32_t reset);

#define CCV_MPPI_BATCH_TRACE_ROWS 1024
int ccv_mppi_batch_resident_set_paths(ccv_mppi_batch* b, const double* path_x, const double* path_y, const int32_t* n_path,
                                      const double* resolution);
int ccv_mppi_batch_resident_set_poses(ccv_mppi_batch* b, const double* state, const uint64_t* seed);
int ccv_mppi_batch_resident_step_enqueue(ccv_mppi_batch* b, double dt, uint64_t iter, int32_t advance);
int ccv_mppi_batch_resident_read(ccv_mppi_batch* b, double* state, int32_t* current_index, double* x_ref, double* y_ref,
                                 double* yaw_ref0, int64_t* steps);
int ccv_mppi_batch_resident_read_trace(ccv_mppi_batch* b, int32_t instance, int32_t max_rows, double* rows, int32_t* n_rows);

#ifdef __cplusplus
}
#endif
#include "ccv_mppi_fleet.h"
#endif
```

Before: 1.892 billion rollouts/s.

## Draw next iteration's Gaussian noise inside the finalize kernel ahead of rollout

Extends the finalize kernel with extra blocks that generate the Philox/Box-Muller normals for iteration iter+1 into a second z buffer. When the next fused rollout arrives with the matching seed, iteration and stream, the z buffers are swapped and a new AHEAD variant of the four-wave rollout kernel runs. That variant loads the normals from memory instead of generating them and skips writing z back. The aim is to take RNG work and the z store off the rollout's critical path and run them in the otherwise lightly occupied finalize launch. The cost is an extra z-sized allocation, host-side key tracking that must be invalidated on injects, stream changes and errors, and extra global reads in the rollout.

Result: slower. 1.582 billion rollouts/s (-16.4%).

```diff
diff --git a/ccv_mppi_path_tracker_amd/build.py b/ccv_mppi_path_tracker_amd/build.py
--- a/ccv_mppi_path_tracker_amd/build.py
+++ b/ccv_mppi_path_tracker_amd/build.py
@@ -6,7 +6,7 @@
 CSRC = os.path.join(_PKG, "csrc")
 LIBDIR = os.path.join(_PKG, "lib")
 LIB = os.path.join(LIBDIR, "libccv_mppi_hip.so")
-KERNEL_UNITS = ["k_r4_fb.hip", "k_batch.hip", "k_batch_varied.hip", "k_batch_shift.hip", "k_batch_obst.hip", "k_batch_obst_shift.hip", "k_batch_moving.hip", "k_batch_moving_shift.hip", "k_batch_grid.hip", "k_batch_grid_shift.hip", "k_r4.hip", "k_r3.hip", "k_pc.hip", "k_pc_fb.hip",
+KERNEL_UNITS = ["k_r4_fb.hip", "k_batch.hip", "k_batch_varied.hip", "k_batch_shift.hip", "k_batch_obst.hip", "k_batch_obst_shift.hip", "k_batch_moving.hip", "k_batch_moving_shift.hip", "k_batch_grid.hip", "k_batch_grid_shift.hip", "k_r4.hip", "k_r4_ahead.hip", "k_r3.hip", "k_pc.hip", "k_pc_fb.hip",
                 "k_solo.hip", "k_solo_fb.hip", "k_plain.hip", "k_update.hip", "k_fleet.hip", "k_fleet_pred.hip"]
 CAPI_UNITS = ["ccv_mppi_capi.hip", "capi_exchange.hip", "capi_resident.hip", "capi_stage.hip", "capi_batch.hip"]
 SOURCES = KERNEL_UNITS + ["mppi_launch.hip"] + CAPI_UNITS + ["ccv_mppi_host.cpp", os.path.join("host", "mppi_node.cpp")]
diff --git a/ccv_mppi_path_tracker_amd/capi.py b/ccv_mppi_path_tracker_amd/capi.py
--- a/ccv_mppi_path_tracker_amd/capi.py
+++ b/ccv_mppi_path_tracker_amd/capi.py
@@ -18,7 +18,7 @@
 ERR_TIMEOUT = -6
 
 DIFF_DRIVE, STEERING_DIFF_DRIVE, FULL_BODY = 0, 1, 2
-FLAG_ROLL_OFF, FLAG_STEER_OFF, FLAG_MIN_SHIFT, FLAG_NO_STATE_STORE = 0x1, 0x2, 0x4, 0x8
+FLAG_ROLL_OFF, FLAG_STEER_OFF, FLAG_MIN_SHIFT, FLAG_NO_STATE_STORE, FLAG_NO_NOISE_AHEAD = 0x1, 0x2, 0x4, 0x8, 0x10
 BATCH_MAX_SAMPLES = 1 << 29
 BATCH_KERNEL_PLAIN, BATCH_KERNEL_ONE_WAVE, BATCH_KERNEL_FOUR_WAVE, BATCH_KERNEL_WIDE = 0, 1, 4, 16
 BATCH_KERNEL_VARIED = 32
@@ -99,6 +99,7 @@
     "ccv_mppi_resident_read": (C.c_int, [_H, _dp, C.POINTER(C.c_int32), _dp, _dp, _dp, C.POINTER(C.c_int64)]),
     "ccv_mppi_resident_read_trace": (C.c_int, [_H, C.c_int32, _dp, C.POINTER(C.c_int32)]),
     "ccv_mppi_timing_enable": (C.c_int, [_H, C.c_int32]),
+    "ccv_mppi_noise_ahead_hits": (C.c_int, [_H, C.POINTER(C.c_uint64)]),
     "ccv_mppi_timing_read": (C.c_int, [_H, _dp, _dp, C.POINTER(C.c_int64), C.c_int32]),
     "ccv_mppi_batch_create": (C.c_int, [C.POINTER(Config), C.c_int32, C.POINTER(_H)]),
     "ccv_mppi_batch_destroy": (C.c_int, [_H]),
diff --git a/ccv_mppi_path_tracker_amd/controller.py b/ccv_mppi_path_tracker_amd/controller.py
--- a/ccv_mppi_path_tracker_amd/controller.py
+++ b/ccv_mppi_path_tracker_amd/controller.py
@@ -12,7 +12,8 @@
         self.code = code
 
 
-def make_config(p: MPPIParams, device=0, sample_offset=0, min_shift=False, no_state_store=False, num_samples=None):
+def make_config(p: MPPIParams, device=0, sample_offset=0, min_shift=False, no_state_store=False, num_samples=None,
+                no_noise_ahead=False):
     cfg = capi.Config()
     cfg.abi_version = capi.ABI_VERSION
     cfg.model = MODEL_IDS[p.model]
@@ -21,7 +22,8 @@
     cfg.sample_offset = int(sample_offset)
     cfg.device = int(device)
     cfg.flags = ((capi.FLAG_ROLL_OFF if p.roll_off else 0) | (capi.FLAG_STEER_OFF if p.steer_off else 0) |
-                 (capi.FLAG_MIN_SHIFT if min_shift else 0) | (capi.FLAG_NO_STATE_STORE if no_state_store else 0))
+                 (capi.FLAG_MIN_SHIFT if min_shift else 0) | (capi.FLAG_NO_STATE_STORE if no_state_store else 0) |
+                 (capi.FLAG_NO_NOISE_AHEAD if no_noise_ahead else 0))
     cfg.control_noise, cfg.lam, cfg.v_ref = p.control_noise, p.lam, p.v_ref
     for d in range(p.udim):
         cfg.u_min[d], cfg.u_max[d] = p.u_min[d], p.u_max[d]
@@ -33,7 +35,7 @@
 class MPPIController:
 
     def __init__(self, params: MPPIParams, device=0, sample_offset=0, num_samples=None, min_shift=False,
-                 no_state_store=False):
+                 no_state_store=False, no_noise_ahead=False):
         self.lib = capi.load()
         self.params = params
         self.K = int(num_samples if num_samples is not None else params.num_samples)
@@ -41,7 +43,7 @@
         self.udim = params.udim
         self.nstate = params.nstate
         self._h = capi._H()
-        cfg = make_config(params, device, sample_offset, min_shift, no_state_store, self.K)
+        cfg = make_config(params, device, sample_offset, min_shift, no_state_store, self.K, no_noise_ahead)
         rc = self.lib.ccv_mppi_create(C.byref(cfg), C.byref(self._h))
         if rc != capi.OK:
             self._h = capi._H()
@@ -223,6 +225,11 @@
 
     def timing_enable(self, on=True, every=1):
         self._check(self.lib.ccv_mppi_timing_enable(self._h, (max(1, int(every)) if on else 0)))
+
+    def noise_ahead_hits(self):
+        n = C.c_uint64()
+        self._check(self.lib.ccv_mppi_noise_ahead_hits(self._h, C.byref(n)))
+        return n.value
 
     def timing_read(self, reset=True):
         a, b, n = C.c_double(), C.c_double(), C.c_int64()
diff --git a/ccv_mppi_path_tracker_amd/csrc/capi_internal.h b/ccv_mppi_path_tracker_amd/csrc/capi_internal.h
--- a/ccv_mppi_path_tracker_amd/csrc/capi_internal.h
+++ b/ccv_mppi_path_tracker_amd/csrc/capi_internal.h
@@ -98,6 +98,8 @@
     bool fused = true;
     const BatchParams* shift = nullptr;
     int K = 0;
+    bool draw = false;
+    DrawArgs draw_args{};
 };
 
 struct DeferredUpdate {
@@ -105,9 +107,21 @@
     UpdatePlan fin{};
 };
 
-struct Core : Shape, KernelChoice, DeviceBuffers, Mailbox, Throttle, Timing, DeferredUpdate {
+struct NoiseAhead {
+    float* d_z_next = nullptr;
+    float* d_z_second = nullptr;
+    bool key_valid = false;
+    uint64_t key_seed = 0, key_iter = 0;
+    hipStream_t key_stream = nullptr;
+    bool draw_armed = false;
+    uint64_t cur_seed = 0, cur_iter = 0;
+    uint64_t hits = 0;
+};
+
+struct Core : Shape, KernelChoice, DeviceBuffers, Mailbox, Throttle, Timing, DeferredUpdate, NoiseAhead {
     std::string err;
 };
+inline void noise_ahead_drop(NoiseAhead& n) { n.key_valid = n.draw_armed = false; }
 
 struct StageState {
     bool have_controls = false, have_rollout = false, have_weights = false;
@@ -210,6 +224,7 @@
 inline int fail(Core* h, int code, const char* what, hipError_t e = hipSuccess) {
     if (h) {
         h->err = what;
+        if (code == CCV_MPPI_ERR_HIP) noise_ahead_drop(*h);
         if (e != hipSuccess) {
             h->err += ": ";
             h->err += hipGetErrorString(e);
@@ -262,7 +277,7 @@
                              const bool shift) {
     KernelFamily f = trig == kTrigUnsafe ? KernelFamily::Plain : family_of(k, mode);
     if (f == KernelFamily::OneWave && !has_one_wave_form(model, form)) f = KernelFamily::FourWave;
-    return RolloutPlan{f, model, mode, f != KernelFamily::Plain && trig == kTrigWide, batch, form, shift, k.lds_window != 0};
+    return RolloutPlan{f, model, mode, f != KernelFamily::Plain && trig == kTrigWide, batch, form, shift, k.lds_window != 0, false};
 }
 
 RolloutPlan plan_of(const ccv_mppi_handle* h, const RolloutArgs& A, int mode);
diff --git a/ccv_mppi_path_tracker_amd/csrc/capi_stage.hip b/ccv_mppi_path_tracker_amd/csrc/capi_stage.hip
--- a/ccv_mppi_path_tracker_amd/csrc/capi_stage.hip
+++ b/ccv_mppi_path_tracker_amd/csrc/capi_stage.hip
@@ -21,6 +21,7 @@
 
 int ccv_mppi_inject_controls(ccv_mppi_handle* h, const double* u_samples) {
     if (!h || !u_samples) return CCV_MPPI_ERR_INVALID_ARG;
+    noise_ahead_drop(*h);
     std::vector<double> tmp((size_t)h->R * h->pitch, 0.0);
     for (int d = 0; d < CCV_MPPI_MAX_UDIM; ++d) h->inj_absmax[d] = 0.0;
     for (int i = 0; i < h->K; ++i)
diff --git a/ccv_mppi_path_tracker_amd/csrc/ccv_mppi_capi.hip b/ccv_mppi_path_tracker_amd/csrc/ccv_mppi_capi.hip
--- a/ccv_mppi_path_tracker_amd/csrc/ccv_mppi_capi.hip
+++ b/ccv_mppi_path_tracker_amd/csrc/ccv_mppi_capi.hip
@@ -1,4 +1,5 @@
 #include <chrono>
+#include <utility>
 #include <new>
 
 #include "capi_internal.h"
@@ -98,7 +99,26 @@
     const unsigned blocks = finalize_blocks(p.args.R);
     if (p.batch && p.shift) hipLaunchKernelGGL(k_finalize_batch_shift, dim3(blocks, p.batch), dim3(kBlock), 0, h.stream, p.args, p.shift, p.K);
     else if (p.batch) hipLaunchKernelGGL(k_finalize_batch, dim3(blocks, p.batch), dim3(kBlock), 0, h.stream, p.args, p.fused ? 1 : 0);
+    else if (p.draw)
+        hipLaunchKernelGGL(k_finalize_draw, dim3(blocks + (unsigned)(p.draw_args.col_blocks * draw_call_groups(p.args.R))), dim3(kBlock), 0, h.stream,
+                           p.args, p.draw_args);
     else hipLaunchKernelGGL(k_finalize, dim3(blocks), dim3(kBlock), 0, h.stream, p.args);
+}
+
+static DrawArgs draw_args(const Core& h) {
+    const uint64_t next = h.cur_iter + 1;
+    DrawArgs D;
+    D.z = h.d_z_next;
+    D.seed_lo = (uint32_t)h.cur_seed;
+    D.seed_hi = (uint32_t)(h.cur_seed >> 32);
+    D.iter_lo = (uint32_t)next;
+    D.iter_hi = (uint32_t)(next >> 32);
+    D.K = h.K;
+    D.pitch = h.pitch;
+    D.R = h.R;
+    D.k_offset = h.cfg.sample_offset;
+    D.col_blocks = (h.pitch + kBlock - 1) / kBlock;
+    return D;
 }
 
 void launch_finalize_advance(Core& h, const UpdatePlan& p, const AdvanceArgs& V) {
@@ -195,7 +215,7 @@
 
 int launch_rollout(ccv_mppi_handle* h, const RolloutArgs& A_in, const Window& W, int mode) {
     RolloutArgs A = A_in;
-    const RolloutPlan plan = plan_of(h, A, mode);
+    RolloutPlan plan = plan_of(h, A, mode);
     const bool coop = plan.family != KernelFamily::Plain;
     A.fuse_update = (coop && mode != MODE_ROLLOUT && !(h->cfg.flags & CCV_MPPI_FLAG_MIN_SHIFT)) ? 1 : 0;
     if (int rc = flush_finalize(h)) return rc;
@@ -208,6 +228,19 @@
         }
     }
     if (mode != MODE_ROLLOUT) h->nparts_last = A.fuse_update ? h->nblocks : 0;
+    const bool ahead_ok = mode == MODE_FUSED && h->d_z_next && plan.family == KernelFamily::FourWave && plan.form == BatchForm::Single &&
+                          h->cfg.model != CCV_MPPI_FULL_BODY && A.fuse_update && !A.frame && !A.pending_vec;
+    const uint64_t seed = (uint64_t)A.seed_hi << 32 | A.seed_lo, iter = (uint64_t)A.iter_hi << 32 | A.iter_lo;
+    if (ahead_ok && h->key_valid && h->key_seed == seed && h->key_iter == iter && h->key_stream == h->stream) {
+        std::swap(h->d_z, h->d_z_next);
+        A.z = h->d_z;
+        plan.ahead = true;
+        ++h->hits;
+    }
+    noise_ahead_drop(*h);
+    h->draw_armed = ahead_ok;
+    h->cur_seed = seed;
+    h->cur_iter = iter;
     if (mode != MODE_FUSED) {
         if (int rc = materialize_controls(h)) return rc;
     }
@@ -221,6 +254,7 @@
 }
 
 int launch_sample(ccv_mppi_handle* h, const RolloutArgs& A) {
+    noise_ahead_drop(*h);
     if (int rc = flush_pending(h)) return rc;
     launch_sample(h->cfg.model, h->stream, A);
     HIP_TRY(h, hipGetLastError());
@@ -264,6 +298,8 @@
 }
 
 int launch_update(ccv_mppi_handle* h, bool normalise, double* vec_out, bool exchange, bool defer) {
+    const bool draw_armed = h->draw_armed;
+    h->draw_armed = false;
     if (h->fin_pending) {
         if (int rc = flush_pending(h)) return rc;
     }
@@ -304,8 +340,17 @@
         h->fin_pending = true;
         return CCV_MPPI_OK;
     }
-    launch_finalize(*h, UpdatePlan{F});
+    UpdatePlan up{F};
+    up.draw = draw_armed && normalise && !vec_out && nparts == h->nblocks && nparts == h->nparts_last;
+    if (up.draw) up.draw_args = draw_args(*h);
+    launch_finalize(*h, up);
     HIP_TRY(h, hipGetLastError());
+    if (up.draw) {
+        h->key_valid = true;
+        h->key_seed = h->cur_seed;
+        h->key_iter = h->cur_iter + 1;
+        h->key_stream = h->stream;
+    }
     return CCV_MPPI_OK;
 }
 
@@ -613,6 +658,7 @@
 int set_stream(Core* h, void* hip_stream) {
     HIP_TRY(h, hipStreamSynchronize(h->stream));
     h->stream = hip_stream ? (hipStream_t)hip_stream : h->own_stream;
+    noise_ahead_drop(*h);
     for (bool& u : h->throttle_used) u = false;
     return CCV_MPPI_OK;
 }
@@ -671,6 +717,15 @@
     if (int rc = create_buffers(h, BufferCounts{nparts_max, pad, R + 1, 4, &h->d_cmin, 1,
                                                 R + 16, R + 4}))
         return bail(rc);
+    const char* nav = std::getenv("CCV_MPPI_NOISE_AHEAD");
+    if (!(cfg->flags & (CCV_MPPI_FLAG_NO_NOISE_AHEAD | CCV_MPPI_FLAG_MIN_SHIFT)) && cfg->model != CCV_MPPI_FULL_BODY &&
+        h->fused == KernelFamily::FourWave && !(nav && std::strcmp(nav, "0") == 0)) {
+        const size_t z_bytes = (size_t)h->R * h->pitch * sizeof(float);
+        if ((e = hipMalloc(&h->d_z_second, z_bytes)) != hipSuccess) return bail(fail(h, CCV_MPPI_ERR_ALLOC, "hipMalloc", e));
+        h->d_z_next = h->d_z_second;
+        if ((e = hipMemset(h->d_z_next, 0, z_bytes)) != hipSuccess) return bail(fail(h, CCV_MPPI_ERR_HIP, "hipMemset", e));
+        if ((e = hipDeviceSynchronize()) != hipSuccess) return bail(fail(h, CCV_MPPI_ERR_HIP, "hipDeviceSynchronize", e));
+    }
 #if defined(CCV_DIAG)
     {
         const size_t dbg_bytes = (size_t)(kDiagHeader + kDiagSlots * kDiagBlocks) * sizeof(unsigned long long);
@@ -689,7 +744,7 @@
     (void)hipSetDevice(h->cfg.device);
     release_buffers(h);
     exchange_release(h);
-    void* bufs[] = {h->d_cmin, h->d_frame, h->d_path, h->d_trace};
+    void* bufs[] = {h->d_cmin, h->d_frame, h->d_path, h->d_trace, h->d_z_second};
     for (void* b : bufs)
         if (b) (void)hipFree(b);
     delete h;
@@ -745,6 +800,12 @@
     return enqueue_iteration(h, x0, dt, x_ref, y_ref, yaw_ref0, seed, iter, true, nullptr);
 }
 
+int ccv_mppi_noise_ahead_hits(ccv_mppi_handle* h, uint64_t* hits) {
+    if (!h || !hits) return CCV_MPPI_ERR_INVALID_ARG;
+    *hits = h->hits;
+    return CCV_MPPI_OK;
+}
+
 int ccv_mppi_partials_size(const ccv_mppi_handle* h) { return h ? h->R + 1 : CCV_MPPI_ERR_INVALID_ARG; }
 
 int ccv_mppi_iterate_partials_enqueue(ccv_mppi_handle* h, const double* x0, double dt, const double* x_ref,
diff --git a/ccv_mppi_path_tracker_amd/csrc/k_r4_ahead.hip b/ccv_mppi_path_tracker_amd/csrc/k_r4_ahead.hip
--- /dev/null
+++ b/ccv_mppi_path_tracker_amd/csrc/k_r4_ahead.hip
@@ -0,0 +1,25 @@
+#include "mppi_launch.h"
+#include "mppi_rollout_r4.h"
+
+namespace ccv {
+
+template <int MODEL>
+static void launch_r4_ahead_model(const RolloutPlan& p, bool tail, const LaunchAt& at, const RolloutArgs& A, const Window& W) {
+    const dim3 grid = blocks_of_64(A, 0), block(kR4Waves * 64);
+    if constexpr (MODEL == CCV_MPPI_DIFF_DRIVE) {
+        if (p.wide) {
+            if (tail) launch_at(k_rollout_r4<MODEL, MODE_FUSED, true, true, BatchForm::Single, false, true>, grid, block, at, A, W);
+            else launch_at(k_rollout_r4<MODEL, MODE_FUSED, true, false, BatchForm::Single, false, true>, grid, block, at, A, W);
+            return;
+        }
+    }
+    if (tail) launch_at(k_rollout_r4<MODEL, MODE_FUSED, false, true, BatchForm::Single, false, true>, grid, block, at, A, W);
+    else launch_at(k_rollout_r4<MODEL, MODE_FUSED, false, false, BatchForm::Single, false, true>, grid, block, at, A, W);
+}
+
+void launch_r4_ahead(const RolloutPlan& p, bool tail, const LaunchAt& at, const RolloutArgs& A, const Window& W) {
+    if (p.model == CCV_MPPI_DIFF_DRIVE) launch_r4_ahead_model<CCV_MPPI_DIFF_DRIVE>(p, tail, at, A, W);
+    else launch_r4_ahead_model<CCV_MPPI_STEERING_DIFF_DRIVE>(p, tail, at, A, W);
+}
+
+}
diff --git a/ccv_mppi_path_tracker_amd/csrc/k_update.hip b/ccv_mppi_path_tracker_amd/csrc/k_update.hip
--- a/ccv_mppi_path_tracker_amd/csrc/k_update.hip
+++ b/ccv_mppi_path_tracker_amd/csrc/k_update.hip
@@ -87,6 +87,46 @@
 
 __global__ __launch_bounds__(kBlock) void k_finalize(const FinalizeArgs A) { finalize_rows(A, (size_t)A.nchunks, RowSum<false>{}); }
 
+__global__ __launch_bounds__(kBlock) void k_finalize_draw(const FinalizeArgs A, const DrawArgs D) {
+    const int fb = finalize_blocks(A.R);
+    if ((int)blockIdx.x < fb) {
+        finalize_rows(A, (size_t)A.nchunks, RowSum<false>{});
+        return;
+    }
+    const int j = (int)blockIdx.x - fb;
+    const int k = (j % D.col_blocks) * kBlock + (int)threadIdx.x;
+    const int call0 = (j / D.col_blocks) * kDrawCalls;
+    if (k >= D.pitch) return;
+    const uint32_t kg = (uint32_t)(D.k_offset + min(k, D.K - 1));
+    uint32_t c0[kDrawCalls], c1[kDrawCalls], c2[kDrawCalls], c3[kDrawCalls];
+#pragma unroll
+    for (int i = 0; i < kDrawCalls; ++i) {
+        c0[i] = kg;
+        c1[i] = (uint32_t)(call0 + i);
+        c2[i] = D.iter_lo;
+        c3[i] = D.iter_hi;
+    }
+    philox4x32_10_n<kDrawCalls>(c0, c1, c2, c3, D.seed_lo, D.seed_hi);
+    uint32_t ba[2 * kDrawCalls], bb[2 * kDrawCalls];
+    float z0[2 * kDrawCalls], z1[2 * kDrawCalls];
+#pragma unroll
+    for (int i = 0; i < kDrawCalls; ++i) {
+        ba[2 * i] = c0[i];
+        bb[2 * i] = c1[i];
+        ba[2 * i + 1] = c2[i];
+        bb[2 * i + 1] = c3[i];
+    }
+    box_muller_f32_n<2 * kDrawCalls>(ba, bb, z0, z1);
+    float* const col = D.z + k;
+    const size_t pitch = (size_t)D.pitch;
+#pragma unroll
+    for (int i = 0; i < 2 * kDrawCalls; ++i) {
+        const int n = 4 * call0 + 2 * i;
+        if (n < D.R) col[(size_t)n * pitch] = z0[i];
+        if (n + 1 < D.R) col[(size_t)(n + 1) * pitch] = z1[i];
+    }
+}
+
 __global__ __launch_bounds__(kBlock) void k_finalize_batch(FinalizeArgs A, const int fused) {
     const size_t b = blockIdx.y;
     const size_t stride = fused ? (size_t)gridDim.y * A.nchunks : (size_t)A.nchunks;
diff --git a/ccv_mppi_path_tracker_amd/csrc/mppi_launch.h b/ccv_mppi_path_tracker_amd/csrc/mppi_launch.h
--- a/ccv_mppi_path_tracker_amd/csrc/mppi_launch.h
+++ b/ccv_mppi_path_tracker_amd/csrc/mppi_launch.h
@@ -22,6 +22,7 @@
     BatchForm form;
     bool shift;
     bool lds_window;
+    bool ahead;
 };
 
 constexpr bool has_one_wave_form(const int model, const BatchForm form) { return !(model == CCV_MPPI_FULL_BODY && form >= BatchForm::Grid); }
diff --git a/ccv_mppi_path_tracker_amd/csrc/mppi_launch.hip b/ccv_mppi_path_tracker_amd/csrc/mppi_launch.hip
--- a/ccv_mppi_path_tracker_amd/csrc/mppi_launch.hip
+++ b/ccv_mppi_path_tracker_amd/csrc/mppi_launch.hip
@@ -4,6 +4,7 @@
 namespace ccv {
 
 void launch_r4(const RolloutPlan& p, bool tail, const LaunchAt& at, const RolloutArgs& A, const Window& W);
+void launch_r4_ahead(const RolloutPlan& p, bool tail, const LaunchAt& at, const RolloutArgs& A, const Window& W);
 void launch_r4_fb(const RolloutPlan& p, bool tail, const LaunchAt& at, const RolloutArgs& A, const Window& W);
 void launch_r3(const RolloutPlan& p, const LaunchAt& at, const RolloutArgs& A, const Window& W);
 void launch_pc(const RolloutPlan& p, const LaunchAt& at, const RolloutArgs& A, const Window& W);
@@ -39,7 +40,7 @@
     case KernelFamily::Plain: return launch_plain(p, at, A, W);
     case KernelFamily::TwoWave: return fb ? launch_pc_fb(p, at, A, W) : launch_pc(p, at, A, W);
     case KernelFamily::ThreeWave: return launch_r3(p, at, A, W);
-    case KernelFamily::FourWave: return fb ? launch_r4_fb(p, tail, at, A, W) : launch_r4(p, tail, at, A, W);
+    case KernelFamily::FourWave: return fb ? launch_r4_fb(p, tail, at, A, W) : p.ahead ? launch_r4_ahead(p, tail, at, A, W) : launch_r4(p, tail, at, A, W);
     case KernelFamily::OneWave: return fb ? launch_solo_fb(p, at, A, W) : launch_solo(p, at, A, W);
     }
 }
diff --git a/ccv_mppi_path_tracker_amd/csrc/mppi_rollout_r4.h b/ccv_mppi_path_tracker_amd/csrc/mppi_rollout_r4.h
--- a/ccv_mppi_path_tracker_amd/csrc/mppi_rollout_r4.h
+++ b/ccv_mppi_path_tracker_amd/csrc/mppi_rollout_r4.h
@@ -92,6 +92,23 @@
     box_muller_f32(r.z, r.w, z[2], z[3]);
 #pragma unroll
     for (int i = 0; i < 4; ++i) sh.zs[b & 1][4 * call + i][lane] = z[i];
+}
+
+template <int N>
+__device__ __forceinline__ void r4_load_normals(const RolloutArgs& A, const int R, const int row0, const int kk, float (&v)[N]) {
+    const size_t pitch = (size_t)A.pitch;
+    const char* const p0 = reinterpret_cast<const char*>(A.z + (size_t)row0 * pitch);
+    const uint32_t koff = (uint32_t)kk * 4u;
+    if (row0 + N <= R) {
+#pragma unroll
+        for (int i = 0; i < N; ++i) v[i] = *reinterpret_cast<const float*>(p0 + (size_t)i * (pitch * 4) + koff);
+    } else {
+#pragma unroll
+        for (int i = 0; i < N; ++i) {
+            v[i] = 0.0f;
+            if (row0 + i < R) v[i] = *reinterpret_cast<const float*>(p0 + (size_t)i * (pitch * 4) + koff);
+        }
+    }
 }
 
 template <int MODEL, int NT>
@@ -173,7 +190,7 @@
     return L;
 }
 
-template <int MODEL, int MODE, bool WIDE = false, bool TAIL = false, BatchForm FORM = BatchForm::Single, bool SHIFT = false>
+template <int MODEL, int MODE, bool WIDE = false, bool TAIL = false, BatchForm FORM = BatchForm::Single, bool SHIFT = false, bool AHEAD = false>
 __global__ __launch_bounds__(kR4Waves * 64, MODEL == CCV_MPPI_FULL_BODY ? 1 : 4) void k_rollout_r4(const RolloutArgs Ak, const Window Wk) {
     constexpr bool BATCH = FORM >= BatchForm::Batch, VARIED = FORM >= BatchForm::Varied, OBST = FORM >= BatchForm::Obst,
                    MOVING = FORM >= BatchForm::Moving, GRID = FORM >= BatchForm::Grid;
@@ -185,6 +202,7 @@
     static_assert(!BATCH || MODE == MODE_FUSED, "batch handles run the fused iteration only");
     static_assert(!SHIFT || VARIED, "the shifted weights are built on the per-instance-parameter kernels");
     static_assert(!OBST || MODE == MODE_FUSED, "the obstacle term is the fused iteration's");
+    static_assert(!AHEAD || (MODE == MODE_FUSED && FORM == BatchForm::Single && !FB), "normals drawn ahead: a single handle's fused iteration");
     __shared__ R4Shared<MODEL> sh;
     ObstLds* obst_lds = nullptr;
     ObstMovLds* obst_mov = nullptr;
@@ -215,7 +233,16 @@
         if (nfull > 0) {
             constexpr int NCALL = kTU * UD / 4;
             const R4Lane L = r4_lane(A);
-            for (int c = wv; c < NCALL; c += kR4Waves) r4_noise_call<MODEL>(A, sh, 0, c, L.lane, L.kg);
+            if constexpr (AHEAD) {
+                for (int c = wv; c < NCALL; c += kR4Waves) {
+                    float v[4];
+                    r4_load_normals<4>(A, (H - 1) * UD, 4 * c, L.kk, v);
+#pragma unroll
+                    for (int i = 0; i < 4; ++i) sh.zs[0][4 * c + i][L.lane] = v[i];
+                }
+            } else {
+                for (int c = wv; c < NCALL; c += kR4Waves) r4_noise_call<MODEL>(A, sh, 0, c, L.lane, L.kg);
+            }
         }
         if (wv == 0) CCV_DIAG_STAMP(A, 3);
         if (wv == 1) {
@@ -267,7 +294,7 @@
     auto early_fetch = [&]() {
         if constexpr (MODE == MODE_FUSED) {
             if (rows.n > 0 && nb_early > 0) {
-                pc_wait_for(seq_stored, nb_early);
+                if constexpr (!AHEAD) pc_wait_for(seq_stored, nb_early);
                 r4_fetch0(A, upd, rows, r4_lane(A).kk);
             }
         }
@@ -277,6 +304,23 @@
             const R4Lane L = r4_lane(A);
             const int lane = L.lane;
             const uint32_t kg = L.kg;
+            if constexpr (AHEAD) {
+                constexpr int NR = kTU * UD;
+                const int R = (H - 1) * UD;
+                float zr[NR];
+                if (nfull > 1) r4_load_normals<NR>(A, R, NR, L.kk, zr);
+                for (int b = 1; b < nfull; ++b) {
+                    r4_rotate_priority(A, b, 0);
+                    if (b >= 2) {
+                        pc_wait_for(seq_ready, b - 1);
+                        pc_wait_for(seq_store, b - 1);
+                    }
+#pragma unroll
+                    for (int r = 0; r < NR; ++r) sh.zs[b & 1][r][lane] = zr[r];
+                    pc_publish(seq_noise, b + 1);
+                    if (b + 1 < nfull) r4_load_normals<NR>(A, R, (b + 1) * NR, L.kk, zr);
+                }
+            } else {
             for (int b = 1; b < nfull; ++b) {
                 r4_rotate_priority(A, b, 0);
                 if (b >= 2) {
@@ -285,6 +329,7 @@
                 }
                 r4_noise_block<MODEL>(A, sh, b, lane, kg);
                 pc_publish(seq_noise, b + 1);
+            }
             }
             CCV_DIAG_STAMP(A, 15);
         }
@@ -376,7 +421,7 @@
             const int t0 = b * kTU;
             float zv[kTU * UD];
             double xv[kTU], yv[kTU];
-            if constexpr (MODE == MODE_FUSED) {
+            if constexpr (MODE == MODE_FUSED && !AHEAD) {
 #pragma unroll
                 for (int r = 0; r < kTU * UD; ++r) zv[r] = sh.zs[b & 1][r][lane];
             }
@@ -393,7 +438,7 @@
             if constexpr (GRID) {
                 grid_issue(grid_acc, xv, yv, tap);
             }
-            if constexpr (MODE == MODE_FUSED) {
+            if constexpr (MODE == MODE_FUSED && !AHEAD) {
                 const int nrows = min(kTU, H - 1 - t0) * UD;
                 char* const zrow = reinterpret_cast<char*>(A.z + (size_t)(t0 * UD) * pitch);
                 static_for<kTU * UD>([&](auto RR) {
@@ -419,7 +464,7 @@
                 grid_sum(grid_acc, tap, t0);
             }
             if constexpr (MODE == MODE_FUSED) {
-                constexpr int kRowsZ = kTU * UD, kRowsAll = kTU * UD + 2 * kTU;
+                constexpr int kRowsZ = AHEAD ? 0 : kTU * UD, kRowsAll = kRowsZ + 2 * kTU;
                 static_assert(kRowsAll <= 63, "vmcnt is a 6-bit counter");
                 if (t0 + kTU <= H - 1 && A.store_xy) asm volatile("s_waitcnt vmcnt(%0)" ::"n"(kRowsAll) : "memory");
                 else if (t0 + kTU <= H - 1) asm volatile("s_waitcnt vmcnt(%0)" ::"n"(kRowsZ) : "memory");
diff --git a/ccv_mppi_path_tracker_amd/csrc/mppi_update.h b/ccv_mppi_path_tracker_amd/csrc/mppi_update.h
--- a/ccv_mppi_path_tracker_amd/csrc/mppi_update.h
+++ b/ccv_mppi_path_tracker_amd/csrc/mppi_update.h
@@ -37,6 +37,16 @@
 constexpr int finalize_blocks(int R) { return (R + 2 + kBlock / 64 - 1) / (kBlock / 64); }
 __global__ void k_finalize(FinalizeArgs A);
 __global__ void k_finalize_batch(FinalizeArgs A, int fused);
+
+constexpr int kDrawCalls = 4;
+struct DrawArgs {
+    float* z;
+    uint32_t seed_lo, seed_hi, iter_lo, iter_hi;
+    int32_t K, pitch, R, k_offset;
+    int32_t col_blocks;
+};
+constexpr int draw_call_groups(int R) { return ((R + 3) / 4 + kDrawCalls - 1) / kDrawCalls; }
+__global__ void k_finalize_draw(FinalizeArgs A, DrawArgs D);
 __global__ void k_finalize_batch_shift(FinalizeArgs A, const BatchParams* P, int K);
 
 constexpr int kMaxRanks = 8;
diff --git a/include/ccv_mppi.h b/include/ccv_mppi.h
--- a/include/ccv_mppi.h
+++ b/include/ccv_mppi.h
@@ -27,6 +27,7 @@
 #define CCV_MPPI_FLAG_STEER_OFF 0x2
 #define CCV_MPPI_FLAG_MIN_SHIFT 0x4
 #define CCV_MPPI_FLAG_NO_STATE_STORE 0x8
+#define CCV_MPPI_FLAG_NO_NOISE_AHEAD 0x10
 
 typedef struct ccv_mppi_config {
     int32_t abi_version;
@@ -116,6 +117,7 @@
 int ccv_mppi_resident_read_trace(ccv_mppi_handle* h, int32_t max_rows, double* rows, int32_t* n_rows);
 
 int ccv_mppi_timing_enable(ccv_mppi_handle* h, int32_t on);
+int ccv_mppi_noise_ahead_hits(ccv_mppi_handle* h, uint64_t* hits);
 int ccv_mppi_timing_read(ccv_mppi_handle* h, double* rollout_us_sum, double* iter_us_sum, int64_t* n_iters,
                          int32_t reset);
 
```
